# rasd3/3D-Dual-Fusion

Measured on AMD Instinct MI355X. Metric: nuScenes sweeps/sec (0.075 m voxel, ~60k pts), higher is better.
Workload: dtype f32 (fp32-grade throughout: every matrix-core GEMM -- C>=32 sparse convs, neck / head convs, FFN, query linears, image projection, value GEMM -- takes its fp32 operands as fp16 hi+lo pairs, 22 significand bits, 3 MFMA products, fp32 accumulate: <= 4e-6 of scale against float64, the grade of the exac

## Files before the change

3d-dual-fusion_amd/csrc/spconv_split.hip:

```cpp
#include <stdlib.h>
#include <algorithm>
#include <string.h>

#include "common.h"

namespace df3d {

typedef float f32x4 __attribute__((ext_vector_type(4)));
typedef unsigned int u32x4 __attribute__((ext_vector_type(4)));
typedef unsigned int u32x2 __attribute__((ext_vector_type(2)));
typedef __bf16 bf16x8 __attribute__((ext_vector_type(8)));

int timing_rec_begin(int cin, int cout, int kvol, int n_out, const int32_t *nbr, int split,
                     hipStream_t stream);
void timing_rec_end(int rec, hipStream_t stream);

DF3D_SPLIT_OVERFLOW_TU(spconv_split)

__device__ __forceinline__ void split3_pair_ref(float x0, float x1, unsigned &hi, unsigned &mid, unsigned &lo) {
  unsigned h, m;
  split_pair_bf16(x0, x1, h, m);
  const float r0 = (x0 - __uint_as_float(h << 16)) - __uint_as_float(m << 16);
  const float r1 = (x1 - __uint_as_float(h & 0xffff0000u)) - __uint_as_float(m & 0xffff0000u);
  unsigned l, unused;
// ... 58 lines not shown
  u32x4 ho, lo;
  split_pair(a[0], a[1], ho[0], lo[0]);
  split_pair(a[2], a[3], ho[1], lo[1]);
  split_pair(b[0], b[1], ho[2], lo[2]);
  split_pair(b[2], b[3], ho[3], lo[3]);
  out[2 * i] = ho;
  out[2 * i + 1] = lo;
}

__global__ __launch_bounds__(256) void rows_absmax_kernel(const float *__restrict__ x, size_t n4, size_t n, float *__restrict__ part) {
  float m = 0.f;
  const size_t stride = (size_t)gridDim.x * 256;
  size_t i = (size_t)blockIdx.x * 256 + threadIdx.x;
  auto upd = [&](f32x4 v) {
    m = fmaxf(fmaxf(m, fmaxf(__builtin_fabsf(v[0]), __builtin_fabsf(v[1]))), fmaxf(__builtin_fabsf(v[2]), __builtin_fabsf(v[3])));
    if (!(v[0] == v[0]) || !(v[1] == v[1]) || !(v[2] == v[2]) || !(v[3] == v[3])) m = __builtin_inff();
  };
  for (; i + 3 * stride < n4; i += 4 * stride) {
    const f32x4 v0 = ((const f32x4 *)x)[i], v1 = ((const f32x4 *)x)[i + stride], v2 = ((const f32x4 *)x)[i + 2 * stride],
                v3 = ((const f32x4 *)x)[i + 3 * stride];
    upd(v0), upd(v1), upd(v2), upd(v3);
  }
  for (; i < n4; i += stride) upd(((const f32x4 *)x)[i]);
  if (blockIdx.x == 0)
    for (size_t t = n4 * 4 + threadIdx.x; t < n; t += 256) m = fmaxf(m, __builtin_fabsf(x[t]));
#pragma unroll
  for (int o = 32; o > 0; o >>= 1) m = fmaxf(m, __shfl_xor(m, o, 64));
  __shared__ float wm[4];
  if ((threadIdx.x & 63) == 0) wm[threadIdx.x >> 6] = m;
  __syncthreads();
  if (threadIdx.x == 0) part[blockIdx.x] = fmaxf(fmaxf(wm[0], wm[1]), fmaxf(wm[2], wm[3]));
}

constexpr int POW2_PARTS = 1024;
__global__ __launch_bounds__(256) void pow2_scale_kernel(const float *__restrict__ part, int nparts, int channels,
                                                         float *__restrict__ scale, float *__restrict__ inv) {
  float m = 0.f;
  for (int i = threadIdx.x; i < nparts; i += 256) m = fmaxf(m, part[i]);
#pragma unroll
  for (int o = 32; o > 0; o >>= 1) m = fmaxf(m, __shfl_xor(m, o, 64));
  __shared__ float wm[4];
  if ((threadIdx.x & 63) == 0) wm[threadIdx.x >> 6] = m;
  __syncthreads();
  const float amax = fmaxf(fmaxf(wm[0], wm[1]), fmaxf(wm[2], wm[3]));
  float s = 1.f;
  if (amax > 0.f && amax < __builtin_inff()) {
    int k = 9 - ((int)((__float_as_uint(amax) >> 23) & 0xffu) - 127);
    k = k > 120 ? 120 : (k < -120 ? -120 : k);
    s = __uint_as_float((unsigned)(k + 127) << 23);
  }
  const int i = blockIdx.x * 256 + threadIdx.x;
  if (i == 0) scale[0] = s, scale[1] = amax;
  if (i < channels) inv[i] = 1.f / s;
}

__global__ __launch_bounds__(256) void split_rows_scaled_kernel(const float *__restrict__ x, size_t nblk, const float *__restrict__ scale,
                                                                u32x4 *__restrict__ out) {
  size_t i = (size_t)blockIdx.x * blockDim.x + threadIdx.x;
  if (i >= nblk) return;
  const float s = *scale;
  f32x4 a = ((const f32x4 *)x)[2 * i] * s, b = ((const f32x4 *)x)[2 * i + 1] * s;
  u32x4 ho, lo;
  split_pair(a[0], a[1], ho[0], lo[0]);
  split_pair(a[2], a[3], ho[1], lo[1]);
  split_pair(b[0], b[1], ho[2], lo[2]);
  split_pair(b[2], b[3], ho[3], lo[3]);
  out[2 * i] = ho;
  out[2 * i + 1] = lo;
}

__global__ __launch_bounds__(256) void split3_rows_kernel(const float *__restrict__ x, size_t nblk, u32x4 *__restrict__ out) {
  size_t i = (size_t)blockIdx.x * blockDim.x + threadIdx.x;
  if (i >= nblk) return;
  f32x4 a = ((const f32x4 *)x)[2 * i], b = ((const f32x4 *)x)[2 * i + 1];
  u32x4 ho, mo, lo;
  split3_pair(a[0], a[1], ho[0], mo[0], lo[0]);
  split3_pair(a[2], a[3], ho[1], mo[1], lo[1]);
  split3_pair(b[0], b[1], ho[2], mo[2], lo[2]);
  split3_pair(b[2], b[3], ho[3], mo[3], lo[3]);
  out[3 * i] = ho;
  out[3 * i + 1] = mo;
  out[3 * i + 2] = lo;
}

__global__ __launch_bounds__(256) void pack_weights3_kernel(const float *__restrict__ w, int K, int cin, int cout,
                                                            u32x4 *__restrict__ out) {
  const int KB = cin / 32;
  size_t total = (size_t)K * cin * cout / 8 * 3;
  size_t i = (size_t)blockIdx.x * blockDim.x + threadIdx.x;
  if (i >= total) return;
  int lane = (int)(i & 63);
  size_t r = i >> 6;
  int part = (int)(r % 3); r /= 3;
  int n = lane & 15, g = lane >> 4;
  const int CW = cout > 128 ? 128 : cout, CT = CW / 16;
  int ct = (int)(r % CT); r /= CT;
  int kb = (int)(r % KB); r /= KB;
  int k = (int)(r % K);
  int col = (int)(r / K) * CW + n * CT + ct;
  int ch0 = kb * 32 + g * 8;
  unsigned v[8];
#pragma unroll
  for (int e = 0; e < 8; e += 2) {
    unsigned h, m, l;
    split3_pair(w[((size_t)k * cin + ch0 + e) * cout + col], w[((size_t)k * cin + ch0 + e + 1) * cout + col], h, m, l);
    v[e >> 1] = part == 0 ? h : (part == 1 ? m : l);
  }
  out[i] = (u32x4){v[0], v[1], v[2], v[3]};
}

__global__ __launch_bounds__(256) void pack_weights_kernel(const float *__restrict__ w, int K, int cin, int cout,
                                                           u32x4 *__restrict__ out) {
  const int KB = cin / 32;
  size_t total = (size_t)K * cin * cout / 4;
  size_t i = (size_t)blockIdx.x * blockDim.x + threadIdx.x;
  if (i >= total) return;
  int lane = (int)(i & 63);
  size_t r = i >> 6;
  int part = (int)(r & 1); r >>= 1;
  int n = lane & 15, g = lane >> 4;
  const int CW = cout > 128 ? 128 : cout, CT = CW / 16;
  int ct = (int)(r % CT); r /= CT;
  int kb = (int)(r % KB); r /= KB;
  int k = (int)(r % K);
  int col = (int)(r / K) * CW + n * CT + ct;
  int ch0 = kb * 32 + g * 8;
  u32x4 o;
#pragma unroll
  for (int e = 0; e < 4; ++e) {
    unsigned hi, lo;
    split_pair_w(w[((size_t)k * cin + ch0 + 2 * e) * cout + col], w[((size_t)k * cin + ch0 + 2 * e + 1) * cout + col], hi, lo);
    o[e] = part ? lo : hi;
  }
  out[i] = o;
}

struct SplitConvArgs {
  const u32x4 *feat;
  const u32x4 *w;
  const int32_t *nbr;
  const float *bias, *scale, *shift, *residual;
  float *out;
  u32x4 *out_split;
  int n_in, n_out, K, relu;
  int dbg;
  int ldi;
  int in_goff;
  int ldo;
  int gy;
  const int32_t *cols;
  const int32_t *order;
  unsigned long long *trace;
  int cbw;
};

#ifdef DF3D_OS_TRACE
#define OS_STAMP(slot)                                                                                          \
  do {                                                                                                          \
    if (a.trace && (threadIdx.x & 63) == 0)                                                                     \
      a.trace[((size_t)(blockIdx.x + gridDim.x * blockIdx.y) * 16 + (threadIdx.x >> 6)) * 8 + (slot)] =        \
          __builtin_amdgcn_s_memtime();                                                                         \
  } while (0)
static unsigned long long *g_os_trace = nullptr;
extern "C" void df3d_debug_set_os_trace(void *p) { g_os_trace = (unsigned long long *)p; }
#else
#define OS_STAMP(slot) do { } while (0)
#endif

#ifdef DF3D_OS_QGATHER
#define OS_QROW (lane >> 2)
#define OS_QSUB (lane & 3)
#else
#define OS_QROW n
#define OS_QSUB g
#endif
#ifdef DF3D_OS_EXPERIMENTS
#define OS_DBG(bit) ((a.dbg & (bit)) != 0)
#else
#define OS_DBG(bit) false
#endif

#define DF3D_MFMA_BF16(A, B, C) \
  __builtin_amdgcn_mfma_f32_16x16x32_bf16(__builtin_bit_cast(bf16x8, A), __builtin_bit_cast(bf16x8, B), C, 0, 0, 0)
template <int NP>
__device__ __forceinline__ f32x4 mfma_parts(const u32x4 &A, const u32x4 &B, const f32x4 &C) {
  if constexpr (NP == 2) return DF3D_MFMA_F16(A, B, C);
  else return DF3D_MFMA_BF16(A, B, C);
}
template <int NP>
__device__ __forceinline__ constexpr float acc_unscale() { return NP == 2 ? DF3D_ACC_UNSCALE : 1.0f; }

__device__ __forceinline__ int xcd_tile(int bid, int nt) {
  const int q = nt >> 3, r = nt & 7, x = bid & 7;
  return x * q + (x < r ? x : r) + (bid >> 3);
}

__device__ __forceinline__ unsigned lds_addr(const void *p) {
  return (unsigned)(size_t)(const __attribute__((address_space(3))) char *)p;
}

struct StepCursor {
  unsigned m;
  int k, kb;
  bool live;
  __device__ __forceinline__ void init(unsigned mask) {
    m = mask;
    live = mask != 0u;
    k = live ? __builtin_ctz(mask) : 0;
    kb = 0;
  }
  template <int KB>
  __device__ __forceinline__ void next() {
    if (!live) return;
    if (++kb == KB) {
      const unsigned m2 = m & (m - 1u);
      if (m2) {
        m = m2;
        k = __builtin_ctz(m2);
        kb = 0;
      } else {
        live = false;
        kb = KB - 1;
      }
    }
  }
};

__device__ u32x4 g_zero_row[192];

template <int CIN, int COUT, int RT, int NW, int KPS, int NP = 2, int KS = 1, bool MG = false>
__global__ __launch_bounds__(NW * KS * 64) void spconv_os_split_kernel(SplitConvArgs a) {
  constexpr int CW = COUT > 128 ? 128 : COUT;
  constexpr int KB = CIN / 32 / KPS, CT = CW / 16, TM = 16 * RT * NW, WROWS = 16 * RT, RQ = CIN / 4;
  constexpr int WQ = KPS * CT * NP * 64;
  constexpr int NT = NW * 64;
  constexpr int WPT = (WQ + NT - 1) / NT;
  constexpr bool RING3 = KS == 1 && WPT <= 4;
  constexpr int NST = RING3 ? 3 : 2;
  __shared__ u32x4 Wl[KS][NST][WQ];
  __shared__ int nbrL[DF3D_MAX_KVOL][TM];
  __shared__ int rowL[TM];
  __shared__ unsigned wg_mask;

  const int wtid = threadIdx.x, lane = wtid & 63;
  const int grp = KS > 1 ? __builtin_amdgcn_readfirstlane(wtid / NT) : 0;
  const int tid = KS > 1 ? wtid - grp * NT : wtid, wave = tid >> 6;
  const int g = lane >> 4, n = lane & 15;
  int nt = gridDim.x, bid = blockIdx.x, tile = bid;
  tile = xcd_tile(bid, nt);
  const int row0 = tile * TM;
  const int col0 = blockIdx.y * CW;

  OS_STAMP(0);
  if (wtid == 0) wg_mask = 0u;
  __syncthreads();
  {
    constexpr int KSTEP = NT * KS / TM;
    static_assert(NT % TM == 0 && KSTEP >= 1, "tile shape");
    const int r = wtid % TM, k0 = wtid / TM;
    int row = row0 + r;
    row = row < a.n_out ? (a.order ? a.order[row] : row) : a.n_out;
    if (k0 == 0) rowL[r] = row;
    unsigned mine = 0u;
    int v[(DF3D_MAX_KVOL + KSTEP - 1) / KSTEP];
#pragma unroll
    for (int i = 0; i < (DF3D_MAX_KVOL + KSTEP - 1) / KSTEP; ++i) {
      int k = k0 + i * KSTEP;
      v[i] = (k < a.K && row < a.n_out) ? a.nbr[(size_t)k * a.n_out + row] : -1;
    }
#pragma unroll
    for (int i = 0; i < (DF3D_MAX_KVOL + KSTEP - 1) / KSTEP; ++i) {
      int k = k0 + i * KSTEP;
      if (k < a.K) nbrL[k][r] = v[i];
      if (TM >= 64) {
        if (__ballot(v[i] >= 0) != 0ull) mine |= 1u << (k & 31);
      } else if (v[i] >= 0) {
        atomicOr(&wg_mask, 1u << k);
      }
    }
    if (TM >= 64 && lane == 0 && mine) atomicOr(&wg_mask, mine);
  }
  __syncthreads();
  unsigned gmask = __builtin_amdgcn_readfirstlane(wg_mask);
  int nact = __popc(gmask);
  if constexpr (KS > 1) {
    const int per = (nact + KS - 1) / KS;
    unsigned rest = gmask, mine = 0u;
    for (int i = 0; rest; ++i, rest &= rest - 1u)
      if (i / per == grp) mine |= rest & (0u - rest);
    gmask = mine;
    nact = per;
  }
  const int steps = nact * KB;

  f32x4 acc[RT][CT];
#pragma unroll
  for (int rt = 0; rt < RT; ++rt)
#pragma unroll
    for (int ct = 0; ct < CT; ++ct) acc[rt][ct] = (f32x4){0.f, 0.f, 0.f, 0.f};

  constexpr int WD = WPT <= 4 ? 3 : 1;
  u32x4 w0[WPT], w1[WPT], w2[WPT];
  StepCursor cw, ca;
  cw.init(gmask);
  ca.init(gmask);
  auto load_w = [&](u32x4 (&wreg)[WPT]) {
    const u32x4 *src = a.w + ((size_t)blockIdx.y * a.K * KB + (size_t)(cw.k * KB + cw.kb)) * WQ;
#pragma unroll
    for (int i = 0; i < WPT; ++i) {
      int e = tid + NT * i;
      wreg[i] = src[(WQ % NT == 0 || e < WQ) ? e : 0];
    }
    cw.template next<KB>();
  };
  auto store_w = [&](int buf, u32x4 (&wreg)[WPT]) {
#pragma unroll
    for (int i = 0; i < WPT; ++i) {
      int e = tid + NT * i;
      if (WQ % NT == 0 || e < WQ) Wl[grp][buf][e] = wreg[i];
    }
  };
#ifndef DF3D_OS_ADEPTH
#define DF3D_OS_ADEPTH 3
#endif
  constexpr int AD = (RT * KPS * NP <= 4) ? DF3D_OS_ADEPTH : 3;
  static_assert(AD % 3 == 0, "the W register sets rotate with period 3");
  u32x4 ar[AD][RT][KPS][NP];
  int idxn[RT];
  auto peek_a = [&]() {
#pragma unroll
    for (int rt = 0; rt < RT; ++rt) idxn[rt] = nbrL[ca.k][wave * WROWS + rt * 16 + OS_QROW];
  };
  auto issue_a = [&](u32x4 (&dst)[RT][KPS][NP]) {
    const int kb = ca.kb * KPS;
#pragma unroll
    for (int rt = 0; rt < RT; ++rt) {
      const int idx = idxn[rt];
      if constexpr (MG) {
#pragma unroll
        for (int j = 0; j < KPS; ++j)
#pragma unroll
          for (int q = 0; q < NP; ++q) dst[rt][j][q] = (u32x4){0u, 0u, 0u, 0u};
        if (ca.live && idx >= 0) {
          const u32x4 *p = a.feat + (size_t)idx * a.ldi + blockIdx.y * a.in_goff + (kb * 4 + OS_QSUB) * NP;
#pragma unroll
          for (int j = 0; j < KPS; ++j)
#pragma unroll
            for (int q = 0; q < NP; ++q) dst[rt][j][q] = p[j * 4 * NP + q];
        }
        continue;
      }
      const u32x4 *p = (ca.live && idx >= 0 && !OS_DBG(1)) ? a.feat + (size_t)idx * a.ldi + blockIdx.y * a.in_goff
                                                             : g_zero_row;
      p += (kb * 4 + OS_QSUB) * NP;
#pragma unroll
      for (int j = 0; j < KPS; ++j) {
#pragma unroll
        for (int q = 0; q < NP; ++q) dst[rt][j][q] = p[j * 4 * NP + q];
      }
    }
    ca.template next<KB>();
  };
#ifdef DF3D_OS_QGATHER
  u32x4 rdy[RT][KPS][NP];
  auto to_operand = [&](u32x4 (&raw)[RT][KPS][NP]) {
#pragma unroll
    for (int rt = 0; rt < RT; ++rt)
#pragma unroll
      for (int j = 0; j < KPS; ++j)
#pragma unroll
        for (int q = 0; q < NP; ++q)
#pragma unroll
          for (int d = 0; d < 4; ++d)
            rdy[rt][j][q][d] = (unsigned)__builtin_amdgcn_ds_bpermute((4 * n + g) * 4, (int)raw[rt][j][q][d]);
  };
#endif
  constexpr int NBATCH_ = KPS * CT / 2;
  constexpr bool BNEXT_IN_PLACE = RING3 && NBATCH_ % 2 == 0;
  u32x4 bnext[BNEXT_IN_PLACE ? 1 : 2 * NP];
  u32x4 bq[2][2 * NP];
  auto step = [&](int s, u32x4 (&raw)[RT][KPS][NP], u32x4 (&rawn)[RT][KPS][NP], u32x4 (&wset)[WPT]) {
// ... 126 lines not shown
        acc[rt][c2] = mfma_parts<NP>(cur[rt][j][0], bh0, acc[rt][c2]);
        acc[rt][c2 + 1] = mfma_parts<NP>(cur[rt][j][0], bh1, acc[rt][c2 + 1]);
      }
      if (OS_DBG(8)) __builtin_amdgcn_s_setprio(0);
    }
    if constexpr (RING3) {
      const u32x4 *wn = Wl[grp][(s + 1) % 3] + lane;
#pragma unroll
      for (int q = 0; q < 2 * NP; ++q) (BNEXT_IN_PLACE ? bq[0][q] : bnext[q]) = wn[q * 64];
    }
    issue_a(raw);
#ifdef DF3D_OS_QGATHER
    to_operand(rawn);
#else
    (void)rawn;
#endif
  };

  OS_STAMP(1);
  if (steps > 0) {
    if constexpr (RING3) {
      load_w(w0);
      load_w(w1);
      store_w(0, w0);
      store_w(1, w1);
      load_w(w1);
      load_w(w2);
      load_w(w0);
    } else {
    load_w(w0);
    store_w(0, w0);
    if constexpr (WD == 3) {
      load_w(w1);
      load_w(w2);
      load_w(w0);
    } else {
      load_w(w0);
    }
    }
#pragma unroll
    for (int j = 0; j < AD; ++j) {
      peek_a();
      issue_a(ar[j]);
    }
    if constexpr (RING3) {
      __syncthreads();
#pragma unroll
      for (int q = 0; q < 2 * NP; ++q) (BNEXT_IN_PLACE ? bq[0][q] : bnext[q]) = Wl[grp][0][lane + q * 64];
    }
    OS_STAMP(2);
#ifdef DF3D_OS_QGATHER
    to_operand(ar[0]);
#endif
    for (int s = 0; s < steps; s += AD) {
#pragma unroll
      for (int j = 0; j < AD; j += 3) {
        step(s + j, ar[j], ar[(j + 1) % AD], w1);
        step(s + j + 1, ar[j + 1], ar[(j + 2) % AD], w2);
        step(s + j + 2, ar[j + 2], ar[(j + 3) % AD], w0);
      }
    }
  }
  OS_STAMP(3);
#ifdef DF3D_OS_TRACE
  if (a.trace && (threadIdx.x & 63) == 0) a.trace[((size_t)(blockIdx.x + gridDim.x * blockIdx.y) * 16 + (threadIdx.x >> 6)) * 8 + 5] = steps;
#endif

  if constexpr (KS > 1) {
    static_assert((KS - 1) * NW * RT * CT * 64 <= KS * 2 * WQ, "the partial sums must fit the weight stages");
    f32x4 *red = (f32x4 *)&Wl[0][0][0];
    __syncthreads();
    if (grp > 0) {
#pragma unroll
      for (int rt = 0; rt < RT; ++rt)
#pragma unroll
        for (int ct = 0; ct < CT; ++ct) red[((((grp - 1) * NW + wave) * RT + rt) * CT + ct) * 64 + lane] = acc[rt][ct];
    }
    __syncthreads();
    if (grp > 0) return;
#pragma unroll
    for (int q = 1; q < KS; ++q)
#pragma unroll
      for (int rt = 0; rt < RT; ++rt)
#pragma unroll
        for (int ct = 0; ct < CT; ++ct) acc[rt][ct] += red[((((q - 1) * NW + wave) * RT + rt) * CT + ct) * 64 + lane];
  }
  static_assert(CT == 2 || CT == 4 || CT == 8, "COUT must be 32, 64, 128 or 256");
  if constexpr (CT == 2) {
    const int col = col0 + n * 2;
    const float2 bi = a.bias ? *(const float2 *)(a.bias + col) : make_float2(0.f, 0.f);
    const float2 sc = a.scale ? *(const float2 *)(a.scale + col) : make_float2(1.f, 1.f);
    const float2 sh = a.shift ? *(const float2 *)(a.shift + col) : make_float2(0.f, 0.f);
    const int oc0 = a.cols ? a.cols[2 * blockIdx.y] : 0, ocnt = a.cols ? a.cols[2 * blockIdx.y + 1] : 0;
#pragma unroll
    for (int rt = 0; rt < RT; ++rt) {
#pragma unroll
      for (int r = 0; r < 4; ++r) {
        const int row = rowL[wave * WROWS + rt * 16 + 4 * g + r];
        if (row >= a.n_out) continue;
        float2 v = make_float2((acc[rt][0][r] * acc_unscale<NP>() + bi.x) * sc.x + sh.x,
                               (acc[rt][1][r] * acc_unscale<NP>() + bi.y) * sc.y + sh.y);
        if (a.cols) {
          if (a.relu) {
            v.x = fmaxf(v.x, 0.f);
            v.y = fmaxf(v.y, 0.f);
          }
          float *dst = a.out + (size_t)row * a.ldo + oc0 + n * 2;
          if (n * 2 < ocnt) dst[0] = v.x;
          if (n * 2 + 1 < ocnt) dst[1] = v.y;
          continue;
        }
        const size_t o = (size_t)row * a.ldo + col;
        if (a.residual) {
          if constexpr (NP == 1) {
            const unsigned rr = *(const unsigned *)((const char *)a.residual + o * 2);
            v.x += bf16lo_to_f32(rr);
            v.y += bf16hi_to_f32(rr);
          } else {
            const float2 rr = *(const float2 *)(a.residual + o);
            v.x += rr.x;
            v.y += rr.y;
          }
        }
        if (a.relu) {
          v.x = fmaxf(v.x, 0.f);
          v.y = fmaxf(v.y, 0.f);
        }
        if (a.out) *(float2 *)(a.out + o) = v;
        if (a.out_split) {
          if constexpr (NP == 3) {
            unsigned hp, mp, lp;
            split3_pair(v.x, v.y, hp, mp, lp);
            char *blk = (char *)a.out_split + (o >> 3) * 48 + (n & 3) * 4;
            *(unsigned *)blk = hp;
            *(unsigned *)(blk + 16) = mp;
            *(unsigned *)(blk + 32) = lp;
            continue;
          }
          if constexpr (NP == 1) {
            *(unsigned *)((char *)a.out_split + o * 2) = bf16_pair(v.x, v.y);
            continue;
          }
          unsigned hp, lp;
          split_pair(v.x, v.y, hp, lp);
          char *blk = (char *)a.out_split + (o >> 3) * 32 + (n & 3) * 4;
          *(unsigned *)blk = hp;
          *(unsigned *)(blk + 16) = lp;
        }
      }
    }
    OS_STAMP(4);
    return;
  } else {
  f32x4 bi[CT / 4], sc[CT / 4], sh[CT / 4];
#pragma unroll
  for (int q = 0; q < CT / 4; ++q) {
    const int col = col0 + n * CT + q * 4;
    bi[q] = a.bias ? *(const f32x4 *)(a.bias + col) : (f32x4){0.f, 0.f, 0.f, 0.f};
    sc[q] = a.scale ? *(const f32x4 *)(a.scale + col) : (f32x4){1.f, 1.f, 1.f, 1.f};
    sh[q] = a.shift ? *(const f32x4 *)(a.shift + col) : (f32x4){0.f, 0.f, 0.f, 0.f};
  }
#pragma unroll
  for (int rt = 0; rt < RT; ++rt) {
#pragma unroll
    for (int r = 0; r < 4; ++r) {
      const int row = rowL[wave * WROWS + rt * 16 + 4 * g + r];
      if (row >= a.n_out) continue;
      if (OS_DBG(32) && acc[rt][0][r] != 1234.567f) continue;
      const size_t o = (size_t)row * a.ldo + col0 + n * CT;
      unsigned h[CT / 2], l[CT / 2], m3[CT / 2];
#pragma unroll
      for (int q = 0; q < CT / 4; ++q) {
        f32x4 v = (f32x4){acc[rt][q * 4][r], acc[rt][q * 4 + 1][r], acc[rt][q * 4 + 2][r], acc[rt][q * 4 + 3][r]};
        v = (v * acc_unscale<NP>() + bi[q]) * sc[q] + sh[q];
        if (a.residual) {
          if constexpr (NP == 1) {
            const u32x2 rr = *(const u32x2 *)((const char *)a.residual + (o + q * 4) * 2);
            v += (f32x4){bf16lo_to_f32(rr[0]), bf16hi_to_f32(rr[0]), bf16lo_to_f32(rr[1]), bf16hi_to_f32(rr[1])};
          } else {
            v += *(const f32x4 *)(a.residual + o + q * 4);
          }
        }
        if (a.relu) {
          v[0] = fmaxf(v[0], 0.f);
          v[1] = fmaxf(v[1], 0.f);
          v[2] = fmaxf(v[2], 0.f);
          v[3] = fmaxf(v[3], 0.f);
        }
        if (a.out) *(f32x4 *)(a.out + o + q * 4) = v;
        if (a.out_split) {
          if constexpr (NP == 3) {
            split3_pair(v[0], v[1], h[q * 2], m3[q * 2], l[q * 2]);
            split3_pair(v[2], v[3], h[q * 2 + 1], m3[q * 2 + 1], l[q * 2 + 1]);
          } else if constexpr (NP == 1) {
            h[q * 2] = bf16_pair(v[0], v[1]);
            h[q * 2 + 1] = bf16_pair(v[2], v[3]);
          } else {
            split_pair(v[0], v[1], h[q * 2], l[q * 2]);
            split_pair(v[2], v[3], h[q * 2 + 1], l[q * 2 + 1]);
          }
        }
      }
      if constexpr (NP == 3) {
        if (a.out_split) {
          char *blk = (char *)a.out_split + (o >> 3) * 48;
          if constexpr (CT == 8) {
            *(u32x4 *)blk = (u32x4){h[0], h[1], h[2], h[3]};
            *(u32x4 *)(blk + 16) = (u32x4){m3[0], m3[1], m3[2], m3[3]};
            *(u32x4 *)(blk + 32) = (u32x4){l[0], l[1], l[2], l[3]};
          } else {
            blk += (n & 1) * 8;
            *(u32x2 *)blk = (u32x2){h[0], h[1]};
            *(u32x2 *)(blk + 16) = (u32x2){m3[0], m3[1]};
            *(u32x2 *)(blk + 32) = (u32x2){l[0], l[1]};
          }
        }
        continue;
      }
      if (a.out_split && NP == 1) {
        char *dst = (char *)a.out_split + o * 2;
        if constexpr (CT == 8) *(u32x4 *)dst = (u32x4){h[0], h[1], h[2], h[3]};
        else *(u32x2 *)dst = (u32x2){h[0], h[1]};
      } else if (a.out_split) {
        char *blk = (char *)a.out_split + (o >> 3) * 32;
        if constexpr (CT == 8) {
          *(u32x4 *)blk = (u32x4){h[0], h[1], h[2], h[3]};
          *(u32x4 *)(blk + 16) = (u32x4){l[0], l[1], l[2], l[3]};
        } else {
          blk += (n & 1) * 8;
          *(u32x2 *)blk = (u32x2){h[0], h[1]};
          *(u32x2 *)(blk + 16) = (u32x2){l[0], l[1]};
        }
      }
    }
  }
  OS_STAMP(4);
  }
}

template <int CIN, int CW>
__global__ __launch_bounds__(768) void spconv_os_lc_kernel(SplitConvArgs a) {
  constexpr int NP = 2, TM = 128, KB = CIN / 32, NS = 4;
  constexpr int RT = 2, CT = CW / 16;
  static_assert(CW == 128, "column block (a 64-column variant of this structure was measured: 24 KB per 384 MFMA clocks "
                           "makes the loaders the pole, 64 -> 64 K = 27 on 66k rows 85 us against 66 us of the kernel above)");
  constexpr int WQ = CT * NP * 64;
  constexpr int AQ = TM * 8;
  constexpr int NLOAD = 8, APL = 16 / NLOAD, WPL = (WQ / 64) / NLOAD;
  __shared__ u32x4 Al[NS][AQ];
  __shared__ u32x4 Wl[NS][WQ];
  __shared__ int nbrL[DF3D_MAX_KVOL][TM];
  __shared__ int rowL[TM];
  __shared__ unsigned wg_mask;

  const int tid = threadIdx.x, lane = tid & 63, wave = tid >> 6;
  const int g = lane >> 4, n = lane & 15;
  const int tile = xcd_tile(blockIdx.x, gridDim.x);
  const int row0 = tile * TM;
  const int cbw = a.cbw > 0 ? a.cbw : 1;
  const int cb0 = blockIdx.y * cbw;
  const int ncb = min(cbw, a.gy - cb0);
  OS_STAMP(6);

  if (tid == 0) wg_mask = 0u;
  __syncthreads();
  {
    constexpr int KSTEP = 768 / TM;
    constexpr int NPASS = (DF3D_MAX_KVOL + KSTEP - 1) / KSTEP;
    const int r = tid % TM, k0 = tid / TM;
    int row = row0 + r;
    row = row < a.n_out ? (a.order ? a.order[row] : row) : a.n_out;
    if (k0 == 0) rowL[r] = row;
    unsigned mine = 0u;
    int v[NPASS];
#pragma unroll
    for (int i = 0; i < NPASS; ++i) {
      int k = k0 + i * KSTEP;
      v[i] = (k < a.K && row < a.n_out) ? a.nbr[(size_t)k * a.n_out + row] : -1;
    }
#pragma unroll
    for (int i = 0; i < NPASS; ++i) {
      int k = k0 + i * KSTEP;
      if (k < a.K) nbrL[k][r] = v[i];
      if (__ballot(v[i] >= 0) != 0ull) mine |= 1u << (k & 31);
    }
    if (lane == 0 && mine) atomicOr(&wg_mask, mine);
  }
  __syncthreads();
  const unsigned gmask = __builtin_amdgcn_readfirstlane(wg_mask);
  const int steps = __popc(gmask) * KB;
  const int total = steps * ncb;
  auto swz = [](int nn) { return ((nn >> 2) & 1) | (((nn >> 1) & 1) << 2); };
  OS_STAMP(0);
#ifdef DF3D_OS_TRACE
  unsigned long long t_a = 0, t_b = 0, t_c = 0, t_x = 0;
#define LC_T0() t_x = __builtin_amdgcn_s_memtime()
#define LC_ACC(v) do { unsigned long long t_y = __builtin_amdgcn_s_memtime(); v += t_y - t_x; t_x = t_y; } while (0)
#define LC_DUMP()                                                                                                   \
  do {                                                                                                              \
    if (a.trace && lane == 0) {                                                                                     \
      unsigned long long *t_ = a.trace + ((size_t)(blockIdx.x + gridDim.x * blockIdx.y) * 16 + wave) * 8;           \
      t_[1] = t_a, t_[2] = t_b, t_[3] = t_c, t_[5] = steps;                                                         \
    }                                                                                                               \
  } while (0)
#else
#define LC_T0() do { } while (0)
#define LC_ACC(v) do { } while (0)
#define LC_DUMP() do { } while (0)
#endif

  if (wave >= 4) {
    __builtin_amdgcn_s_setprio(3);
    const int lw = wave - 4;
    StepCursor cu;
    cu.init(gmask);
    const u32x4 *abase[APL], *wbase = nullptr;
    int astep[APL];
    int cbl = cb0;
    auto issue = [&](int t) {
      const int st = t & (NS - 1);
      if (cu.kb == 0) {
        int idx[APL];
#pragma unroll
        for (int i = 0; i < APL; ++i) idx[i] = nbrL[cu.k][(lw * APL + i) * 8 + (lane >> 3)];
#pragma unroll
        for (int i = 0; i < APL; ++i) {
          const int r = (lw * APL + i) * 8 + (lane >> 3);
          const int unit = (lane & 7) ^ swz(r & 15);
          abase[i] = idx[i] >= 0 ? a.feat + (size_t)idx[i] * a.ldi + cbl * a.in_goff + unit : g_zero_row + (lane & 7);
          astep[i] = idx[i] >= 0 ? 8 : 0;
        }
        wbase = a.w + ((size_t)cbl * a.K * KB + (size_t)cu.k * KB) * WQ + (lw * WPL) * 64 + lane;
      }
      if (!OS_DBG(64)) {
#pragma unroll
        for (int i = 0; i < APL; ++i)
          __builtin_amdgcn_global_load_lds(abase[i] + cu.kb * astep[i],
                                           (__attribute__((address_space(3))) void *)&Al[st][(lw * APL + i) * 64], 16, 0, 0);
#pragma unroll
        for (int i = 0; i < WPL; ++i)
          __builtin_amdgcn_global_load_lds(wbase + (size_t)cu.kb * WQ + i * 64,
                                           (__attribute__((address_space(3))) void *)&Wl[st][(lw * WPL + i) * 64], 16, 0, 0);
      }
      cu.template next<KB>();
      if (!cu.live) {
        ++cbl;
        cu.init(gmask);
      }
    };
    constexpr int PPS = APL + WPL;
    LC_T0();
    for (int t = 0; t < NS && t < total; ++t) issue(t);
    LC_ACC(t_a);
    for (int s = -1; s < total; ++s) {
      if (s + 3 < total) asm volatile("s_waitcnt vmcnt(%0) lgkmcnt(0)" ::"n"(PPS) : "memory");
      else asm volatile("s_waitcnt vmcnt(0) lgkmcnt(0)" ::: "memory");
      LC_ACC(t_b);
      asm volatile("s_barrier" ::: "memory");
      LC_ACC(t_c);
      if (s >= 0 && s + NS < total) issue(s + NS);
      LC_ACC(t_a);
    }
    LC_DUMP();
    return;
  }

  __builtin_amdgcn_s_setprio(1);
  const int wr = wave;
  f32x4 acc[RT][CT];
#pragma unroll
  for (int rt = 0; rt < RT; ++rt)
#pragma unroll
    for (int ct = 0; ct < CT; ++ct) acc[rt][ct] = (f32x4){0.f, 0.f, 0.f, 0.f};
  const unsigned a_lds = lds_addr(&Al[0][0]) + (unsigned)((wr * 32 + n) * 8) * 16u;
  const unsigned a_addr0 = a_lds + (unsigned)((g * 2) ^ swz(n)) * 16u;
  const unsigned a_addr1 = a_lds + (unsigned)((g * 2 + 1) ^ swz(n)) * 16u;
  const unsigned w_addr = lds_addr(&Wl[0][0]) + (unsigned)lane * 16u;
#define LC_READ(dst, addr, off) asm volatile("ds_read_b128 %0, %1 offset:%2" : "=v"(dst) : "v"(addr), "n"(off))
#define LC_SB() __builtin_amdgcn_sched_barrier(0)
#define LC_M(rt, c, ap, br, buf, slot) acc[rt][c] = DF3D_MFMA_F16(af[buf][rt][ap], bq[slot][br], acc[rt][c])
#define LC_BATCH(i, buf, slot, RA, RB, RC, RD, RE, RF, RG, RH)                    \
  do {                                                                            \
    if (OS_DBG(4)) break;                                                         \
    LC_M(0, (i) * 2, 1, 0, buf, slot); LC_SB(); RA; LC_SB();                      \
    LC_M(0, (i) * 2 + 1, 1, 2, buf, slot); LC_SB(); RB; LC_SB();                  \
    LC_M(1, (i) * 2, 1, 0, buf, slot); LC_SB(); RC; LC_SB();                      \
    LC_M(1, (i) * 2 + 1, 1, 2, buf, slot); LC_SB(); RD; LC_SB();                  \
    LC_M(0, (i) * 2, 0, 1, buf, slot); LC_SB(); RE; LC_SB();                      \
    LC_M(0, (i) * 2 + 1, 0, 3, buf, slot); LC_SB(); RF; LC_SB();                  \
// ... 138 lines not shown
  if (steps == 0)
    for (int cb = cb0; cb < cb0 + ncb; ++cb) epilogue(cb);
  split_range_flag(e_amax);
#undef LC_READ
#undef LC_SB
#undef LC_M
#undef LC_BATCH
#undef LC_BATCH_X
#undef LC_WAITALL
#undef LC_NONE
#undef LC_READ_B4
#undef LC_READ_A4
#undef LC_STEP
  __builtin_amdgcn_s_setprio(0);
  LC_DUMP();
#undef LC_T0
#undef LC_ACC
#undef LC_DUMP
  OS_STAMP(4);

  OS_STAMP(7);
}

static int g_num_cu = 0;
static int num_cu() {
  if (!g_num_cu) {
    hipDeviceProp_t p;
    g_num_cu = (hipGetDeviceProperties(&p, 0) == hipSuccess && p.multiProcessorCount > 0) ? p.multiProcessorCount : 256;
  }
  return g_num_cu;
}

template <int CIN>
static int launch_os_lc(const SplitConvArgs &a_, hipStream_t stream) {
  SplitConvArgs a = a_;
  const int tiles = cdiv(a.n_out, 128), ncu = num_cu();
  int best_ny = a.gy;
  double best = 1e30;
  for (int ny = 1; ny <= a.gy; ++ny) {
    const double cost = (double)cdiv((long long)tiles * ny, ncu) * (cdiv(a.gy, ny) + 0.5);
    if (cost < best - 1e-9) best = cost, best_ny = ny;
  }
  a.cbw = cdiv(a.gy, best_ny);
  static const char *force = getenv("DF3D_LC_CBW");
  if (force && atoi(force) > 0) a.cbw = atoi(force) < a.gy ? atoi(force) : a.gy;
  hipLaunchKernelGGL((spconv_os_lc_kernel<CIN, 128>), dim3(tiles, cdiv(a.gy, a.cbw)), dim3(768), 0, stream, a);
  return DF3D_OK;
}

static bool use_lc(const SplitConvArgs &a) {
  const char *t = getenv("DF3D_OS_LC");
  if (a.cols) return false;
  if (t && t[0] == '0') return false;
  if (t && t[0] == '1') return true;
  return a.K > 1 && (long long)cdiv(a.n_out, 128) * a.gy >= 190;
}


template <int CIN, int COUT>
static int launch_os_split(const SplitConvArgs &a, hipStream_t stream) {
  int rt = 1, nw = a.n_out >= 16 * 1024 ? 8 : 2, kps = 1;
  if constexpr (COUT == 128 && CIN % 32 == 0) {
    if (use_lc(a)) return launch_os_lc<CIN>(a, stream);
  }
  static const char *cfg = getenv("DF3D_OS_CFG");
  if (cfg && cfg[0] && cfg[1] == ',') {
    rt = cfg[0] - '0';
    nw = atoi(cfg + 2);
    const char *c2 = strchr(cfg + 2, ',');
    if (c2) kps = atoi(c2 + 1);
  }
  constexpr int KMAX = CIN >= 64 ? 2 : 1;
  if (kps > KMAX) kps = KMAX;
#define DF3D_OS_LAUNCH(RT, NW, KPS)                                                                      \
  hipLaunchKernelGGL((spconv_os_split_kernel<CIN, COUT, RT, NW, KPS>), dim3(cdiv(a.n_out, 16 * RT * NW), a.gy), \
                     dim3(NW * 64), 0, stream, a)
  if (kps == 2) {
    if (rt == 2) DF3D_OS_LAUNCH(2, 4, KMAX);
    else if (nw == 2) DF3D_OS_LAUNCH(1, 2, KMAX);
    else if (nw == 8) DF3D_OS_LAUNCH(1, 8, KMAX);
    else DF3D_OS_LAUNCH(1, 4, KMAX);
  } else if (nw == 16) DF3D_OS_LAUNCH(1, 16, 1);
  else if (rt == 2 && nw == 8) DF3D_OS_LAUNCH(2, 8, 1);
  else if (nw == 8) {
    const char *mg = getenv("DF3D_OS_MASKED");
    const bool masked = mg ? mg[0] == '1' : (a.K == 27 && !a.cols && CIN == 32);
    if (masked)
      hipLaunchKernelGGL((spconv_os_split_kernel<CIN, COUT, 1, 8, 1, 2, 1, true>), dim3(cdiv(a.n_out, 128), a.gy), dim3(512), 0,
                         stream, a);
    else DF3D_OS_LAUNCH(1, 8, 1);
  }
  else if (rt == 2 && nw == 4) DF3D_OS_LAUNCH(2, 4, 1);
  else if (rt == 2 && nw == 2) DF3D_OS_LAUNCH(2, 2, 1);
  else if (rt == 1 && nw == 4) DF3D_OS_LAUNCH(1, 4, 1);
  else DF3D_OS_LAUNCH(1, 2, 1);
#undef DF3D_OS_LAUNCH
  return DF3D_OK;
}

template <int CIN, int COUT>
static int launch_os_split_wide(const SplitConvArgs &a, hipStream_t stream) {
  const int CS = a.gy;
  if constexpr (COUT % 128 == 0) {
    if (use_lc(a)) return launch_os_lc<CIN>(a, stream);
  }
  int rt = 1, nw = (long long)a.n_out * CS >= 128 * 384 ? 8 : (long long)a.n_out * CS >= 64 * 192 ? 4 : 2;
  static const char *cfg = getenv("DF3D_OS_WIDE");
  if (cfg && cfg[0] && cfg[1] == ',') {
    rt = cfg[0] - '0';
    nw = atoi(cfg + 2);
  }
  if constexpr (CIN <= 256 && COUT % 128 == 0) {
    const char *ks = getenv("DF3D_OS_KSPLIT");
    const long long waves = (long long)cdiv(a.n_out, 64) * CS * 4;
    if (!(cfg && cfg[0]) && nw == 4 && a.K >= 3 && !(ks && ks[0] == '0') && waves <= 6LL * num_cu()) {
      hipLaunchKernelGGL((spconv_os_split_kernel<CIN, COUT, 1, 4, 1, 2, 3>), dim3(cdiv(a.n_out, 64), CS), dim3(768), 0,
                         stream, a);
      return DF3D_OK;
    }
  }
#define DF3D_OS_LAUNCH(RT, NW)                                                                                  \
  hipLaunchKernelGGL((spconv_os_split_kernel<CIN, COUT, RT, NW, 1>), dim3(cdiv(a.n_out, 16 * RT * NW), CS), \
                     dim3(NW * 64), 0, stream, a)
  if (rt == 2 && nw == 4) DF3D_OS_LAUNCH(2, 4);
  else if (rt == 2) DF3D_OS_LAUNCH(2, 2);
  else if (nw == 8) DF3D_OS_LAUNCH(1, 8);
  else if (nw == 4) DF3D_OS_LAUNCH(1, 4);
  else DF3D_OS_LAUNCH(1, 2);
#undef DF3D_OS_LAUNCH
  return DF3D_OK;
}

template <int CIN, int COUT>
static int launch_os_bf16(const SplitConvArgs &a, hipStream_t stream) {
  if ((long long)a.n_out * a.gy >= 16 * 1024)
    hipLaunchKernelGGL((spconv_os_split_kernel<CIN, COUT, 1, 8, 1, 1>), dim3(cdiv(a.n_out, 128), a.gy), dim3(512), 0, stream, a);
  else
    hipLaunchKernelGGL((spconv_os_split_kernel<CIN, COUT, 1, 2, 1, 1>), dim3(cdiv(a.n_out, 32), a.gy), dim3(128), 0, stream, a);
  return DF3D_OK;
}

template <int CIN, int COUT>
static int launch_os_p3(const SplitConvArgs &a, hipStream_t stream) {
  const long long work = (long long)a.n_out * a.gy;
  if (work >= 32 * 1024)
    hipLaunchKernelGGL((spconv_os_split_kernel<CIN, COUT, 1, 8, 1, 3>), dim3(cdiv(a.n_out, 128), a.gy), dim3(512), 0, stream, a);
  else if (work >= 12 * 1024)
    hipLaunchKernelGGL((spconv_os_split_kernel<CIN, COUT, 1, 4, 1, 3>), dim3(cdiv(a.n_out, 64), a.gy), dim3(256), 0, stream, a);
  else
    hipLaunchKernelGGL((spconv_os_split_kernel<CIN, COUT, 1, 2, 1, 3>), dim3(cdiv(a.n_out, 32), a.gy), dim3(128), 0, stream, a);
  return DF3D_OK;
}

#define DF3D_CONV_SHAPES(X) \
  X(256, 256, wide, 1)      \
  X(256, 128, wide, 1)      \
  X(128, 256, wide, 1)      \
  X(512, 64, wide, 0)       \
  X(512, 128, wide, 0)      \
  X(128, 32, os, 0)         \
  X(128, 64, os, 1)         \
  X(128, 128, os, 1)        \
  X(64, 128, os, 1)         \
  X(64, 64, os, 1)          \
  X(32, 64, os, 1)          \
  X(64, 32, os, 1)          \
  X(32, 32, os, 1)

enum { FAM_os, FAM_wide };

template <int NP, int CIN, int COUT, int FAM, bool B16>
static int launch_shape(const SplitConvArgs &a, hipStream_t stream) {
  if constexpr (NP == 3) return launch_os_p3<CIN, COUT>(a, stream);
  else if constexpr (NP == 1 && B16) return launch_os_bf16<CIN, COUT>(a, stream);
  else if constexpr (NP == 1) return DF3D_EINVAL;
  else if constexpr (FAM == FAM_wide) return launch_os_split_wide<CIN, COUT>(a, stream);
  else return launch_os_split<CIN, COUT>(a, stream);
}

static bool shape_ok(int parts, int cin, int cout) {
#define X(CIN, COUT, FAM, B16) \
  if (cin == CIN && cout == COUT) return parts != 1 || B16;
  DF3D_CONV_SHAPES(X)
#undef X
  return false;
}

template <int NP>
static int launch_any(int cin, int cout, const SplitConvArgs &a, hipStream_t stream) {
#define X(CIN, COUT, FAM, B16) \
  if (cin == CIN && cout == COUT) return launch_shape<NP, CIN, COUT, FAM_##FAM, B16>(a, stream);
  DF3D_CONV_SHAPES(X)
#undef X
  return DF3D_EINVAL;
}

struct ConvFormat {
  int parts;
  const char *what;
  int timing;
  int both_bit;
  bool tuning;
  int (*rows)(const float *, long long, int, void *, void *);
  void (*pack_kernel)(const float *, int, int, int, u32x4 *);
  int (*launch)(int cin, int cout, const SplitConvArgs &, hipStream_t);
  int bytes_per_channel() const { return 2 * parts; }
  size_t packed_bytes(int kvol, int cin, int cout) const {
    if (!shape_ok(parts, cin, cout) || kvol <= 0 || kvol > DF3D_MAX_KVOL) return 0;
    return (size_t)kvol * cin * cout * bytes_per_channel();
  }
};

static const ConvFormat g_formats[3] = {
    {1, "bf16", 2, 0, false, df3d_rows_to_bf16, pack_weights_bf16_kernel, launch_any<1>},
    {2, "split-precision", 1, 8, true, df3d_split_rows, pack_weights_kernel, launch_any<2>},
    {3, "three-part", 3, 0, false, df3d_split_rows3, pack_weights3_kernel, launch_any<3>},
};
static const ConvFormat &conv_format(int parts) { return g_formats[parts - 1]; }

static int pack_filters(const ConvFormat &f, const char *entry, const float *filters, int groups, int kvol, int cin, int cout,
                        void *packed, hipStream_t stream) {
  DF3D_CHECK_ARG(filters && packed && groups >= 1, "%s: bad argument", entry);
  DF3D_CHECK_ARG(f.packed_bytes(kvol, cin, cout) != 0 && (groups == 1 || cout <= 128),
                 "%s: shape K=%d cin=%d cout=%d (%d groups) has no %s kernel", entry, kvol, cin, cout, groups, f.what);
  const size_t total = (size_t)groups * kvol * cin * cout / 8 * f.parts;
  hipLaunchKernelGGL(f.pack_kernel, dim3(cdiv((long long)total, 256)), dim3(256), 0, stream, filters, groups * kvol, cin, cout,
                     (u32x4 *)packed);
  DF3D_LAUNCH_CHECK();
  return DF3D_OK;
}

struct ConvCall {
  const void *in;
  int n_in, in_channels, cin, in_group_stride;
  const void *packed;
  int kvol, cout, groups;
  const int32_t *nbr;
  int n_out;
  const float *bias, *scale, *shift;
  const void *residual;
  int relu;
  float *out;
  int out_channels;
  const int32_t *out_cols;
  void *out_rows;
  const int32_t *order;
  bool tag_both;
};

static int conv_launch(const ConvFormat &f, const char *entry, const ConvCall &c, hipStream_t stream) {
  DF3D_CHECK_ARG(c.in && c.packed && c.nbr && (c.out || c.out_rows), "%s: null argument", entry);
  DF3D_CHECK_ARG(c.kvol > 0 && c.kvol <= DF3D_MAX_KVOL, "%s: kernel volume %d unsupported", entry, c.kvol);
  DF3D_CHECK_ARG(shape_ok(f.parts, c.cin, c.cout), "%s: cin=%d cout=%d has no %s kernel", entry, c.cin, c.cout, f.what);
  DF3D_CHECK_ARG(c.groups >= 1 && c.groups <= 65535, "%s: groups", entry);
  DF3D_CHECK_ARG(c.in_channels % 8 == 0 && c.in_group_stride % 8 == 0 && c.in_group_stride >= 0 &&
                     (long long)(c.groups - 1) * c.in_group_stride + c.cin <= c.in_channels,
                 "%s: input columns [g*%d, g*%d+%d) must lie inside the %d-channel rows", entry, c.in_group_stride,
                 c.in_group_stride, c.cin, c.in_channels);
  DF3D_CHECK_ARG(!c.residual || (c.groups == 1 && c.out_channels == c.cout), "%s: a residual needs one group and dense output rows",
                 entry);
  if (c.out_cols) {
    DF3D_CHECK_ARG(c.cout == 32 && !c.out_rows, "%s: compact output columns need cout = 32 and no operand rows out", entry);
  } else {
    DF3D_CHECK_ARG(c.out_channels % 8 == 0 && (long long)c.groups * c.cout <= c.out_channels,
                   "%s: %d x %d output columns do not fit %d-channel rows", entry, c.groups, c.cout, c.out_channels);
  }
  if (c.n_out == 0) return DF3D_OK;
  const char *dbg = f.tuning ? getenv("DF3D_OS_DBG") : nullptr;
  SplitConvArgs a = {(const u32x4 *)c.in, (const u32x4 *)c.packed, c.nbr, c.bias, c.scale, c.shift, (const float *)c.residual,
                     c.out, (u32x4 *)c.out_rows, c.n_in, c.n_out, c.kvol, c.relu, dbg ? atoi(dbg) : 0,
                     c.in_channels / 8 * f.parts, c.in_group_stride / 8 * f.parts, c.out_channels,
                     c.groups * (c.cout > 128 ? c.cout / 128 : 1), c.out_cols, c.order};
#ifdef DF3D_OS_TRACE
  if (f.tuning) a.trace = g_os_trace;
#endif
  int rec = timing_rec_begin(c.cin, c.cout * c.groups, c.kvol, c.n_out, c.nbr,
                             f.timing | (c.tag_both && c.out && c.out_rows ? f.both_bit : 0), stream);
  int rc = f.launch(c.cin, c.cout, a, stream);
  if (rc) return rc;
  timing_rec_end(rec, stream);
  DF3D_LAUNCH_CHECK();
  return DF3D_OK;
}

size_t conv_operand_packed_bytes(int parts, int kvol, int cin, int cout) { return conv_format(parts).packed_bytes(kvol, cin, cout); }

int conv_operand_rows(int parts, const float *x, long long n, int c, void *rows, hipStream_t stream) {
  return conv_format(parts).rows(x, n, c, rows, (void *)stream);
}

int conv_operand_run(int parts, const void *in, int n_in, int cin, const void *packed, int kvol, int cout, const int32_t *nbr,
                     int n_out, const float *bias, const float *scale, const float *shift, const void *residual, int relu,
                     float *out, void *out_rows, hipStream_t stream) {
  const ConvFormat &f = conv_format(parts);
  return conv_launch(f, "backbone_run", ConvCall{in, n_in, cin, cin, 0, packed, kvol, cout, 1, nbr, n_out, bias, scale, shift,
                                                 residual, relu, out, cout, nullptr, out_rows, nullptr, true},
                     stream);
}

}

using namespace df3d;

extern "C" size_t df3d_conv_packed_weight_bytes3(int kvol, int cin, int cout) { return conv_format(3).packed_bytes(kvol, cin, cout); }

extern "C" int df3d_conv_pack_weights3(const float *filters, int groups, int kvol, int cin, int cout, void *packed, void *stream_) {
  return pack_filters(conv_format(3), "conv_pack_weights3", filters, groups, kvol, cin, cout, packed, (hipStream_t)stream_);
}

extern "C" int df3d_split_rows3(const float *features, long long n, int c, void *split3, void *stream_) {
  hipStream_t stream = (hipStream_t)stream_;
  DF3D_CHECK_ARG(features && split3, "split_rows3: null argument");
  DF3D_CHECK_ARG(c > 0 && c % 8 == 0 && n >= 0, "split_rows3: channels must be a multiple of 8 (got %d)", c);
  size_t nblk = (size_t)n * c / 8;
  if (nblk == 0) return DF3D_OK;
  hipLaunchKernelGGL(split3_rows_kernel, dim3(cdiv((long long)nblk, 256)), dim3(256), 0, stream, features, nblk, (u32x4 *)split3);
  DF3D_LAUNCH_CHECK();
  return DF3D_OK;
}

extern "C" int df3d_conv_rows_split3(const void *in_split3, int n_in, int in_channels, int cin, int in_group_stride,
                                     const void *packed3, int kvol, int cout, int groups, const int32_t *nbr, int n_out,
                                     const float *bias, const float *scale, const float *shift, const float *residual,
                                     int relu, float *out, int out_channels, const int32_t *out_cols, void *out_split3,
                                     void *stream_) {
  return conv_launch(conv_format(3), "conv_rows_split3",
                     ConvCall{in_split3, n_in, in_channels, cin, in_group_stride, packed3, kvol, cout, groups, nbr, n_out, bias,
                              scale, shift, residual, relu, out, out_channels, out_cols, out_split3, nullptr, false},
                     (hipStream_t)stream_);
}

extern "C" size_t df3d_conv_packed_weight_bytes(int kvol, int cin, int cout) { return conv_format(2).packed_bytes(kvol, cin, cout); }

extern "C" int df3d_conv_pack_weights(const float *filters, int kvol, int cin, int cout, void *packed, void *stream_) {
  return pack_filters(conv_format(2), "conv_pack_weights", filters, 1, kvol, cin, cout, packed, (hipStream_t)stream_);
}

extern "C" int df3d_conv_pack_weights_groups(const float *filters, int groups, int kvol, int cin, int cout, void *packed,
                                             void *stream_) {
  DF3D_CHECK_ARG(cout <= 128, "conv_pack_weights_groups: shape K=%d cin=%d cout=%d has no grouped split-precision kernel", kvol, cin,
                 cout);
  return pack_filters(conv_format(2), "conv_pack_weights_groups", filters, groups, kvol, cin, cout, packed, (hipStream_t)stream_);
}

static int pow2_scale(const float *x, size_t ne, float *scale, float *inv, int inv_channels, hipStream_t stream) {
  int wgs = 1;
  if (ne) {
    wgs = (int)std::min<size_t>(POW2_PARTS, cdiv((long long)(ne / 4), 256 * 4) + 1);
    hipLaunchKernelGGL(rows_absmax_kernel, dim3(wgs), dim3(256), 0, stream, x, ne / 4, ne, scale + 2);
  } else {
    DF3D_HIP(hipMemsetAsync(scale + 2, 0, sizeof(float), stream));
  }
  hipLaunchKernelGGL(pow2_scale_kernel, dim3(std::max(1, cdiv(inv_channels, 256))), dim3(256), 0, stream, scale + 2, wgs,
                     inv_channels, scale, inv ? inv : scale);
  return DF3D_OK;
}

extern "C" int df3d_pow2_scale_floats(void) { return 2 + POW2_PARTS; }

extern "C" int df3d_split_rows_scaled(const float *features, long long n, int c, void *split, float *scale, float *inv_scale,
                                      int inv_channels, void *stream_) {
  hipStream_t stream = (hipStream_t)stream_;
  DF3D_CHECK_ARG(features && split && scale && inv_scale, "split_rows_scaled: null argument");
  DF3D_CHECK_ARG(c > 0 && c % 8 == 0 && n >= 0 && inv_channels >= 1, "split_rows_scaled: channels must be a multiple of 8 (got %d)", c);
  DF3D_CHECK_ARG((size_t)features % 16 == 0, "split_rows_scaled: rows must be 16-byte aligned");
  const size_t ne = (size_t)n * c, nblk = ne / 8;
  int rc = pow2_scale(features, ne, scale, inv_scale, inv_channels, stream);
  if (rc) return rc;
  if (nblk)
    hipLaunchKernelGGL(split_rows_scaled_kernel, dim3(cdiv((long long)nblk, 256)), dim3(256), 0, stream, features, nblk, scale,
                       (u32x4 *)split);
  DF3D_LAUNCH_CHECK();
  return DF3D_OK;
}

extern "C" int df3d_rows_pow2_scale(const float *x, long long n_elems, float *scale, void *stream_) {
  hipStream_t stream = (hipStream_t)stream_;
  DF3D_CHECK_ARG(x && scale && n_elems >= 0, "rows_pow2_scale: bad argument");
  DF3D_CHECK_ARG((size_t)x % 16 == 0, "rows_pow2_scale: rows must be 16-byte aligned");
  int rc = pow2_scale(x, (size_t)n_elems, scale, nullptr, 0, stream);
  if (rc) return rc;
  DF3D_LAUNCH_CHECK();
  return DF3D_OK;
}

extern "C" int df3d_split_rows(const float *features, long long n, int c, void *split, void *stream_) {
  hipStream_t stream = (hipStream_t)stream_;
  DF3D_CHECK_ARG(features && split, "split_rows: null argument");
  DF3D_CHECK_ARG(c > 0 && c % 8 == 0 && n >= 0, "split_rows: channels must be a multiple of 8 (got %d)", c);
  size_t nblk = (size_t)n * c / 8;
  if (nblk == 0) return DF3D_OK;
  hipLaunchKernelGGL(split_rows_kernel, dim3(cdiv((long long)nblk, 256)), dim3(256), 0, stream, features, nblk,
                     (u32x4 *)split);
  DF3D_LAUNCH_CHECK();
  return DF3D_OK;
}

extern "C" int df3d_sparse_conv_split(const void *features_split, int n_in, int cin, const void *packed_filters,
                                      int kvol, int cout, const int32_t *nbr, int n_out, const float *bias,
                                      const float *scale, const float *shift, const float *residual, int relu,
                                      float *out, void *out_split, const int32_t *tile_rows, int ntiles,
                                      void *stream_) {
  return conv_launch(conv_format(2), "sparse_conv_split",
                     ConvCall{features_split, n_in, cin, cin, 0, packed_filters, kvol, cout, 1, nbr, n_out, bias, scale, shift,
                              residual, relu, out, cout, nullptr, out_split, ntiles == -1 ? tile_rows : nullptr, true},
                     (hipStream_t)stream_);
}

extern "C" int df3d_conv_rows_split(const void *in_split, int n_in, int in_channels, int cin, int in_group_stride,
                                    const void *packed_filters, int kvol, int cout, int groups, const int32_t *nbr,
                                    int n_out, const float *bias, const float *scale, const float *shift, int relu,
                                    float *out, int out_channels, const int32_t *out_cols, void *out_split,
                                    void *stream_) {
  return conv_launch(conv_format(2), "conv_rows_split",
                     ConvCall{in_split, n_in, in_channels, cin, in_group_stride, packed_filters, kvol, cout, groups, nbr, n_out,
                              bias, scale, shift, nullptr, relu, out, out_channels, out_cols, out_split, nullptr, false},
                     (hipStream_t)stream_);
}

extern "C" int df3d_rows_to_bf16(const float *features, long long n, int c, void *rows_bf16, void *stream_) {
  hipStream_t stream = (hipStream_t)stream_;
  DF3D_CHECK_ARG(c > 0 && c % 8 == 0 && n >= 0, "rows_to_bf16: channels must be a multiple of 8 (got %d)", c);
  size_t nblk = (size_t)n * c / 8;
  if (nblk == 0) return DF3D_OK;
  DF3D_CHECK_ARG(features && rows_bf16, "rows_to_bf16: null argument");
  hipLaunchKernelGGL(bf16_rows_kernel, dim3(cdiv((long long)nblk, 256)), dim3(256), 0, stream, features, nblk,
                     (u32x4 *)rows_bf16);
  DF3D_LAUNCH_CHECK();
  return DF3D_OK;
}

extern "C" int df3d_rows_from_bf16(const void *rows_bf16, long long n, int c, float *features, void *stream_) {
  hipStream_t stream = (hipStream_t)stream_;
  DF3D_CHECK_ARG(c > 0 && c % 8 == 0 && n >= 0, "rows_from_bf16: channels must be a multiple of 8 (got %d)", c);
  size_t nblk = (size_t)n * c / 8;
  if (nblk == 0) return DF3D_OK;
  DF3D_CHECK_ARG(features && rows_bf16, "rows_from_bf16: null argument");
  hipLaunchKernelGGL(bf16_rows_to_f32_kernel, dim3(cdiv((long long)nblk, 256)), dim3(256), 0, stream,
                     (const u32x4 *)rows_bf16, nblk, features);
  DF3D_LAUNCH_CHECK();
  return DF3D_OK;
}

extern "C" size_t df3d_conv_packed_weight_bytes_bf16(int kvol, int cin, int cout) { return conv_format(1).packed_bytes(kvol, cin, cout); }

extern "C" int df3d_conv_pack_weights_bf16(const float *filters, int kvol, int cin, int cout, void *packed,
                                           void *stream_) {
  return pack_filters(conv_format(1), "conv_pack_weights_bf16", filters, 1, kvol, cin, cout, packed, (hipStream_t)stream_);
}

extern "C" int df3d_sparse_conv_bf16(const void *features_bf16, int n_in, int cin, const void *packed_filters, int kvol,
                                     int cout, const int32_t *nbr, int n_out, const float *bias, const float *scale,
                                     const float *shift, const void *residual_bf16, int relu, float *out,
                                     void *out_bf16, void *stream_) {
  return conv_launch(conv_format(1), "sparse_conv_bf16",
                     ConvCall{features_bf16, n_in, cin, cin, 0, packed_filters, kvol, cout, 1, nbr, n_out, bias, scale, shift,
                              residual_bf16, relu, out, cout, nullptr, out_bf16, nullptr, true},
                     (hipStream_t)stream_);
}
```

3d-dual-fusion_amd/dualfusion/_lib.py:

```python
import ctypes
import os

_HERE = os.path.dirname(os.path.abspath(__file__))
LIB_PATH = os.path.join(os.path.dirname(_HERE), "csrc", "libdf3d_hip.so")

c_int = ctypes.c_int
c_uint = ctypes.c_uint
c_longlong = ctypes.c_longlong
c_size_t = ctypes.c_size_t
c_float = ctypes.c_float
c_void_p = ctypes.c_void_p
c_ulonglong = ctypes.c_ulonglong
c_char_p = ctypes.c_char_p

SIGNATURES = {
    "df3d_version": (c_int, []),
    "df3d_last_error": (c_char_p, []),
    "df3d_device_count": (c_int, []),
    "df3d_device_arch": (c_int, [c_char_p, c_int]),
    "df3d_split_overflow": (c_int, [c_int, c_char_p, c_int]),
    "df3d_split_overflow_collect": (c_int, [c_void_p, c_int, c_void_p]),
    "df3d_split_overflow_units": (c_int, [c_char_p, c_int]),
    "df3d_hard_voxelize_workspace_bytes": (c_size_t, [c_int, c_int, c_int]),
    "df3d_hard_voxelize": (c_int, [c_void_p, c_int, c_int, c_void_p, c_void_p, c_int, c_int, c_int,
                                   c_void_p, c_void_p, c_void_p, c_void_p, c_void_p, c_void_p, c_size_t, c_void_p]),
    "df3d_hard_voxelize_batched": (c_int, [c_void_p, c_int, c_int, c_void_p, c_void_p, c_int, c_int, c_int, c_int,
                                           c_void_p, c_void_p, c_void_p, c_void_p, c_void_p, c_void_p, c_size_t,
                                           c_void_p]),
    "df3d_grid_bytes": (c_size_t, [c_int, c_void_p]),
    "df3d_grid_build": (c_int, [c_void_p, c_int, c_int, c_void_p, c_void_p, c_size_t, c_void_p, c_void_p]),
    "df3d_subm_neighbors": (c_int, [c_void_p, c_void_p, c_void_p, c_int, c_int, c_void_p, c_void_p, c_void_p,
                                    c_void_p, c_void_p]),
    "df3d_conv_out_indices": (c_int, [c_void_p, c_int, c_int, c_void_p, c_void_p, c_void_p, c_void_p, c_void_p,
                                      c_void_p, c_void_p, c_size_t, c_void_p, c_int, c_void_p, c_void_p]),
    "df3d_conv_neighbors": (c_int, [c_void_p, c_void_p, c_void_p, c_int, c_int, c_void_p, c_void_p, c_void_p,
                                    c_void_p, c_void_p, c_void_p, c_void_p]),
    "df3d_conv_transpose_out_indices": (c_int, [c_void_p, c_int, c_int, c_void_p, c_void_p, c_void_p, c_void_p, c_void_p,
                                                c_void_p, c_void_p, c_size_t, c_void_p, c_int, c_void_p, c_void_p]),
    "df3d_conv_transpose_neighbors": (c_int, [c_void_p, c_void_p, c_void_p, c_int, c_int, c_void_p, c_void_p, c_void_p,
                                              c_void_p, c_void_p, c_void_p, c_void_p]),
    "df3d_nbr_to_pairs_workspace_bytes": (c_size_t, [c_int, c_int]),
    "df3d_nbr_to_pairs": (c_int, [c_void_p, c_int, c_int, c_int, c_void_p, c_void_p, c_void_p, c_size_t, c_void_p]),
    "df3d_pairs_to_nbr": (c_int, [c_void_p, c_void_p, c_int, c_int, c_int, c_void_p, c_void_p]),
    "df3d_sparse_conv_fused": (c_int, [c_void_p, c_int, c_int, c_void_p, c_int, c_int, c_void_p, c_int,
                                       c_void_p, c_void_p, c_void_p, c_void_p, c_int, c_void_p, c_void_p]),
    "df3d_nbr_row_lists_bytes": (c_size_t, [c_int, c_int]),
    "df3d_nbr_row_lists": (c_int, [c_void_p, c_int, c_int, c_int, c_void_p, c_size_t, c_void_p]),
    "df3d_sparse_conv_fused_lists": (c_int, [c_void_p, c_int, c_int, c_void_p, c_int, c_int, c_void_p, c_void_p, c_int, c_void_p,
                                             c_void_p, c_void_p, c_void_p, c_int, c_void_p, c_void_p, c_void_p]),
    "df3d_sparse_conv_grouped": (c_int, [c_void_p, c_int, c_int, c_int, c_int, c_void_p, c_int, c_int, c_int, c_void_p, c_int,
                                         c_void_p, c_void_p, c_void_p, c_int, c_void_p, c_int, c_int, c_void_p]),
    "df3d_conv_tile_count": (c_int, [c_int, c_int, c_int, c_int]),
    "df3d_conv_tiles_workspace_bytes": (c_size_t, [c_int]),
    "df3d_conv_tiles": (c_int, [c_void_p, c_int, c_int, c_int, c_void_p, c_void_p, c_size_t, c_void_p]),
    "df3d_sparse_conv_fused_tiled": (c_int, [c_void_p, c_int, c_int, c_void_p, c_int, c_int, c_void_p, c_int,
                                             c_void_p, c_void_p, c_void_p, c_void_p, c_int, c_void_p, c_void_p, c_int,
                                             c_void_p]),
    "df3d_timing_begin": (c_int, []),
    "df3d_timing_end": (c_int, []),
    "df3d_timing_get": (c_int, [c_int, c_void_p, c_void_p]),
    "df3d_sparse_to_dense": (c_int, [c_void_p, c_void_p, c_int, c_int, c_int, c_void_p, c_void_p, c_void_p]),
    "df3d_ms_deform_attn_forward": (c_int, [c_void_p, c_void_p, c_void_p, c_void_p, c_void_p,
                                            c_int, c_int, c_int, c_int, c_int, c_int, c_int, c_void_p, c_void_p]),
    "df3d_ms_deform_attn_backward": (c_int, [c_void_p, c_void_p, c_void_p, c_void_p, c_void_p, c_void_p, c_int, c_int,
                                             c_int, c_int, c_int, c_int, c_int, c_void_p, c_void_p, c_void_p, c_void_p]),
    "df3d_ms_deform_attn_backward_binned_workspace_bytes": (c_size_t, [c_int, c_int, c_int, c_int, c_int, c_int]),
    "df3d_ms_deform_attn_backward_binned_slab_bytes": (c_size_t, [c_int, c_int, c_int, c_int, c_int, c_int, c_int]),
    "df3d_ms_deform_attn_backward_binned": (c_int, [c_void_p] * 6 + [c_int] * 7 + [c_void_p] * 4 + [c_size_t, c_void_p, c_void_p]),
    "df3d_ms_deform_attn_backward_plan": (c_int, [c_int] * 7 + [c_void_p, c_void_p, c_int]),
    "df3d_ms_deform_attn_backward_binned_ml_workspace_bytes": (c_size_t, [c_int] * 5 + [c_void_p, c_int]),
    "df3d_ms_deform_attn_backward_binned_ml_slab_bytes": (c_size_t, [c_int] * 6 + [c_void_p]),
    "df3d_ms_deform_attn_backward_binned_ml": (c_int, [c_void_p] * 8 + [c_int] * 7 + [c_void_p] * 4 + [c_size_t, c_void_p, c_void_p]),
    "df3d_ms_deform_attn_forward_f64": (c_int, [c_void_p] * 5 + [c_int] * 7 + [c_void_p, c_void_p]),
    "df3d_ms_deform_attn_backward_f64_workspace_bytes": (c_size_t, [c_int] * 6),
    "df3d_ms_deform_attn_backward_f64": (c_int, [c_void_p] * 6 + [c_int] * 7 + [c_void_p] * 4 + [c_size_t, c_void_p]),
    "df3d_furthest_point_sample": (c_int, [c_void_p, c_int, c_int, c_int, c_void_p, c_void_p, c_void_p]),
    "df3d_pe_gather_add": (c_int, [c_void_p, c_void_p, c_void_p, c_void_p, c_void_p, c_void_p, c_void_p, c_longlong, c_int, c_int,
                                   c_void_p, c_void_p]),
    "df3d_group_attention": (c_int, [c_void_p, c_int, c_int, c_int, c_int, c_void_p, c_void_p]),
    "df3d_group_attention_split": (c_int, [c_void_p, c_int, c_int, c_int, c_int, c_void_p, c_void_p, c_void_p]),
    "df3d_group_attention_backward": (c_int, [c_void_p, c_void_p, c_int, c_int, c_int, c_int, c_void_p, c_void_p]),
    "df3d_ball_query": (c_int, [c_void_p, c_void_p, c_int, c_int, c_int, c_float, c_float, c_int, c_void_p, c_void_p]),
    "df3d_group_points": (c_int, [c_void_p, c_void_p, c_int, c_int, c_int, c_int, c_int, c_void_p, c_void_p]),
    "df3d_gather_points": (c_int, [c_void_p, c_void_p, c_int, c_int, c_int, c_int, c_void_p, c_void_p]),
    "df3d_project_voxels": (c_int, [c_void_p, c_int, c_int, c_int, c_void_p, c_void_p, c_void_p, c_void_p, c_void_p,
                                    c_void_p, c_float, c_void_p, c_void_p, c_void_p, c_void_p, c_void_p, c_void_p,
                                    c_void_p]),
    "df3d_scatter_to_image": (c_int, [c_void_p, c_void_p, c_void_p, c_void_p, c_void_p, c_int, c_int, c_int, c_int,
                                      c_int, c_int, c_void_p, c_void_p, c_void_p]),
    "df3d_assemble_queries": (c_int, [c_void_p, c_void_p, c_void_p, c_void_p, c_void_p, c_void_p, c_void_p,
                                      c_int, c_int, c_int, c_int, c_int, c_int, c_int, c_int,
                                      c_void_p, c_void_p, c_void_p, c_void_p, c_void_p]),
    "df3d_scatter_winner": (c_int, [c_void_p, c_void_p, c_void_p, c_int, c_int, c_int, c_int, c_int, c_void_p, c_void_p]),
    "df3d_gate_scatter_rows": (c_int, [c_void_p, c_int, c_void_p, c_void_p, c_void_p, c_void_p, c_void_p, c_int, c_int, c_int,
                                       c_int, c_int, c_void_p, c_void_p, c_int, c_void_p]),
    "df3d_gate_scatter": (c_int, [c_void_p, c_void_p, c_void_p, c_void_p, c_int, c_int, c_int, c_int, c_int,
                                  c_void_p, c_void_p, c_int, c_void_p]),
    "df3d_gate_finish": (c_int, [c_void_p, c_void_p, c_void_p, c_int, c_int, c_int, c_void_p, c_void_p]),
    "df3d_query_pixel_rows_workspace_bytes": (c_size_t, [c_int, c_int, c_int, c_int]),
    "df3d_query_pixel_rows": (c_int, [c_void_p, c_void_p, c_void_p, c_int, c_int, c_int, c_int, c_int, c_void_p, c_void_p,
                                      c_void_p, c_size_t, c_void_p]),
    "df3d_assemble_queries2_compact": (c_int, [c_void_p, c_void_p, c_void_p, c_void_p, c_void_p, c_void_p, c_void_p, c_void_p,
                                               c_void_p, c_int, c_int, c_int, c_int, c_int, c_int, c_int, c_int, c_void_p,
                                               c_void_p, c_void_p, c_void_p, c_void_p, c_void_p, c_void_p]),
    "df3d_imgproj_split_compact": (c_int, [c_void_p, c_int, c_int, c_int, c_void_p, c_void_p, c_void_p, c_void_p, c_void_p,
                                           c_void_p]),
    "df3d_gate_rows": (c_int, [c_void_p, c_int, c_void_p, c_void_p, c_void_p, c_int, c_int, c_int, c_void_p, c_int, c_void_p]),
    "df3d_gate_finish_bias": (c_int, [c_void_p, c_void_p, c_void_p, c_void_p, c_int, c_int, c_int, c_void_p, c_void_p]),
    "df3d_fusion_writeback_split": (c_int, [c_void_p, c_void_p, c_void_p, c_void_p, c_void_p, c_int, c_int, c_int, c_int,
                                            c_void_p, c_void_p, c_void_p]),
    "df3d_sparse_to_dense_rows_split": (c_int, [c_void_p, c_void_p, c_int, c_int, c_int, c_void_p, c_void_p, c_void_p]),
    "df3d_query_slots": (c_int, [c_void_p, c_void_p, c_int, c_int, c_int, c_void_p, c_void_p, c_void_p]),
    "df3d_assemble_queries2": (c_int, [c_void_p, c_void_p, c_void_p, c_void_p, c_void_p, c_void_p, c_void_p,
                                       c_void_p, c_void_p, c_int, c_int, c_int, c_int, c_int, c_int, c_int, c_int,
                                       c_void_p, c_void_p, c_void_p, c_void_p, c_void_p, c_void_p, c_void_p]),
    "df3d_assemble_queries2_slots": (c_int, [c_void_p, c_void_p, c_void_p, c_void_p, c_void_p, c_void_p, c_void_p,
                                             c_void_p, c_void_p, c_int, c_int, c_int, c_int, c_int, c_int, c_int, c_int,
                                             c_void_p, c_void_p, c_void_p, c_void_p, c_void_p, c_void_p, c_void_p, c_void_p,
                                             c_void_p, c_void_p]),
    "df3d_conv_packed_weight_bytes": (c_size_t, [c_int, c_int, c_int]),
    "df3d_conv_pack_weights": (c_int, [c_void_p, c_int, c_int, c_int, c_void_p, c_void_p]),
    "df3d_bn_rows_supported": (c_int, [c_int]),
    "df3d_bn_rows_scratch_doubles": (c_int, [c_int]),
    "df3d_bn_rows_forward": (c_int, [c_void_p, c_longlong, c_int, c_void_p, c_void_p, c_float, c_float, c_int, c_void_p,
                                     c_void_p, c_void_p, c_void_p, c_void_p, c_void_p]),
    "df3d_bn_rows_backward": (c_int, [c_void_p, c_void_p, c_longlong, c_int, c_void_p, c_int, c_void_p, c_void_p, c_void_p,
                                      c_void_p, c_void_p]),
    "df3d_conv_pack_weights_groups": (c_int, [c_void_p, c_int, c_int, c_int, c_int, c_void_p, c_void_p]),
    "df3d_split_rows_scaled": (c_int, [c_void_p, c_longlong, c_int, c_void_p, c_void_p, c_void_p, c_int, c_void_p]),
    "df3d_split_rows": (c_int, [c_void_p, c_longlong, c_int, c_void_p, c_void_p]),
    "df3d_sparse_conv_split": (c_int, [c_void_p, c_int, c_int, c_void_p, c_int, c_int, c_void_p, c_int, c_void_p,
                                       c_void_p, c_void_p, c_void_p, c_int, c_void_p, c_void_p, c_void_p, c_int,
                                       c_void_p]),
    "df3d_ffn_packed_bytes": (c_size_t, [c_int, c_int]),
    "df3d_ffn_pack": (c_int, [c_void_p, c_void_p, c_int, c_int, c_void_p, c_void_p]),
    "df3d_ffn_fused": (c_int, [c_void_p, c_longlong, c_int, c_int, c_void_p, c_void_p, c_void_p, c_void_p, c_void_p,
                               c_void_p, c_float, c_void_p, c_void_p]),
    "df3d_ffn_set_precision": (c_int, [c_int]),
    "df3d_ffn_fused_jobs": (c_int, [c_void_p, c_int, c_int, c_int, c_void_p]),
    "df3d_timing_count_pairs": (c_int, [c_int]),
    "df3d_timing_filter": (c_int, [c_int, c_int, c_int]),
    "df3d_timing_sample": (c_int, [c_int]),
    "df3d_timing_get2": (c_int, [c_int, c_void_p, c_void_p, c_void_p, c_void_p]),
    "df3d_sparse_to_dense_rows": (c_int, [c_void_p, c_void_p, c_int, c_int, c_int, c_void_p, c_void_p, c_void_p]),
    "df3d_conv2d_neighbors": (c_int, [c_int, c_int, c_int, c_int, c_int, c_int, c_int, c_int, c_void_p, c_void_p]),
    "df3d_rows_to_bf16": (c_int, [c_void_p, ctypes.c_longlong, c_int, c_void_p, c_void_p]),
    "df3d_rows_from_bf16": (c_int, [c_void_p, ctypes.c_longlong, c_int, c_void_p, c_void_p]),
    "df3d_conv_packed_weight_bytes_bf16": (c_size_t, [c_int, c_int, c_int]),
    "df3d_conv_pack_weights_bf16": (c_int, [c_void_p, c_int, c_int, c_int, c_void_p, c_void_p]),
    "df3d_sparse_conv_bf16": (c_int, [c_void_p, c_int, c_int, c_void_p, c_int, c_int, c_void_p, c_int, c_void_p, c_void_p,
                                      c_void_p, c_void_p, c_int, c_void_p, c_void_p, c_void_p]),
    "df3d_invert_neighbors": (c_int, [c_void_p, c_int, c_int, c_int, c_void_p, c_void_p]),
    "df3d_chanfirst_dot": (c_int, [c_void_p, c_void_p, c_int, c_int, c_longlong, c_void_p, c_void_p]),
    "df3d_sparse_conv_grad_filters_scaled": (c_int, [c_void_p, c_int, c_int, c_void_p, c_int, c_int, c_void_p, c_int, c_void_p,
                                                    c_void_p, c_void_p]),
    "df3d_sparse_conv_grad_filters_bf16": (c_int, [c_void_p, c_int, c_int, c_void_p, c_int, c_int, c_void_p, c_int, c_void_p, c_void_p]),
    "df3d_rows_grad_weights_scaled": (c_int, [c_void_p, c_void_p, c_longlong, c_int, c_int, c_void_p, c_void_p, c_void_p, c_void_p]),
    "df3d_grad_filters_kernel": (c_int, [c_int, c_int, c_int, c_int, c_int]),
    "df3d_pow2_scale_floats": (c_int, []),
    "df3d_rows_pow2_scale": (c_int, [c_void_p, c_longlong, c_void_p, c_void_p]),
    "df3d_rows_grad_weights": (c_int, [c_void_p, c_void_p, c_longlong, c_int, c_int, c_void_p, c_void_p]),
    "df3d_sparse_conv_grad_filters": (c_int, [c_void_p, c_int, c_int, c_void_p, c_int, c_int, c_void_p, c_int, c_void_p,
                                              c_void_p]),
    "df3d_conv_rows_split": (c_int, [c_void_p, c_int, c_int, c_int, c_int, c_void_p, c_int, c_int, c_int, c_void_p, c_int,
                                     c_void_p, c_void_p, c_void_p, c_int, c_void_p, c_int, c_void_p, c_void_p, c_void_p]),
    "df3d_conv_packed_weight_bytes3": (c_size_t, [c_int, c_int, c_int]),
    "df3d_conv_pack_weights3": (c_int, [c_void_p, c_int, c_int, c_int, c_int, c_void_p, c_void_p]),
    "df3d_split_rows3": (c_int, [c_void_p, ctypes.c_longlong, c_int, c_void_p, c_void_p]),
    "df3d_conv_rows_split3": (c_int, [c_void_p, c_int, c_int, c_int, c_int, c_void_p, c_int, c_int, c_int, c_void_p, c_int,
                                      c_void_p, c_void_p, c_void_p, c_void_p, c_int, c_void_p, c_int, c_void_p, c_void_p,
                                      c_void_p]),
    "df3d_boxes_bev_pairwise": (c_int, [c_void_p, c_int, c_void_p, c_int, c_int, c_void_p, c_void_p]),
    "df3d_nms_bev_workspace_bytes": (c_size_t, [c_int, c_int]),
    "df3d_nms_bev": (c_int, [c_void_p, c_void_p, c_int, c_int, c_float, c_int, c_int, c_void_p, c_void_p, c_void_p,
                             c_size_t, c_void_p]),
    "df3d_centerhead_predict_workspace_bytes": (c_size_t, [c_int, c_void_p]),
    "df3d_centerhead_predict": (c_int, [c_void_p, c_int, c_void_p, c_void_p, c_void_p, c_void_p, c_void_p, c_void_p,
                                        c_size_t, c_void_p]),
    "df3d_head_final_conv": (c_int, [c_void_p, c_int, c_int, c_int, c_int, c_int, c_void_p, c_void_p, c_void_p, c_void_p,
                                     c_int, c_void_p]),
    "df3d_head_final_packed_bytes": (c_size_t, [c_int]),
    "df3d_head_final_pack": (c_int, [c_void_p, c_int, c_void_p, c_void_p]),
    "df3d_head_final_conv_packed": (c_int, [c_void_p, c_int, c_int, c_int, c_int, c_int, c_void_p, c_void_p, c_void_p,
                                            c_void_p, c_int, c_void_p]),
    "df3d_head_final_conv_backward": (c_int, [c_void_p, c_int, c_void_p, c_int, c_int, c_int, c_int, c_int, c_void_p, c_void_p,
                                              c_void_p, c_void_p, c_void_p]),
    "df3d_centerhead_loss_workspace_bytes": (c_size_t, [c_int, c_int, c_int, c_int]),
    "df3d_centerhead_loss": (c_int, [c_void_p, c_void_p, c_int, c_int, c_int, c_int, c_int, c_int, c_void_p, c_int, c_float,
                                     c_void_p, c_void_p, c_size_t, c_void_p]),
    "df3d_centerhead_loss_grad": (c_int, [c_void_p, c_void_p, c_void_p, c_int, c_int, c_int, c_int, c_int, c_int, c_void_p, c_int, c_float,
                                     c_void_p, c_void_p, c_size_t, c_void_p]),
    "df3d_centerhead_loss_slots": (c_int, [c_void_p, c_void_p, c_int, c_int, c_int, c_int, c_int, c_int, c_void_p, c_int, c_float,
                                           c_void_p, c_void_p, c_size_t, c_void_p]),
    "df3d_head_regress_packed_bytes": (c_size_t, [c_int]),
    "df3d_head_regress_pack": (c_int, [c_void_p, c_int, c_void_p, c_void_p]),
    "df3d_head_regress_at": (c_int, [c_void_p, c_int, c_int, c_int, c_void_p, c_int, c_int, c_int, c_void_p, c_void_p, c_void_p,
                                     c_void_p, c_void_p, c_void_p, c_void_p, c_void_p, c_void_p]),
    "df3d_heatmap_proposals_workspace_bytes":(c_size_t, [c_int, c_int, c_int, c_int]),
    "df3d_heatmap_proposals": (c_int, [c_void_p, c_int, c_int, c_int, c_int, c_int, c_int, c_uint, c_int, c_void_p, c_int,
                                       c_int, c_void_p, c_void_p, c_void_p, c_void_p, c_void_p, c_void_p, c_void_p,
                                       c_void_p, c_size_t, c_void_p]),
    "df3d_transfusion_decode": (c_int, [c_void_p, c_void_p, c_void_p, c_int, c_int, c_int, c_void_p, c_void_p, c_void_p,
                                        c_void_p, c_void_p, c_void_p]),
    "df3d_furthest_point_sample_with_dist": (c_int, [c_void_p, c_int, c_int, c_int, c_void_p, c_void_p, c_void_p]),
    "df3d_group_points_grad": (c_int, [c_void_p, c_void_p, c_int, c_int, c_int, c_int, c_int, c_void_p, c_void_p]),
    "df3d_gather_points_grad": (c_int, [c_void_p, c_void_p, c_int, c_int, c_int, c_int, c_void_p, c_void_p]),
    "df3d_rows_linear_packed_bytes": (c_size_t, [c_int, c_int]),
    "df3d_rows_linear": (c_int, [c_void_p, c_void_p, c_void_p, c_longlong, c_int, c_void_p, c_int, c_int, c_void_p, c_void_p, c_int,
                                 c_int, c_void_p, c_int, c_int, c_void_p, c_void_p, c_void_p, c_float, c_void_p]),
    "df3d_voxel_image_sample": (c_int, [c_void_p, c_int, c_int, c_float, c_void_p, c_void_p, c_void_p, c_void_p, c_void_p, c_int, c_int,
                                        c_int, c_int, c_int, c_float, c_float, c_void_p, c_void_p, c_void_p, c_void_p, c_void_p,
                                        c_void_p]),
    "df3d_backbone_inputs_ready": (c_int, [c_void_p]),
    "df3d_lt_layer_packed_bytes": (c_longlong, []),
    "df3d_lt_layer_vector_floats": (c_int, []),
    "df3d_lt_layer": (c_int, [c_void_p, c_int, c_int, c_int, c_int, c_int, c_int, c_void_p, c_void_p, c_float, c_float, c_void_p, c_void_p]),
    "df3d_lt_layer_pe_packed_bytes": (c_longlong, []),
    "df3d_lt_layer_pe_vector_floats": (c_int, []),
    "df3d_lt_layer_gather": (c_int, [c_void_p, c_void_p, c_void_p, c_int, c_void_p, c_void_p, c_float, c_float, c_void_p, c_void_p]),
    "df3d_lt_layer_scatter": (c_int, [c_void_p, c_int, c_void_p, c_void_p, c_float, c_float, c_void_p, c_void_p, c_void_p]),
    "df3d_boxes_overlap_bev_xyxyr": (c_int, [c_void_p, c_int, c_void_p, c_int, c_void_p, c_void_p]),
    "df3d_tf_match_cost": (c_int, [c_void_p, c_int, c_int, c_int, c_int, c_int, c_void_p, c_void_p, c_void_p, c_int, c_int,
                                   c_void_p, c_void_p, c_void_p, c_void_p, c_void_p]),
    "df3d_draw_heatmap_gaussian": (c_int, [c_void_p, c_void_p, c_void_p, c_int, c_int, c_int, c_int, c_int, c_int, c_void_p,
                                           c_void_p, c_void_p]),
    "df3d_gaussian_focal_loss_workspace_bytes": (c_size_t, [c_longlong]),
    "df3d_gaussian_focal_loss": (c_int, [c_void_p, c_longlong, c_longlong, c_longlong, c_void_p, c_int, c_int, c_int, c_float,
                                         c_float, c_float, c_void_p, c_void_p, c_void_p, c_size_t, c_void_p]),
    "df3d_tf_query_loss": (c_int, [c_void_p, c_void_p, c_void_p, c_int, c_int, c_int, c_int, c_int, c_int, c_int, c_void_p,
                                   c_void_p, c_void_p, c_int, c_int, c_void_p, c_void_p, c_void_p, c_void_p]),
    "df3d_sparse_maxpool": (c_int, [c_void_p, c_int, c_int, c_void_p, c_int, c_int, c_void_p, c_void_p]),
    "df3d_sparse_maxpool_backward": (c_int, [c_void_p, c_void_p, c_void_p, c_int, c_int, c_void_p, c_int, c_void_p, c_void_p]),
    "df3d_dynamic_voxelize": (c_int, [c_void_p, c_longlong, c_int, c_void_p, c_void_p, c_void_p, c_void_p]),
    "df3d_dynamic_scatter_plan_workspace_bytes": (c_size_t, [c_longlong, c_void_p]),
    "df3d_dynamic_scatter_plan": (c_int, [c_void_p, c_longlong, c_int] + [c_void_p] * 7 + [c_size_t, c_void_p]),
    "df3d_dynamic_scatter_reduce": (c_int, [c_void_p, c_int, c_int, c_void_p, c_void_p, c_int, c_int, c_void_p, c_void_p]),
    "df3d_voxel_to_point": (c_int, [c_void_p, c_int, c_int, c_void_p, c_void_p, c_longlong, c_void_p, c_void_p]),
    "df3d_dynamic_scatter_max_backward": (c_int, [c_void_p, c_void_p, c_void_p, c_int, c_longlong, c_int, c_int, c_void_p,
                                                  c_void_p, c_void_p, c_void_p]),
    "df3d_topk_keys_workspace_bytes": (c_size_t, [c_int, c_longlong, c_int]),
    "df3d_topk_keys": (c_int, [c_void_p, c_int, c_longlong, c_int, c_void_p, c_void_p, c_void_p, c_size_t, c_void_p]),
    "df3d_cross_attention_workspace_bytes": (c_size_t, [c_int, c_int, c_int, c_int]),
    "df3d_cross_attention_train": (c_int, [c_void_p, c_int, c_void_p, c_int, c_void_p, c_int, c_int, c_int, c_int, c_int, c_int,
                                           c_float, c_float, c_ulonglong, c_void_p, c_int, c_void_p, c_void_p, c_size_t, c_void_p]),
    "df3d_cross_attention_backward": (c_int, [c_void_p, c_int, c_void_p, c_int, c_void_p, c_int, c_void_p, c_int, c_void_p,
                                              c_void_p, c_int, c_int, c_int, c_int, c_int, c_float, c_float, c_ulonglong,
                                              c_void_p, c_int, c_void_p, c_int, c_void_p, c_int, c_void_p]),
    "df3d_cross_attention": (c_int, [c_void_p, c_int, c_void_p, c_int, c_void_p, c_int, c_int, c_int, c_int, c_int, c_int,
                                     c_float, c_void_p, c_int, c_void_p, c_size_t, c_void_p]),
    "df3d_imgproj_packed_bytes": (c_size_t, [c_int, c_int]),
    "df3d_imgproj_pack": (c_int, [c_void_p, c_int, c_int, c_void_p, c_void_p]),
    "df3d_imgproj_split": (c_int, [c_void_p, c_int, c_int, c_int, c_void_p, c_void_p, c_void_p, c_void_p]),
    "df3d_value_fold_gemm": (c_int, [c_void_p, c_void_p, c_int, c_int, c_void_p, c_void_p, c_void_p, c_float, c_int,
                                     c_void_p, c_void_p, c_void_p, c_void_p, c_void_p, c_void_p, c_void_p]),
    "df3d_value_fold_gemm_bf16": (c_int, [c_void_p, c_void_p, c_int, c_int, c_void_p, c_void_p, c_void_p, c_float, c_int,
                                          c_void_p, c_void_p, c_void_p, c_void_p, c_void_p, c_void_p, c_void_p]),
    "df3d_backbone_run": (c_int, [c_void_p, c_int, c_void_p, c_void_p, c_int, c_int, c_int, c_void_p, c_void_p,
                                  c_size_t, c_void_p, c_void_p, c_void_p]),
    "df3d_backbone_geometry": (c_int, [c_void_p, c_int, c_void_p, c_int, c_int, c_int, c_void_p, c_void_p, c_size_t, c_void_p,
                                       c_void_p, c_void_p, c_void_p]),
    "df3d_backbone_convs": (c_int, [c_void_p, c_void_p, c_void_p, c_size_t, c_void_p, c_void_p, c_void_p]),
    "df3d_backbone_convs_range": (c_int, [c_void_p, c_void_p, c_int, c_int, c_void_p, c_size_t, c_void_p, c_void_p, c_void_p]),
    "df3d_backbone_geometry_wait": (c_int, [c_void_p, c_void_p]),
    "df3d_frame_head_image_wait": (c_int, [c_void_p, c_void_p]),
    "df3d_head_worker_create": (c_void_p, [c_int]),
    "df3d_head_worker_destroy": (c_int, [c_void_p]),
    "df3d_frame_head_submit": (c_int, [c_void_p, c_void_p, c_void_p, c_size_t, c_void_p]),
    "df3d_frame_head_wait": (c_int, [c_void_p, c_void_p, c_void_p, c_void_p, c_void_p]),
    "df3d_backbone_release": (c_int, [c_void_p]),
    "df3d_actr_prep": (c_int, [c_void_p, c_void_p, c_void_p, c_longlong, c_int, c_void_p, c_void_p, c_void_p]),
    "df3d_relu_dropout_bf16": (c_int, [c_void_p, c_longlong, c_float, c_ulonglong, c_void_p]),
    "df3d_relu_dropout_backward_bf16": (c_int, [c_void_p, c_void_p, c_longlong, c_float, c_void_p, c_void_p]),
    "df3d_relu_dropout": (c_int, [c_void_p, c_longlong, c_float, c_ulonglong, c_void_p]),
    "df3d_relu_dropout_backward": (c_int, [c_void_p, c_void_p, c_longlong, c_float, c_void_p, c_void_p]),
    "df3d_dropout_add_layernorm": (c_int, [c_void_p, c_void_p, c_void_p, c_void_p, c_float, c_float, c_ulonglong, c_longlong, c_int,
                                           c_void_p, c_void_p, c_void_p, c_void_p]),
    "df3d_dropout_add_layernorm_backward": (c_int, [c_void_p, c_void_p, c_void_p, c_void_p, c_float, c_ulonglong, c_longlong, c_int,
                                                    c_void_p, c_void_p, c_void_p, c_void_p, c_void_p]),
    "df3d_add_layernorm": (c_int, [c_void_p, c_void_p, c_void_p, c_void_p, c_float, c_longlong, c_int, c_void_p,
                                   c_void_p]),
    "df3d_add_layernorm_split": (c_int, [c_void_p, c_void_p, c_void_p, c_void_p, c_float, c_longlong, c_int, c_void_p,
                                   c_void_p, c_void_p]),
    "df3d_bigate_sum": (c_int, [c_void_p, c_void_p, c_void_p, c_void_p, c_void_p, c_void_p, c_longlong, c_int,
                                c_void_p, c_void_p, c_void_p]),
    "df3d_ms_deform_attn_fused": (c_int, [c_void_p, c_longlong, c_void_p, c_void_p, c_void_p, c_void_p, c_void_p,
                                          c_void_p, c_void_p, c_longlong,
                                          c_int, c_int, c_int, c_int, c_int, c_int, c_int, c_void_p, c_void_p]),
    "df3d_ms_deform_attn_fused_bf16": (c_int, [c_void_p, c_longlong, c_void_p, c_void_p, c_void_p, c_void_p, c_void_p,
                                               c_void_p, c_void_p, c_longlong,
                                               c_int, c_int, c_int, c_int, c_int, c_int, c_int, c_void_p, c_void_p]),
    "df3d_rows_groupnorm": (c_int, [c_void_p, c_int, c_int, c_int, c_int, c_void_p, c_void_p, c_float, c_void_p,
                                    c_void_p, c_void_p]),
    "df3d_scaled_moments": (c_int, [c_void_p, c_longlong, c_longlong, c_void_p, c_int, c_int, c_int, c_void_p,
                                    c_void_p]),
    "df3d_groupnorm_fold": (c_int, [c_void_p, c_void_p, c_void_p, c_void_p, c_float, c_int, c_int, c_int, c_int,
                                    c_void_p, c_void_p, c_int, c_void_p, c_void_p, c_void_p]),
    "df3d_fusion_writeback": (c_int, [c_void_p, c_void_p, c_void_p, c_void_p, c_void_p, c_int, c_int, c_int, c_int,
                                      c_void_p, c_void_p]),
}

_lib = None


DF3D_OK, DF3D_EINVAL, DF3D_ENOMEM, DF3D_EHIP = 0, -1, -2, -3


class Df3dError(RuntimeError):
    pass


class StreamArg(c_void_p):
    """What ops._stream() passes as the stream of a launch: lets a recording launch tape (dualfusion/tape.py) tell launches
    from queries and find the argument to rewrite."""


_recorder = None


# ... 34 lines not shown
```

3d-dual-fusion_amd/dualfusion/apitimer.py:

```python
import ctypes

from . import _lib

_NO_STREAM = ("df3d_version", "df3d_last_error", "df3d_device_count", "df3d_device_arch", "df3d_timing_", "df3d_ffn_set_precision",
              "df3d_conv_tile_count", "df3d_bn_rows_supported", "df3d_bn_rows_scratch_doubles", "df3d_debug_")
CONV_ENTRIES = ("df3d_sparse_conv_fused", "df3d_sparse_conv_grouped", "df3d_sparse_conv_fused_tiled", "df3d_sparse_conv_split", "df3d_sparse_conv_bf16",
                "df3d_conv_rows_split", "df3d_backbone_run")


def _ops_stream():
    from . import ops
    return ops._stream()


def _ival(a):
    if isinstance(a, bool):
        return int(a)
    if isinstance(a, int):
        return a
    if isinstance(a, (ctypes.c_int, ctypes.c_longlong, ctypes.c_size_t, ctypes.c_uint)):
        return int(a.value)
    if isinstance(a, float):
        return a
    if isinstance(a, ctypes.c_float):
        return float(a.value)
    return None


class _Proxy(object):
    def __init__(self, real, timer):
        self.__dict__["_real"], self.__dict__["_timer"], self.__dict__["_cache"] = real, timer, {}

    def __getattr__(self, name):
        fn = getattr(self._real, name)
        if not name.startswith("df3d_") or name.endswith("_bytes") or any(name.startswith(p) for p in _NO_STREAM):
            return fn
        w = self._cache.get(name)
        if w is None:
            timer = self._timer

            def w(*args, _fn=fn, _name=name):
                return timer._call(_name, _fn, args)
            self._cache[name] = w
        return w


class ApiTimer(object):
    def __init__(self):
        self.hip = ctypes.CDLL("libamdhip64.so")
        self.hip.hipEventCreate.argtypes = [ctypes.POINTER(ctypes.c_void_p)]
        self.hip.hipEventRecord.argtypes = [ctypes.c_void_p, ctypes.c_void_p]
        self.hip.hipEventElapsedTime.argtypes = [ctypes.POINTER(ctypes.c_float), ctypes.c_void_p, ctypes.c_void_p]
        self.hip.hipEventDestroy.argtypes = [ctypes.c_void_p]
        self.hip.hipDeviceSynchronize.argtypes = []
        self._raw, self.records, self._real = [], [], None

    def _event(self):
        e = ctypes.c_void_p()
        if self.hip.hipEventCreate(ctypes.byref(e)) != 0:
            raise _lib.Df3dError("hipEventCreate failed")
        return e

    def _call(self, name, fn, args):
        stream = args[-1] if args else None
        if isinstance(stream, int):
            stream = ctypes.c_void_p(stream)
        if not isinstance(stream, ctypes.c_void_p) or (stream.value or 0) != (_ops_stream().value or 0):
            return fn(*args)
        extra = None
        if name == "df3d_ffn_fused_jobs":
            try:
                arr = getattr(args[0], "_obj", args[0])
                extra = sum(int(arr[i].rows) for i in range(int(_ival(args[1]))))
            except Exception:
                extra = None
        elif name == "df3d_centerhead_loss_slots":
            try:
                arr = getattr(args[0], "_obj", args[0])
                extra = sum(int(arr[i].num_classes) for i in range(int(_ival(args[2]))))
            except Exception:
                extra = None
        e0, e1 = self._event(), self._event()
        self.hip.hipEventRecord(e0, stream)
        rc = fn(*args)
        self.hip.hipEventRecord(e1, stream)
        self._raw.append((name, e0, e1, tuple(_ival(a) for a in args), extra))
        return rc

    def start(self):
        self._real = _lib.load()
        _lib._lib = _Proxy(self._real, self)
        return self

    def stop(self):
        _lib._lib = self._real
        self.hip.hipDeviceSynchronize()
        ms = ctypes.c_float()
        for name, e0, e1, ints, extra in self._raw:
            self.hip.hipEventElapsedTime(ctypes.byref(ms), e0, e1)
            self.records.append(dict(name=name, ms=float(ms.value), args=ints, extra=extra))
            self.hip.hipEventDestroy(e0)
            self.hip.hipEventDestroy(e1)
        self._raw = []
        return self.records


def _msda(a, value_bytes=4):
    N, S, M, D, Lq, L, P = a[10:17]
    by = min(N * S * M * D, N * Lq * M * L * P * 4 * D) * value_bytes + N * Lq * M * L * P * 12 + N * Lq * M * D * 4
    return by, 10 * N * Lq * M * L * P * D, "hbm", "bilinear sampling + weighted sum of %d x %d queries, %d heads x %d points" % (N, Lq, M, L * P)


def _msda_f64(a, at, backward=False):
    N, S, M, D, Lq, L, P = a[at:at + 7]
    value_bytes = 8
    pts = N * Lq * M * L * P
    by = min(N * S * M * D, pts * 4 * D) * value_bytes + pts * 3 * value_bytes + N * Lq * M * D * value_bytes
    what = "bilinear sampling + weighted sum of %d x %d queries, %d heads x %d points, float64" % (N, Lq, M, L * P)
    if not backward:
        return by, 10 * pts * D, "hbm", what
    by += N * Lq * M * D * value_bytes + N * S * M * D * value_bytes + pts * 3 * value_bytes + pts * 4 * 4 * 3 + N * S * M * 12
    return by, 30 * pts * D, "hbm", "backward of " + what + " (ordered sums, no float atomics)"


def _ffn(a, rows):
    d_model, d_ffn = a[2], a[3]
    if rows is None:
        return None, None, "mfma", "fused feed-forward"
    return rows * d_model * 8 + 2 * d_model * d_ffn * 4, 4 * rows * d_model * d_ffn, "mfma", "LayerNorm(x + W2 relu(W1 x)) of %d query rows" % rows


def _imgproj(a):
    nimg, cin, S = a[1], a[2], a[3]
    return nimg * S * (cin * 4 + 512 + 4), 2 * nimg * S * cin * 144, "hbm", "u = Wcat[144 x %d] img of %d maps x %d pixels -> split rows + gate" % (cin, nimg, S)


def _value_gemm(a, out_bytes=4):
    nimg, S = a[2], a[3]
    return nimg * S * (512 * 2 + 256 * out_bytes), 2 * nimg * S * 128 * 256 + 4 * nimg * S * 128, "hbm", "GroupNorm moments + folded value GEMM [%d x %d px, 128] -> 256" % (nimg, S)


def _assemble(a):
    n, C, Ci, B, ncam, H, W, max_ne = a[9:17]
    return B * ncam * max_ne * (C + Ci + 5) * 4, 0, "hbm", "gather of %d x %d query slots: %d voxel + %d image channels" % (B * ncam, max_ne, C, Ci)


def _rows(elems_in, elems_out, what):
    return (elems_in + elems_out) * 4, 0, "hbm", what


def _regress_at(a):
    B, H, W, T, M, NB = a[1], a[2], a[3], a[5], a[6], a[7]
    banks = T * NB
    by = banks * (147456 + 9 * 64 * 4 * 4) + T * B * M * (9 + 40)
    return by, 0, "hbm", "regression branches at the live ones of %d object slots, %d tasks x %d branches (latency-bound)" % (B * M, T, NB)


def _loss_slots(a, classes):
    n, B, H, W, M, D = a[2:8]
    if classes is None:
# ... 78 lines not shown
```

3d-dual-fusion_amd/dualfusion/heads.py:

```python
import copy
import os

import torch
from torch import nn

from . import ops as _ops
from .registry import HEADS


def _clamped_sigmoid(x):
    return torch.clamp(x.sigmoid_(), min=1e-4, max=1 - 1e-4)


def _transpose_and_gather_feat(feat, ind):
    feat = feat.permute(0, 2, 3, 1).contiguous()
    feat = feat.view(feat.size(0), -1, feat.size(3))
    return feat.gather(1, ind.unsqueeze(2).expand(ind.size(0), ind.size(1), feat.size(2)))


def reg_loss(output, mask, ind, target):
    pred = _transpose_and_gather_feat(output, ind)
    mask = mask.float().unsqueeze(2)
    loss = torch.nn.functional.l1_loss(pred * mask, target * mask, reduction='none')
    loss = loss / (mask.sum() + 1e-4)
# ... 166 lines not shown
        for k in ("_row_plan", "_row_fit", "_plan_tensors"):
            self.__dict__.pop(k, None)
        return super(CenterHead, self).train(mode)

    def _state_tensors(self):
        ts = self.__dict__.get("_plan_tensors")
        if ts is None:
            ts = self.__dict__["_plan_tensors"] = list(self.parameters()) + list(self.buffers())
        return ts

    def _row_kernels_fit(self, x):
        hit = self.__dict__.get("_row_fit")
        if hit is None:
            hit = self.__dict__["_row_fit"] = self._row_kernels_fit_uncached()
        return hit

    def _row_kernels_fit_uncached(self):
        sc = self.shared_conv[0]
        ok = sc.in_channels == 512 and sc.out_channels == 64 and sc.kernel_size == (3, 3)
        for task in self.tasks:
            for head in task.heads:
                fc = getattr(task, head)
                ok = ok and len(fc) == 4 and isinstance(fc[1], nn.BatchNorm2d) and fc[0].kernel_size == (3, 3) \
                    and fc[0].out_channels == 64 and fc[3].out_channels <= 32
        return ok

    def _train_rows_fit(self):
        bns = [getattr(task, head)[1] for task in self.tasks for head in task.heads]
        fcs = [getattr(task, head) for task in self.tasks for head in task.heads]
        return (all(fc[3].out_channels <= 4 and fc[3].bias is not None and fc[0].bias is not None for fc in fcs)
                and all((b.momentum, b.eps, b.training, b.affine, b.track_running_stats) ==
                        (bns[0].momentum, bns[0].eps, bns[0].training, bns[0].affine, bns[0].track_running_stats) for b in bns))

    @staticmethod
    def _filters(conv, pad_to=None):
        w = conv.weight.detach().float().permute(2, 3, 1, 0).reshape(9, conv.in_channels, conv.out_channels)
        if pad_to is not None and pad_to > conv.out_channels:
            w = torch.cat([w, w.new_zeros(9, conv.in_channels, pad_to - conv.out_channels)], 2)
        return w.contiguous()

    @staticmethod
    def _fold(bn):
        scale = bn.weight.float() * torch.rsqrt(bn.running_var.float() + bn.eps)
        return scale, bn.bias.float() - bn.running_mean.float() * scale

    def _plan(self):
        key = tuple((p.data_ptr(), p._version) for p in self._state_tensors()) + (_ops.split_parts(),)
        plan = self.__dict__.get("_row_plan")
        if plan is not None and plan["key"] == key:
            return plan
        sc, sbn = self.shared_conv[0], self.shared_conv[1]
        s_scale, s_shift = self._fold(sbn)
        dev = sc.weight.device
        mid_filters, mid_bias, mid_scale, mid_shift, fin_packed, fin_bias, cols, layout = [], [], [], [], [], [], [], []
        fin_w4, fin_b4 = [], []
        c0 = 0
        for t, task in enumerate(self.tasks):
            for head in task.heads:
                fc = getattr(task, head)
                mid_filters.append(self._filters(fc[0]))
                mid_bias.append(fc[0].bias.detach().float())
                a, b = self._fold(fc[1])
                mid_scale.append(a)
                mid_shift.append(b)
                k = fc[3].out_channels
                fin_packed.append(_ops.conv_pack_weights(self._filters(fc[3], 32)))
                fin_bias.append(torch.cat([fc[3].bias.detach().float(), torch.zeros(32 - k, device=dev)]))
                if k <= 4:
                    fin_w4.append(self._filters(fc[3], 4))
                    fin_b4.append(torch.cat([fc[3].bias.detach().float(), torch.zeros(4 - k, device=dev)]))
                cols.append((c0, k))
                layout.append((t, head, c0, k))
                c0 += k
        mid_pair = 2 if len(mid_filters) % 2 == 0 else 1
        mid_packed = [_ops.conv_pack_weights(torch.cat(mid_filters[i:i + mid_pair], dim=2).contiguous())
                      for i in range(0, len(mid_filters), mid_pair)]
        plan = dict(key=key, shared=_ops.conv_pack_weights(self._filters(sc)), s_bias=sc.bias.detach().float().contiguous(),
                    s_scale=s_scale.contiguous(), s_shift=s_shift.contiguous(),
                    mid=torch.cat(mid_packed), mid_pair=mid_pair, mid_bias=torch.cat(mid_bias).contiguous(),
                    mid_scale=torch.cat(mid_scale).contiguous(), mid_shift=torch.cat(mid_shift).contiguous(),
                    fin=torch.cat(fin_packed), fin_bias=torch.cat(fin_bias).contiguous(),
                    cols=torch.tensor(cols, dtype=torch.int32, device=dev).contiguous(), layout=layout,
                    groups=len(cols), width=(c0 + 7) // 8 * 8, nbr={},
                    fin_w4=torch.stack(fin_w4).contiguous() if len(fin_w4) == len(cols) else None,
                    fin_b4=torch.stack(fin_b4).contiguous() if len(fin_b4) == len(cols) else None)
        self.__dict__["_row_plan"] = plan
        return plan

    @torch.no_grad()
    def forward_rows_fp32(self, x):
        from .necks import _rows_of
        key = tuple((p.data_ptr(), p._version) for p in self._state_tensors())
        plan = self.__dict__.get("_row_plan_fp32")
        if plan is None or plan["key"] != key:
            sc, sbn = self.shared_conv[0], self.shared_conv[1]
            dev = sc.weight.device
            s_scale, s_shift = self._fold(sbn)
            branches = [(t, head, getattr(task, head)) for t, task in enumerate(self.tasks) for head in task.heads]
            nb = len(branches)
            per = int(os.environ.get("DF3D_HEAD_FP32_PAIR", "2"))
            if nb % per:
                per = 1
            folds = [self._fold(fc[1]) for _, _, fc in branches]
            mid_w = torch.stack([torch.cat([self._filters(fc[0]) for _, _, fc in branches[i:i + per]], 2)
                                 for i in range(0, nb, per)]).contiguous()
            mid_bias = torch.cat([fc[0].bias.detach().float() if fc[0].bias is not None else torch.zeros(64, device=dev)
                                  for _, _, fc in branches]).contiguous()
            kp = 16 if max(fc[3].out_channels for _, _, fc in branches) <= 16 else 32
            fin_w = torch.stack([self._filters(fc[3], kp) for _, _, fc in branches]).contiguous()
            fin_b = torch.cat([torch.cat([fc[3].bias.detach().float() if fc[3].bias is not None
                                          else torch.zeros(fc[3].out_channels, device=dev),
                                          torch.zeros(kp - fc[3].out_channels, device=dev)]) for _, _, fc in branches]).contiguous()
            plan = dict(key=key, shared=self._filters(sc), s_bias=sc.bias.detach().float().contiguous() if sc.bias is not None else None,
                        s_scale=s_scale.contiguous(), s_shift=s_shift.contiguous(), branches=branches, kp=kp,
                        mid_w=mid_w, mid_bias=mid_bias, mid_scale=torch.cat([f[0] for f in folds]).contiguous(),
                        mid_shift=torch.cat([f[1] for f in folds]).contiguous(), fin_w=fin_w, fin_b=fin_b, nbr={})
            self.__dict__["_row_plan_fp32"] = plan
        B, _, H, W = x.shape
        rows, _ = _rows_of(x)
        if (B, H, W) not in plan["nbr"]:
            plan["nbr"][(B, H, W)] = _ops.conv2d_neighbors(B, H, W, 3, 3, 1, 1, False, x.device)[0]
        nbr = plan["nbr"][(B, H, W)]
        n = B * H * W
        s1 = _ops.sparse_conv_fused(rows.contiguous(), plan["shared"], nbr, n, bias=plan["s_bias"], scale=plan["s_scale"],
                                    shift=plan["s_shift"], relu=True)
        mid = _ops.sparse_conv_grouped(s1, plan["mid_w"], nbr, n, bias=plan["mid_bias"], scale=plan["mid_scale"],
                                       shift=plan["mid_shift"], relu=True, group_in=0)
        out = _ops.sparse_conv_grouped(mid, plan["fin_w"], nbr, n, bias=plan["fin_b"], group_in=64)
        rets = [dict() for _ in self.tasks]
        kp = plan["kp"]
        for i, (t, head, fc) in enumerate(plan["branches"]):
            k = fc[3].out_channels
            r = out[:, i * kp:i * kp + k]
            v = r.view(B, H, W, k).permute(0, 3, 1, 2)
            v._df3d_rows = (r, None, v._version)
            rets[t][head] = v
        return rets

    @torch.no_grad()
    def forward_rows(self, x):
        from .necks import _rows_of
        plan = self._plan()
        B, _, H, W = x.shape
        rows, split = _rows_of(x)
        if (split is None or split.dtype != torch.uint8
                or split.shape[1] != _ops.split_width(rows.shape[1])):
            split = _ops.split_rows(rows.contiguous())
        if (B, H, W) not in plan["nbr"]:
            plan["nbr"][(B, H, W)] = _ops.conv2d_neighbors(B, H, W, 3, 3, 1, 1, False, x.device)[0]
        nbr = plan["nbr"][(B, H, W)]
        n = B * H * W
        G = plan["groups"]
        _, s1 = _ops.conv_rows_split(split, 512, 0, plan["shared"], 64, 1, nbr, n, plan["s_bias"], plan["s_scale"],
                                     plan["s_shift"], relu=True, want_out=False, want_split=True)
        _, s2 = _ops.conv_rows_split(s1, 64, 0, plan["mid"], 64 * plan["mid_pair"], G // plan["mid_pair"], nbr, n,
                                     plan["mid_bias"], plan["mid_scale"], plan["mid_shift"], relu=True, want_out=False,
                                     want_split=True)
        if (plan["fin_w4"] is not None and os.environ.get("DF3D_HEAD_FINAL", "valu") == "valu"
                and _ops.CONV_PRECISION != "split3"):
            if "fin_pk" not in plan:
                plan["fin_pk"] = (_ops.head_final_pack(plan["fin_w4"])
                                  if os.environ.get("DF3D_HEADFINAL", "mfma")[:1] != "v" else None)
            out = _ops.head_final_conv(s2, B, H, W, plan["fin_w4"], plan["fin_b4"], plan["cols"], plan["width"],
                                       packed=plan["fin_pk"])
        else:
            out, _ = _ops.conv_rows_split(s2, 64, 64, plan["fin"], 32, G, nbr, n, plan["fin_bias"], None, None, relu=False,
                                          out_channels=plan["width"], out_cols=plan["cols"])
        rets = [dict() for _ in self.tasks]
        for t, head, c0, k in plan["layout"]:
            r = out[:, c0:c0 + k]
            v = r.view(B, H, W, k).permute(0, 3, 1, 2)
            v._df3d_rows = (r, None, v._version)
            rets[t][head] = v
        return rets

    _SITE_CODES = (("reg", 2), ("height", 1), ("dim", 3), ("vel", 2), ("rot", 2))

    def _sites_plan(self, plan):
        if "sites" in plan:
            return plan["sites"]
        plan["sites"] = None
        names = [n for n, _ in self._SITE_CODES]
        vel = all("vel" in task.heads for task in self.tasks)
        want = {n: k for n, k in self._SITE_CODES if vel or n != "vel"}
        for task in self.tasks:
            if set(task.heads) != set(want) | {"hm"} or any(getattr(task, n)[3].out_channels != k for n, k in want.items()) \
                    or any(getattr(task, n)[0].bias is None or getattr(task, n)[3].bias is None for n in task.heads):
                return None
        dev = self.shared_conv[0].weight.device
        pad4 = lambda fc: torch.cat([fc[3].bias.detach().float(), torch.zeros(4 - fc[3].out_channels, device=dev)])
        hms = [task.hm for task in self.tasks]
        pair = 2 if len(hms) % 2 == 0 else 1
        f1 = [self._filters(fc[0]) for fc in hms]
        folds = [self._fold(fc[1]) for fc in hms]
        cols, c0 = [], 0
        for fc in hms:
            cols.append((c0, fc[3].out_channels))
            c0 += fc[3].out_channels
        w4 = torch.stack([self._filters(fc[3], 4) for fc in hms]).contiguous()
        sites = dict(hm_mid=torch.cat([_ops.conv_pack_weights(torch.cat(f1[i:i + pair], dim=2).contiguous())
                                       for i in range(0, len(f1), pair)]), hm_pair=pair,
                     hm_bias=torch.cat([fc[0].bias.detach().float() for fc in hms]).contiguous(),
                     hm_scale=torch.cat([a for a, _ in folds]).contiguous(), hm_shift=torch.cat([b for _, b in folds]).contiguous(),
                     hm_w4=w4, hm_b4=torch.stack([pad4(fc) for fc in hms]).contiguous(),
                     hm_pk=_ops.head_final_pack(w4) if os.environ.get("DF3D_HEADFINAL", "mfma")[:1] != "v" else None,
                     hm_cols=cols, hm_cols_dev=torch.tensor(cols, dtype=torch.int32, device=dev).contiguous(),
                     hm_width=(c0 + 7) // 8 * 8, vel=vel, ncodes=10 if vel else 8)
        banks, rcols = [], []
        for task in self.tasks:
            c = 0
            for n in names:
                if n in want:
                    banks.append(getattr(task, n))
                    rcols.append((c, want[n]))
                    c += want[n]
        rfolds = [self._fold(fc[1]) for fc in banks]
        sites.update(w1=_ops.head_regress_pack(torch.stack([self._filters(fc[0]) for fc in banks]).contiguous()),
                     bias1=torch.stack([fc[0].bias.detach().float() for fc in banks]).contiguous(),
                     scale1=torch.stack([a for a, _ in rfolds]).contiguous(), shift1=torch.stack([b for _, b in rfolds]).contiguous(),
                     w2=torch.stack([self._filters(fc[3], 4) for fc in banks]).contiguous(),
                     b2=torch.stack([pad4(fc) for fc in banks]).contiguous(),
                     cols=torch.tensor(rcols, dtype=torch.int32, device=dev).contiguous())
        plan["sites"] = sites
        return sites

    def loss_sites_wanted(self, example):
        if os.environ.get("DF3D_HEAD_LOSS_SITES", "1") == "0" or self.dataset not in ('waymo', 'nuscenes'):
            return False
        if not isinstance(example, dict):
            return False
        T = len(self.tasks)
        for k in ("hm", "ind", "mask", "cat", "anno_box"):
            v = example.get(k)
            if not isinstance(v, (list, tuple)) or len(v) < T or not all(torch.is_tensor(a) and a.is_cuda for a in v[:T]):
                return False
        return True

    def loss_sites_fit(self, x):
        if (self.training or torch.is_grad_enabled() or not x.is_cuda or x.dtype != torch.float32 or not self._row_kernels_fit(x)
                or _ops.CONV_PRECISION in ("fp32", "split3") or os.environ.get("DF3D_HEAD_FINAL", "valu") != "valu"):
            return False
        plan = self._plan()
        if plan["fin_w4"] is None:
            return False
        sites = self._sites_plan(plan)
        return sites is not None and len(self.code_weights) == sites["ncodes"]

    @torch.no_grad()
    def forward_loss_dense(self, x):
        from .necks import _rows_of
        self.__dict__.pop("_packed_train", None)
        plan = self._plan()
        sites = self._sites_plan(plan)
        B, _, H, W = x.shape
        rows, split = _rows_of(x)
        if (split is None or split.dtype != torch.uint8 or split.shape[1] != _ops.split_width(rows.shape[1])):
            split = _ops.split_rows(rows.contiguous())
        if (B, H, W) not in plan["nbr"]:
            plan["nbr"][(B, H, W)] = _ops.conv2d_neighbors(B, H, W, 3, 3, 1, 1, False, x.device)[0]
        nbr = plan["nbr"][(B, H, W)]
        n = B * H * W
        T = len(self.tasks)
        _, s1 = _ops.conv_rows_split(split, 512, 0, plan["shared"], 64, 1, nbr, n, plan["s_bias"], plan["s_scale"],
                                     plan["s_shift"], relu=True, want_out=False, want_split=True)
        _, s2 = _ops.conv_rows_split(s1, 64, 0, sites["hm_mid"], 64 * sites["hm_pair"], T // sites["hm_pair"], nbr, n,
                                     sites["hm_bias"], sites["hm_scale"], sites["hm_shift"], relu=True, want_out=False,
                                     want_split=True)
        out = _ops.head_final_conv(s2, B, H, W, sites["hm_w4"], sites["hm_b4"], sites["hm_cols_dev"], sites["hm_width"],
                                   packed=sites["hm_pk"])
        return out, s1, (B, H, W)

    @torch.no_grad()
    def loss_sites(self, example, dense):
        out_hm, s1, (B, H, W) = dense
        sites = self._sites_plan(self._plan())
        T = len(self.tasks)
        pred = _ops.head_regress_at(s1, B, H, W, [example['ind'][t] for t in range(T)], [example['mask'][t] for t in range(T)],
                                    sites["w1"], sites["bias1"], sites["scale1"], sites["shift1"], sites["w2"], sites["b2"],
                                    sites["cols"])
        ncodes = sites["ncodes"]
        tasks = []
        for t, (c0, k) in enumerate(sites["hm_cols"]):
            p = pred[t]
            d = dict(hm=out_hm[:, c0:c0 + k], reg=p[:, 0:2], height=p[:, 2:3], dim=p[:, 3:6], rot=p[:, ncodes - 2:ncodes])
            if sites["vel"]:
                d['vel'] = p[:, 6:8]
            tasks.append(d)
        targets = [dict(hm=example['hm'][t], ind=example['ind'][t], mask=example['mask'][t], cat=example['cat'][t],
                        anno_box=example['anno_box'][t]) for t in range(T)]
        out = _ops.centerhead_loss(tasks, targets, B, H, W, self.code_weights, self.weight, reg_by_slot=True)
        return {'loss': out[:, 0], 'hm_loss': out[:, 1], 'loc_loss': out[:, 2], 'num_positive': out[:, 3],
                'loc_loss_elem': out[:, 4:4 + ncodes]}

    def _final_pack(self, branches, dev):
        key = (tuple(fc[3].out_channels for _, _, fc in branches), str(dev))
        hit = self.__dict__.get("_final_pack_cache")
        if hit is not None and hit["key"] == key:
            return hit
        widx, bidx, cols, layout = [], [], [], []
        wbase = bbase = c0 = 0
        for _, _, fc in branches:
            k = fc[3].out_channels
            assert k <= 4 and fc[3].in_channels == 64 and fc[3].kernel_size == (3, 3)
            j, c, tap = torch.meshgrid(torch.arange(4), torch.arange(64), torch.arange(9), indexing="ij")
            idx = wbase + (j * 64 + c) * 9 + tap
            idx = torch.where(j < k, idx, torch.full_like(idx, -1))
            widx.append(idx.permute(2, 1, 0))
            bidx.append(torch.tensor([bbase + jj if jj < k else -1 for jj in range(4)]))
            cols.append((c0, k))
            layout.append((c0, k))
            wbase += k * 64 * 9
            bbase += k
            c0 += k
        widx = torch.stack(widx)
        bidx = torch.stack(bidx)
        widx[widx < 0] = wbase
        bidx[bidx < 0] = bbase
        def inverse(idx, n):
            inv = torch.zeros(n + 1, dtype=torch.long)
            flat = idx.reshape(-1)
            inv[flat] = torch.arange(flat.numel())
            return inv
        hit = dict(key=key, widx=widx.to(dev), bidx=bidx.to(dev), layout=layout, width=(c0 + 7) // 8 * 8,
                   winv=inverse(widx, wbase).to(dev), binv=inverse(bidx, bbase).to(dev),
                   cols=torch.tensor(cols, dtype=torch.int32, device=dev).contiguous())
        self.__dict__["_final_pack_cache"] = hit
        return hit

    def forward_rows_train(self, x):
        from .necks import _bn_rows, _rows_of, _train_stack
        F = torch.nn.functional
        tables = self.__dict__.setdefault("_train_tables", {})
        B, _, H, W = x.shape
        rows, _ = _rows_of(x)
        sc, sbn = self.shared_conv[0], self.shared_conv[1]
        s, _, _ = _train_stack([(sc, sbn, True, 1)], rows, B, H, W, tables)
        nbr = tables[(B, H, W, 3, 3, 1, 1, False)][0]
        mkey = (B, H, W, "mirror")
        if mkey not in tables:
            tables[mkey] = nbr.flip(0).contiguous()
        branches = [(t, head, getattr(task, head)) for t, task in enumerate(self.tasks) for head in task.heads]
        G = len(branches)
        w = torch.cat([fc[0].weight.reshape(-1) for _, _, fc in branches]).view(G, 64, 64, 3, 3)
        w = w.permute(0, 3, 4, 2, 1).reshape(G, 9, 64, 64)
        b = torch.cat([fc[0].bias for _, _, fc in branches])
        m = _BranchConvFunction.apply(s, w, b, nbr, tables[mkey])
        bns = [fc[1] for _, _, fc in branches]
        mean = torch.cat([bn.running_mean for bn in bns])
        var = torch.cat([bn.running_var for bn in bns])
        if bns[0].training and _ops.bn_rows_supported(G * 64):
            m = _ops.BatchNormRowsFunction.apply(m, torch.cat([bn.weight for bn in bns]), torch.cat([bn.bias for bn in bns]),
                                                 mean, var, bns[0].momentum, bns[0].eps, True)
        else:
            m = torch.relu(F.batch_norm(m, mean, var, torch.cat([bn.weight for bn in bns]),
                                        torch.cat([bn.bias for bn in bns]), bns[0].training, bns[0].momentum, bns[0].eps))
        if bns[0].training:
            with torch.no_grad():
                torch._foreach_copy_([bn.running_mean for bn in bns], list(mean.split(64)))
                torch._foreach_copy_([bn.running_var for bn in bns], list(var.split(64)))
                torch._foreach_add_([bn.num_batches_tracked for bn in bns], 1)
        pack = self._final_pack(branches, m.device)
        flat_w = torch.cat([fc[3].weight.reshape(-1) for _, _, fc in branches] + [m.new_zeros(1)])
        flat_b = torch.cat([fc[3].bias for _, _, fc in branches] + [m.new_zeros(1)])
        w4 = _PermuteGather.apply(flat_w, pack["widx"].reshape(-1), pack["winv"]).view(G, 9, 64, 4)
        b4 = _PermuteGather.apply(flat_b, pack["bidx"].reshape(-1), pack["binv"]).view(G, 4)
        out = _HeadFinalFunction.apply(m, w4, b4, pack["cols"], pack["width"], B, H, W)
        rets = [dict() for _ in self.tasks]
        maps = out.view(B, H, W, -1)
        cols = [dict() for _ in self.tasks]
        for (t, head, fc), (c0, k) in zip(branches, pack["layout"]):
            cols[t][head] = (c0, k)
        self.__dict__["_packed_train"] = (out, cols, (B, H, W))
        for (t, head, fc), (c0, k) in zip(branches, pack["layout"]):
            v = maps[..., c0:c0 + k].permute(0, 3, 1, 2)
            rets[t][head] = v.clone() if head == 'hm' else v
        return rets

    def loss_rows(self, example):
        stash = self.__dict__.pop("_packed_train", None)
        if stash is None or self.dataset not in ('waymo', 'nuscenes'):
            return None
        out, cols, (B, H, W) = stash
        need = ("hm", "ind", "mask", "cat", "anno_box")
        if any(k not in example for k in need) or not all(torch.is_tensor(v) and v.is_cuda for k in need for v in example[k]):
            return None
        targets = [dict(hm=example["hm"][t].float(), ind=example["ind"][t].long(), mask=example["mask"][t],
                        cat=example["cat"][t].long(), anno_box=example["anno_box"][t].float()) for t in range(len(self.tasks))]
        vals = _ops.CenterHeadLossFunction.apply(out, cols, targets, B, H, W, list(self.code_weights), float(self.weight))
        n = len(self.code_weights)
        det = vals.detach()
        return {"loss": [vals[t, 0] for t in range(len(cols))], "hm_loss": [det[t, 1] for t in range(len(cols))],
                "loc_loss": [det[t, 2] for t in range(len(cols))], "loc_loss_elem": [det[t, 4:4 + n] for t in range(len(cols))],
                "num_positive": [det[t, 3] for t in range(len(cols))]}

    def loss(self, example, preds_dicts, batch_dict=None, host_copies=True, **kwargs):
        from collections import defaultdict
        self.__dict__.pop("_packed_train", None)
        rets = []
        for task_id, preds_dict in enumerate(preds_dicts):
            preds_dict['hm'] = _clamped_sigmoid(preds_dict['hm'])
            hm_loss = fast_focal_loss(preds_dict['hm'], example['hm'][task_id], example['ind'][task_id],
                                      example['mask'][task_id], example['cat'][task_id])
            target_box = example['anno_box'][task_id]
            if self.dataset not in ('waymo', 'nuscenes'):
                raise NotImplementedError()
            if 'vel' in preds_dict:
                preds_dict['anno_box'] = torch.cat((preds_dict['reg'], preds_dict['height'], preds_dict['dim'],
                                                    preds_dict['vel'], preds_dict['rot']), dim=1)
            else:
                preds_dict['anno_box'] = torch.cat((preds_dict['reg'], preds_dict['height'], preds_dict['dim'],
                                                    preds_dict['rot']), dim=1)
                target_box = target_box[..., [0, 1, 2, 3, 4, 5, -2, -1]]
            box_loss = reg_loss(preds_dict['anno_box'], example['mask'][task_id], example['ind'][task_id], target_box)
            loc_loss = (box_loss * box_loss.new_tensor(self.code_weights)).sum()
            loss = hm_loss + self.weight * loc_loss
            ret = {}
            if batch_dict is not None and "auxseg_loss" in batch_dict:
                auxseg_loss = sum(a[task_id] for a in batch_dict['auxseg_loss'])
                ret['auxseg_loss'] = auxseg_loss
                loss = loss + auxseg_loss
# ... 90 lines not shown
```

3d-dual-fusion_amd/dualfusion/necks.py:

```python
import os
import numpy as np
import torch
from torch import nn

from . import ops as _ops
from .registry import MM_BACKBONES, MM_NECKS, NECKS


def _bn(norm_cfg, planes):
    cfg = dict(norm_cfg or dict(type="BN", eps=1e-3, momentum=0.01))
    t = cfg.pop("type", "BN")
    if t not in ("BN", "BN2d"):
        raise KeyError("unsupported norm type for the BEV neck: %s" % t)
    cfg.pop("requires_grad", None)
    return nn.BatchNorm2d(planes, **cfg)


def _bn_rows(bn, x, relu=False):
    return _ops.batch_norm_rows(bn, x, relu)


def _train_stack(groups, rows, B, H, W, tables):
    from .spconv.conv import SparseConvFunction
    for conv, bn, relu, pad in groups:
# ... 35 lines not shown

class _Layer(object):

    def __init__(self, conv, bn, relu):
        self.conv, self.bn, self.relu = conv, bn, relu
        self.transposed = isinstance(conv, nn.ConvTranspose2d)
        self._key = None

    def prepare(self, pad):
        c = self.conv
        key = (c.weight.data_ptr(), c.weight._version, self.bn.running_var._version, self.bn.weight._version,
               _ops.CONV_PRECISION)
        if key == self._key:
            return
        w = c.weight.detach().float()
        if self.transposed:
            self.filters = w.permute(2, 3, 0, 1).reshape(-1, w.shape[0], w.shape[1]).contiguous()
        else:
            self.filters = w.permute(2, 3, 1, 0).reshape(-1, w.shape[1], w.shape[0]).contiguous()
        self.weights = _ops.ConvFilters(self.filters)
        inv = torch.rsqrt(self.bn.running_var.float() + self.bn.eps)
        self.scale = (self.bn.weight.float() * inv).contiguous()
        self.shift = (self.bn.bias.float() - self.bn.running_mean.float() * self.scale).contiguous()
        self.bias = c.bias.detach().float().contiguous() if c.bias is not None else None
        self.kh, self.kw = int(c.kernel_size[0]), int(c.kernel_size[1])
        self.stride = int(c.stride[0])
        self.pad = pad
        self._key = key


@NECKS.register_module
class RPN(nn.Module):
    def __init__(self, layer_nums, ds_layer_strides, ds_num_filters, us_layer_strides, us_num_filters,
                 num_input_features, norm_cfg=None, name="rpn", logger=None, **kwargs):
        super(RPN, self).__init__()
        self._layer_strides = list(ds_layer_strides)
        self._num_filters = list(ds_num_filters)
        self._layer_nums = list(layer_nums)
        self._upsample_strides = list(us_layer_strides)
        self._num_upsample_filters = list(us_num_filters)
        self._num_input_features = num_input_features
        self._norm_cfg = norm_cfg if norm_cfg is not None else dict(type="BN", eps=1e-3, momentum=0.01)
        assert len(self._layer_strides) == len(self._layer_nums) == len(self._num_filters)
        assert len(self._num_upsample_filters) == len(self._upsample_strides)
        self._upsample_start_idx = len(self._layer_nums) - len(self._upsample_strides)
        ratios = [self._upsample_strides[i] / np.prod(self._layer_strides[:i + self._upsample_start_idx + 1])
                  for i in range(len(self._upsample_strides))]
        assert all(r == ratios[0] for r in ratios)
        in_filters = [self._num_input_features] + self._num_filters[:-1]
        blocks, deblocks = [], []
        for i, layer_num in enumerate(self._layer_nums):
            planes = self._num_filters[i]
            mods = [nn.ZeroPad2d(1), nn.Conv2d(in_filters[i], planes, 3, stride=self._layer_strides[i], bias=False),
                    _bn(self._norm_cfg, planes), nn.ReLU()]
            for _ in range(layer_num):
                mods += [nn.Conv2d(planes, planes, 3, padding=1, bias=False), _bn(self._norm_cfg, planes), nn.ReLU()]
            blocks.append(nn.Sequential(*mods))
            j = i - self._upsample_start_idx
            if j >= 0:
                stride = self._upsample_strides[j]
                up = self._num_upsample_filters[j]
                if stride > 1:
                    conv = nn.ConvTranspose2d(planes, up, int(stride), stride=int(stride), bias=False)
                else:
                    st = int(np.round(1 / stride))
                    conv = nn.Conv2d(planes, up, st, stride=st, bias=False)
                deblocks.append(nn.Sequential(conv, _bn(self._norm_cfg, up), nn.ReLU()))
        self.blocks = nn.ModuleList(blocks)
        self.deblocks = nn.ModuleList(deblocks)

    @property
    def downsample_factor(self):
        factor = np.prod(self._layer_strides)
        if len(self._upsample_strides) > 0:
            factor /= self._upsample_strides[-1]
        return factor

    def init_weights(self):
        for m in self.modules():
            if isinstance(m, nn.Conv2d):
                nn.init.xavier_uniform_(m.weight)

    def forward_reference(self, x):
        ups = []
        for i in range(len(self.blocks)):
            x = self.blocks[i](x)
            if i - self._upsample_start_idx >= 0:
                ups.append(self.deblocks[i - self._upsample_start_idx](x))
        return torch.cat(ups, dim=1) if ups else x

    @staticmethod
    def _groups(seq):
        mods = list(seq)
        out, pad, i = [], 0, 0
        while i < len(mods):
            m = mods[i]
            if isinstance(m, nn.ZeroPad2d):
                pad = int(m.padding[0])
                i += 1
                continue
            assert isinstance(m, (nn.Conv2d, nn.ConvTranspose2d)) and isinstance(mods[i + 1], nn.BatchNorm2d)
            relu = i + 2 < len(mods) and isinstance(mods[i + 2], nn.ReLU)
            out.append((m, mods[i + 1], relu, pad + int(m.padding[0])))
            pad = 0
            i += 3 if relu else 2
        return out

    def _plan(self):
        plan = self.__dict__.get("_row_plan")
        if plan is None:
            plan = {"blocks": [[(_Layer(c, b, r), p) for c, b, r, p in self._groups(blk)] for blk in self.blocks],
                    "deblocks": [[(_Layer(c, b, r), p) for c, b, r, p in self._groups(d)] for d in self.deblocks],
                    "nbr": {}}
            self.__dict__["_row_plan"] = plan
        return plan

    def train(self, mode=True):
        self.__dict__.pop("_row_plan", None)
        return super(RPN, self).train(mode)

    @staticmethod
    def _table(layer, pad, B, H, W, tables, device):
        layer.prepare(pad)
        key = (B, H, W, layer.kh, layer.kw, layer.stride, layer.pad, layer.transposed)
        if key not in tables:
            tables[key] = _ops.conv2d_neighbors(B, H, W, layer.kh, layer.kw, layer.stride, layer.pad, layer.transposed,
                                                device)
        return tables[key]

    def accepts_split_rows(self):
        if _ops.CONV_PRECISION != "split" or self.training or os.environ.get("DF3D_FUSION_TAIL", "1") != "1":
            return False
        plan = self._plan()
        if not plan["blocks"] or not plan["blocks"][0]:
            return False
        layer, pad = plan["blocks"][0][0]
        layer.prepare(pad)
        return layer.weights.kind == "split"

    @staticmethod
    def _cat_width(plan):
        if plan.get("cat", (None, 0))[0] != _ops.CONV_PRECISION:
            lasts = [stack[-1] for stack in plan["deblocks"] if stack]
            for layer, pad in lasts:
                layer.prepare(pad)
            ok = (len(lasts) > 1 and len(lasts) == len(plan["deblocks"]) and os.environ.get("DF3D_NECK_CAT", "1") != "0"
                  and all(l.weights.kind in ("split", "split3") and l.filters.shape[2] % 8 == 0 for l, _ in lasts))
            plan["cat"] = (_ops.CONV_PRECISION, sum(l.filters.shape[2] for l, _ in lasts) if ok else 0)
        return plan["cat"][1]

    @staticmethod
    def _run(layer, pad, rows, split, B, H, W, tables):
        nbr, Ho, Wo = RPN._table(layer, pad, B, H, W, tables, rows.device)
        out, orows = _ops.conv(layer.weights, nbr, nbr.shape[1], rows=rows, operand=split, bias=layer.bias, scale=layer.scale,
                               shift=layer.shift, relu=layer.relu)
        return out, orows, Ho, Wo

    @torch.no_grad()
    def forward_rows(self, rows, B, H, W):
        plan = self._plan()
        tables = plan["nbr"]
        if isinstance(rows, SplitRows):
            x, xs = _NoRows(rows.split.device), rows.split
        else:
            x, xs = rows.contiguous(), None
        ups = []
        cat, cat_rows, cat_split, col0 = self._cat_width(plan), None, None, 0
        for i, blk in enumerate(plan["blocks"]):
            for layer, pad in blk:
                x, xs, H, W = self._run(layer, pad, x, xs, B, H, W, tables)
            j = i - self._upsample_start_idx
            if j >= 0:
                u, us, uh, uw = x, xs, H, W
                stack = plan["deblocks"][j]
                for layer, pad in stack[:-1] if cat else stack:
                    u, us, uh, uw = self._run(layer, pad, u, us, B, uh, uw, tables)
                if cat:
                    layer, pad = stack[-1]
                    nbr, uh, uw = self._table(layer, pad, B, uh, uw, tables, x.device)
                    if cat_rows is None:
                        cat_rows = torch.empty((nbr.shape[1], cat), dtype=torch.float32, device=x.device)
                        cat_split = torch.empty((nbr.shape[1], _ops.split_width(cat)), dtype=torch.uint8, device=x.device)
                    K, cin, cout = layer.filters.shape
                    _ops.conv_rows_split(us if us is not None else _ops.split_rows(u), cin, 0, layer.weights.packed, cout, 1, nbr,
                                         nbr.shape[1], layer.bias, layer.scale, layer.shift, layer.relu,
                                         into=(cat_rows, cat_split, col0))
                    col0 += cout
                    u = None
                ups.append((u, uh, uw))
        if not ups:
            return x.view(B, H, W, -1).permute(0, 3, 1, 2)
        uh, uw = ups[0][1], ups[0][2]
        assert all(h == uh and w == uw for _, h, w in ups)
        if cat:
            return _as_nchw(cat_rows, cat_split, B, uh, uw)
        out = torch.cat([u for u, _, _ in ups], 1) if len(ups) > 1 else ups[0][0]
        return out.view(B, uh, uw, -1).permute(0, 3, 1, 2)

    def forward_rows_train(self, rows, B, H, W):
        tables = self.__dict__.setdefault("_train_tables", {})
        ups = []
        for i, blk in enumerate(self.blocks):
            rows, H, W = _train_stack(self._groups(blk), rows, B, H, W, tables)
            j = i - self._upsample_start_idx
            if j >= 0:
                ups.append(_train_stack(self._groups(self.deblocks[j]), rows, B, H, W, tables))
        if not ups:
            return rows.view(B, H, W, -1).permute(0, 3, 1, 2).contiguous()
        uh, uw = ups[0][1], ups[0][2]
        assert all(h == uh and w == uw for _, h, w in ups)
        out = torch.cat([u for u, _, _ in ups], 1) if len(ups) > 1 else ups[0][0]
        return out.view(B, uh, uw, -1).permute(0, 3, 1, 2).contiguous()

    def forward(self, x):
        if not x.is_cuda or x.dtype != torch.float32:
            return self.forward_reference(x)
        B, C, H, W = x.shape
        rows = x.permute(0, 2, 3, 1).reshape(B * H * W, C)
        if self.training or torch.is_grad_enabled():
            return self.forward_rows_train(rows, B, H, W)
        return self.forward_rows(rows, B, H, W)


def _norm2d(norm_cfg, planes):
    cfg = dict(norm_cfg or dict(type="BN", eps=1e-3, momentum=0.01))
    t = cfg.pop("type", "BN")
    if t not in ("BN", "BN2d"):
        raise KeyError("unsupported norm type for the BEV neck: %s" % t)
    cfg.pop("requires_grad", None)
    return nn.BatchNorm2d(planes, **cfg)


def _conv2d(conv_cfg, cin, cout, k, **kw):
    cfg = dict(conv_cfg or dict(type="Conv2d", bias=False))
    t = cfg.pop("type", "Conv2d")
    if t not in ("Conv2d", "Conv"):
        raise KeyError("unsupported conv type for the BEV neck: %s" % t)
    kw.update(cfg)
    return nn.Conv2d(cin, cout, k, **kw)


def _rows_of(x):
    cached = getattr(x, "_df3d_rows", None)
    if cached is not None and cached[2] == x._version:
        return cached[0], cached[1]
    B, C, H, W = x.shape
    return x.permute(0, 2, 3, 1).reshape(B * H * W, C), None


def _as_nchw(rows, split, B, H, W):
    out = rows.view(B, H, W, -1).permute(0, 3, 1, 2)
    out._df3d_rows = (rows, split, out._version)
    return out


class _RowStacks(nn.Module):

    def _stacks(self, name, seqs):
        plan = self.__dict__.get("_row_plan")
        if plan is None:
            plan = self.__dict__["_row_plan"] = {"nbr": {}}
        if name not in plan:
            plan[name] = [[(_Layer(c, b, r), p) for c, b, r, p in RPN._groups(s)] for s in seqs]
        return plan[name], plan["nbr"]

    def train(self, mode=True):
        self.__dict__.pop("_row_plan", None)
        return super(_RowStacks, self).train(mode)

    @staticmethod
    def _fast(x):
        return x.is_cuda and x.dtype == torch.float32 and not torch.is_grad_enabled()


@MM_BACKBONES.register_module()
class SECOND(_RowStacks):
    def __init__(self, in_channels=128, out_channels=[128, 128, 256], layer_nums=[3, 5, 5], layer_strides=[2, 2, 2],
                 norm_cfg=dict(type="BN", eps=1e-3, momentum=0.01), conv_cfg=dict(type="Conv2d", bias=False)):
        super(SECOND, self).__init__()
        assert len(layer_strides) == len(layer_nums) == len(out_channels)
        in_filters = [in_channels] + list(out_channels[:-1])
        blocks = []
        for i, layer_num in enumerate(layer_nums):
            mods = [_conv2d(conv_cfg, in_filters[i], out_channels[i], 3, stride=layer_strides[i], padding=1),
                    _norm2d(norm_cfg, out_channels[i]), nn.ReLU(inplace=True)]
            for _ in range(layer_num):
                mods += [_conv2d(conv_cfg, out_channels[i], out_channels[i], 3, padding=1),
                         _norm2d(norm_cfg, out_channels[i]), nn.ReLU(inplace=True)]
            blocks.append(nn.Sequential(*mods))
        self.blocks = nn.ModuleList(blocks)

    def init_weights(self, pretrained=None):
        if isinstance(pretrained, str):
            self.load_state_dict(torch.load(pretrained, map_location="cpu").get("state_dict", {}), strict=False)

    def forward_reference(self, x):
        outs = []
        for blk in self.blocks:
            x = blk(x)
            outs.append(x)
        return tuple(outs)

    def forward(self, x):
        if (self.training or torch.is_grad_enabled()) and _train_rows_ok(x):
            tables = self.__dict__.setdefault("_train_tables", {})
            B, _, H, W = x.shape
            rows, _ = _rows_of(x)
            outs = []
# ... 83 lines not shown
```

3d-dual-fusion_amd/dualfusion/ops.py:

```python
import collections
import ctypes
import os

import torch

from . import _lib


_raw_stream = getattr(torch._C, "_cuda_getCurrentRawStream", None)


def _stream():
    if _raw_stream is not None:
        return _lib.StreamArg(_raw_stream(torch.cuda.current_device()))
    return _lib.StreamArg(torch.cuda.current_stream().cuda_stream)


def _ptr(t):
    if t is None:
        return ctypes.c_void_p(0)
    rec = _lib._recorder
    if rec is not None:
        rec._tape.keep.append(t)
    return ctypes.c_void_p(t.data_ptr())
# ... 385 lines not shown


class grad_precision(_Arithmetic):

    def _inside(self, mode, all_fp32):
        return ("split3" if mode == "split" else mode), all_fp32


_Format = collections.namedtuple("_Format", "parts dtype packed_bytes pack pack_groups rows conv conv_rows")
FORMATS = {
    "bf16": _Format(1, torch.bfloat16, "df3d_conv_packed_weight_bytes_bf16", "df3d_conv_pack_weights_bf16", None,
                    "df3d_rows_to_bf16", "df3d_sparse_conv_bf16", None),
    "split": _Format(2, torch.uint8, "df3d_conv_packed_weight_bytes", "df3d_conv_pack_weights", "df3d_conv_pack_weights_groups",
                     "df3d_split_rows", "df3d_sparse_conv_split", "df3d_conv_rows_split"),
    "split3": _Format(3, torch.uint8, "df3d_conv_packed_weight_bytes3", "df3d_conv_pack_weights3", "df3d_conv_pack_weights3",
                      "df3d_split_rows3", "df3d_conv_rows_split3", "df3d_conv_rows_split3"),
}
_PACK_TAKES_GROUPS = ("df3d_conv_pack_weights_groups", "df3d_conv_pack_weights3")


def split_kind():
    return "split3" if CONV_PRECISION == "split3" else "split"


def operand_width(kind, channels):
    fmt = FORMATS[kind]
    return 2 * fmt.parts * int(channels) // fmt.dtype.itemsize


def split_parts():
    return FORMATS[split_kind()].parts


def split_width(channels):
    return operand_width(split_kind(), channels)


def conv_kind(kvol, cin, cout):
    fmt = FORMATS.get(CONV_PRECISION)
    if fmt is not None and getattr(_lib.load(), fmt.packed_bytes)(int(kvol), int(cin), int(cout)) > 0:
        return CONV_PRECISION
    return "fp32"


def conv_split_supported(kvol, cin, cout):
    return CONV_PRECISION in ("split", "split3") and conv_kind(kvol, cin, cout) != "fp32"


def conv_bf16_supported(kvol, cin, cout):
    return _lib.load().df3d_conv_packed_weight_bytes_bf16(int(kvol), int(cin), int(cout)) > 0


def grad_scaled():
    return os.environ.get("DF3D_GRAD_SCALED", "1") != "0"


ConvGradPlan = collections.namedtuple("ConvGradPlan", "mode scaled blocks wgrad_bf16 fixed_scale")


def conv_grad_plan(kvol, cin, cout, amp, grouped=False):
    kvol, cin, cout, amp = int(kvol), int(cin), int(cout), bool(amp)
    mode = CONV_PRECISION

    def serves(m, c_in, c_out):
        return m in FORMATS and getattr(_lib.load(), FORMATS[m].packed_bytes)(kvol, c_in, c_out) > 0

    if grouped:
        if mode == "split" and grad_scaled():
            return ConvGradPlan("split", True, False, False, False)
        if mode in ("split", "split3"):
            return ConvGradPlan("split3", False, False, False, False)
        return ConvGradPlan("split", False, False, False, True)
    in_blocks = cin > 128 and cin % 128 == 0
    if mode == "split" and not amp and cout % 8 == 0 and grad_scaled():
        whole = serves("split", cout, cin)
        if whole or (in_blocks and serves("split", cout, 128)):
            return ConvGradPlan("split", True, not whole, False, False)
    if amp and serves("bf16", cout, cin):
        return ConvGradPlan("bf16", False, False, True, False)
    if mode == "bf16":
        return ConvGradPlan("fp32", False, False, amp, False)
    mode = "split3" if mode == "split" else mode
    return ConvGradPlan(mode, False, in_blocks and not serves(mode, cout, cin) and serves(mode, cout, 128), amp, False)


def _pack_filters(kind, filters, grouped=False):
    lib = _lib.load()
    fmt = FORMATS[kind]
    _chk(filters, torch.float32, "filters")
    G = filters.shape[0] if grouped else 1
    K, cin, cout = filters.shape[-3:]
    entry = fmt.pack_groups if grouped else fmt.pack
    nbytes = getattr(lib, fmt.packed_bytes)(K, cin, cout)
    if entry is None or nbytes == 0 or (grouped and cout > 128):
        raise _lib.Df3dError("no %s%s kernel for K=%d cin=%d cout=%d" % ("grouped " if grouped else "", kind, K, cin, cout))
    packed = torch.empty((G * nbytes,), dtype=torch.uint8, device=filters.device)
    args = (_ptr(filters),) + ((G,) if entry in _PACK_TAKES_GROUPS else ()) + (K, cin, cout, _ptr(packed), _stream())
    _lib.check(getattr(lib, entry)(*args), entry)
    return packed


def conv_pack_weights(filters):
    return _pack_filters(split_kind(), filters)


def conv_pack_weights_groups(filters):
    return _pack_filters(split_kind(), filters, grouped=True)


def conv_pack_weights_bf16(filters):
    return _pack_filters("bf16", filters)


def operand_rows(kind, features):
    lib = _lib.load()
    fmt = FORMATS[kind]
    _chk(features, torch.float32, "features")
    n, c = features.shape
    out = torch.empty((n, operand_width(kind, c)), dtype=fmt.dtype, device=features.device)
    _lib.check(getattr(lib, fmt.rows)(_ptr(features), n, c, _ptr(out), _stream()), fmt.rows)
    return out


def split_rows(features):
    return operand_rows(split_kind(), features)


def rows_to_bf16(features):
    return operand_rows("bf16", features)


def rows_from_bf16(rows):
    lib = _lib.load()
    _chk(rows, torch.bfloat16, "rows")
    n, c = rows.shape
    out = torch.empty((n, c), dtype=torch.float32, device=rows.device)
    _lib.check(lib.df3d_rows_from_bf16(_ptr(rows), n, c, _ptr(out), _stream()), "df3d_rows_from_bf16")
    return out


def split_rows_scaled(features, inv_channels):
    lib = _lib.load()
    _chk(features, torch.float32, "features")
    n, c = features.shape
    out = torch.empty((n, 4 * c), dtype=torch.uint8, device=features.device)
    scale = torch.empty((int(lib.df3d_pow2_scale_floats()),), dtype=torch.float32, device=features.device)
    inv = torch.empty((int(inv_channels),), dtype=torch.float32, device=features.device)
    rc = lib.df3d_split_rows_scaled(_ptr(features), n, c, _ptr(out), _ptr(scale), _ptr(inv), int(inv_channels), _stream())
    _lib.check(rc, "df3d_split_rows_scaled")
    return out, inv, scale


def _conv_operands(kind, rows, packed, nbr, n_out, cin, cout, bias, scale, shift, residual, relu, want_f32, want_rows,
                   order=None):
    lib = _lib.load()
    fmt = FORMATS[kind]
    _chk(rows, fmt.dtype, "operand rows")
    _chk(packed, torch.uint8, "packed")
    _chk(nbr, torch.int32, "nbr")
    K = nbr.shape[0]
    if rows.shape[1] != operand_width(kind, cin) or packed.numel() != K * cin * cout * 2 * fmt.parts:
        raise _lib.Df3dError("%s operands do not match K=%d cin=%d cout=%d" % (kind, K, cin, cout))
    for t, nm in ((bias, "bias"), (scale, "scale"), (shift, "shift")):
        if t is not None:
            _chk(t, torch.float32, nm)
    if residual is not None:
        _chk(residual, torch.bfloat16 if kind == "bf16" else torch.float32, "residual")
    dev = nbr.device
    out = torch.empty((n_out, cout), dtype=torch.float32, device=dev) if want_f32 else None
    orows = torch.empty((n_out, operand_width(kind, cout)), dtype=fmt.dtype, device=dev) if want_rows else None
    head = (_ptr(rows), rows.shape[0], cin)
    epilogue = (_ptr(bias), _ptr(scale), _ptr(shift), _ptr(residual), int(bool(relu)))
    if kind == "bf16":
        rc = lib.df3d_sparse_conv_bf16(*head, _ptr(packed), K, cout, _ptr(nbr), int(n_out), *epilogue, _ptr(out), _ptr(orows),
                                       _stream())
    elif kind == "split":
        rc = lib.df3d_sparse_conv_split(*head, _ptr(packed), K, cout, _ptr(nbr), int(n_out), *epilogue, _ptr(out), _ptr(orows),
                                        _ptr(order), -1 if order is not None else 0, _stream())
    else:
        rc = lib.df3d_conv_rows_split3(*head, cin, 0, _ptr(packed), K, cout, 1, _ptr(nbr), int(n_out), *epilogue, _ptr(out), cout,
                                       None, _ptr(orows), _stream())
    _lib.check(rc, fmt.conv)
    return out, orows


def sparse_conv_split(features_split, packed, nbr, n_out, cin, cout, bias=None, scale=None, shift=None,
                      residual=None, relu=False, emit_split=True, order=None):
    return _conv_operands(split_kind(), features_split, packed, nbr, n_out, cin, cout, bias, scale, shift, residual, relu,
                          True, emit_split, order)


def sparse_conv_bf16(rows, packed, nbr, n_out, cin, cout, bias=None, scale=None, shift=None, residual=None, relu=False,
                     want_f32=False, want_bf16=True):
    return _conv_operands("bf16", rows, packed, nbr, n_out, cin, cout, bias, scale, shift, residual, relu, want_f32, want_bf16)


class ConvFilters(object):
    __slots__ = ("filters", "kind", "packed")

    def __init__(self, filters, kind=None):
        K, cin, cout = filters.shape
        self.filters = filters
        self.kind = conv_kind(K, cin, cout) if kind is None else kind
        self.packed = _pack_filters(self.kind, filters) if self.kind != "fp32" else None


def conv_filters(owner, weight, kvol, cin, cout):
    kind = conv_kind(kvol, cin, cout)
    key = (weight.data_ptr(), weight._version, str(weight.device), kind)
    cache = owner.__dict__.setdefault("_conv_filters", {})
    hit = cache.get(kind)
    if hit is None or hit[0] != key:
        hit = cache[kind] = (key, ConvFilters(weight.detach().contiguous().float().view(kvol, cin, cout), kind))
    return hit[1]


def is_operand(kind, rows, channels):
    fmt = FORMATS.get(kind)
    return (fmt is not None and isinstance(rows, torch.Tensor) and rows.dtype == fmt.dtype and rows.dim() == 2
            and rows.shape[1] == operand_width(kind, channels))


def conv(filters, nbr, n_out, rows=None, operand=None, bias=None, scale=None, shift=None, residual=None, relu=False,
         want_f32=True, want_operand=True, tiles=None, order=None):
    kind = filters.kind
    K, cin, cout = filters.filters.shape
    if kind == "fp32":
        return sparse_conv_fused(rows, filters.filters, nbr, n_out, bias=bias, scale=scale, shift=shift, residual=residual,
                                 relu=relu, tiles=tiles), None
    if kind != CONV_PRECISION:
        raise _lib.Df3dError("conv: filters packed for %r cannot run in the %r mode; pack them again (conv_filters does)"
                             % (kind, CONV_PRECISION))
    if not is_operand(kind, operand, cin):
        operand = operand_rows(kind, rows)
    if kind == "bf16":
        if residual is not None and residual.dtype != torch.bfloat16:
            residual = rows_to_bf16(residual.contiguous().float())
        return _conv_operands(kind, operand, filters.packed, nbr, n_out, cin, cout, bias, scale, shift, residual, relu,
                              want_f32, want_operand)
    return _conv_operands(kind, operand, filters.packed, nbr, n_out, cin, cout, bias, scale, shift, residual, relu, True,
                          want_operand, order)


def invert_neighbors(nbr, n_in):
    lib = _lib.load()
    _chk(nbr, torch.int32, "nbr")
    K, n_out = nbr.shape
    inv = torch.empty((K, int(n_in)), dtype=torch.int32, device=nbr.device)
    rc = lib.df3d_invert_neighbors(_ptr(nbr), K, n_out, int(n_in), _ptr(inv), _stream())
    _lib.check(rc, "df3d_invert_neighbors")
    return inv


def rows_pow2_scale(x):
    lib = _lib.load()
    _chk(x, torch.float32, "x")
    scale = torch.empty((int(lib.df3d_pow2_scale_floats()),), dtype=torch.float32, device=x.device)
    _lib.check(lib.df3d_rows_pow2_scale(_ptr(x), int(x.numel()), _ptr(scale), _stream()), "df3d_rows_pow2_scale")
    return scale


def sparse_conv_grad_filters(features, grad_out, nbr, grad_scale=None, bf16=False):
    lib = _lib.load()
    _chk(features, torch.float32, "features")
    _chk(grad_out, torch.float32, "grad_out")
    _chk(nbr, torch.int32, "nbr")
    K, n_out = nbr.shape
    if grad_out.shape[0] != n_out:
        raise ValueError("grad_out rows do not match the neighbour table")
    cin, cout = features.shape[1], grad_out.shape[1]
    gw = torch.empty((K, cin, cout), dtype=torch.float32, device=features.device)
    entry, scale = "df3d_sparse_conv_grad_filters", ()
    if bf16 and os.environ.get("DF3D_WGRAD_BF16", "1") != "0":
        entry += "_bf16"
    elif grad_scale is not None and grad_scaled():
        _chk(grad_scale, torch.float32, "grad_scale")
        entry, scale = entry + "_scaled", (_ptr(grad_scale),)
    rc = getattr(lib, entry)(_ptr(features), features.shape[0], cin, _ptr(grad_out), n_out, cout, _ptr(nbr), K, *scale, _ptr(gw),
                             _stream())
    _lib.check(rc, entry)
    return gw


def rows_grad_weights(x, grad_out, x_scale=None, g_scale=None, two_part=False):
    lib = _lib.load()
    _chk(x, torch.float32, "x")
    _chk(grad_out, torch.float32, "grad_out")
    n, cin = x.shape
    if grad_out.shape[0] != n:
        raise _lib.Df3dError("rows_grad_weights: %d rows against %d" % (n, grad_out.shape[0]))
    cout = grad_out.shape[1]
    gw = torch.empty((cin, cout), dtype=torch.float32, device=x.device)
    entry, scales = "df3d_rows_grad_weights", ()
    if (two_part or x_scale is not None or g_scale is not None) and grad_scaled():
        entry, scales = entry + "_scaled", (_ptr(x_scale), _ptr(g_scale))
    _lib.check(getattr(lib, entry)(_ptr(x), _ptr(grad_out), int(n), int(cin), int(cout), *scales, _ptr(gw), _stream()), entry)
    return gw


def _column_blocks(wt):
    K, cout, cin = wt.shape
    return wt.view(K, cout, cin // 128, 128).permute(2, 0, 1, 3).contiguous()


def sparse_conv_backward(features, filters, grad_out, nbr, subm, inv=None, bf16=False):
    K = nbr.shape[0]
    n_in = features.shape[0]
    grad_out = grad_out.contiguous()
    if inv is None:
        if subm:
            inv = getattr(nbr, "_df3d_mirror", None)
            if inv is None or inv[1] != nbr._version:
                inv = nbr._df3d_mirror = (nbr.flip(0).contiguous(), nbr._version)
            inv = inv[0]
        else:
            inv = invert_neighbors(nbr, n_in)
    wt = filters.transpose(1, 2).contiguous()
    cout, cin = wt.shape[1], wt.shape[2]
    plan = conv_grad_plan(K, cin, cout, bf16)
    rows = inv_s = g_scale = None
    with precision(plan.mode):
        if plan.scaled:
            rows, inv_s, g_scale = split_rows_scaled(grad_out, cin)
        if plan.blocks:
            g_in, _ = conv_rows_split(rows if plan.scaled else split_rows(grad_out), cout, 0,
                                      conv_pack_weights_groups(_column_blocks(wt)), 128, cin // 128, inv, n_in, scale=inv_s)
        else:
            g_in, _ = conv(ConvFilters(wt), inv, n_in, rows=grad_out, operand=rows, scale=inv_s, want_operand=False)
    return g_in, sparse_conv_grad_filters(features.contiguous(), grad_out, nbr, grad_scale=g_scale, bf16=plan.wgrad_bf16)


def conv_rows_split(in_split, cin, in_group_stride, packed, cout, groups, nbr, n_out, bias=None, scale=None, shift=None,
                    relu=False, out_channels=None, out_cols=None, want_out=True, want_split=False, into=None):
    lib = _lib.load()
    _chk(in_split, torch.uint8, "in_split")
    _chk(packed, torch.uint8, "packed")
    _chk(nbr, torch.int32, "nbr")
    fmt = FORMATS[split_kind()]
    pb = 2 * fmt.parts
    n_in, in_channels = in_split.shape[0], in_split.shape[1] // pb
    K = nbr.shape[0]
    if packed.numel() != groups * K * cin * cout * pb or in_split.shape[1] != pb * in_channels:
        raise _lib.Df3dError("packed filters do not match groups=%d K=%d cin=%d cout=%d (%d parts)" % (groups, K, cin, cout, pb // 2))
    for t, nm in ((bias, "bias"), (scale, "scale"), (shift, "shift")):
        if t is not None:
            _chk(t, torch.float32, nm)
    dev = in_split.device

    def launch(po, oc, pcols, ps):
        residual = (None,) if fmt.parts == 3 else ()
        rc = getattr(lib, fmt.conv_rows)(_ptr(in_split), n_in, in_channels, int(cin), int(in_group_stride), _ptr(packed), K,
                                         int(cout), int(groups), _ptr(nbr), int(n_out), _ptr(bias), _ptr(scale), _ptr(shift),
                                         *residual, int(bool(relu)), po, oc, pcols, ps, _stream())
        _lib.check(rc, fmt.conv_rows)

    if into is not None:
        out, osp, col0 = into
        col0 = int(col0)
        if out_cols is not None or (out is None and osp is None) or col0 % 8:
            raise _lib.Df3dError("conv_rows_split: `into` takes rows and a column offset that is a multiple of 8")
        oc = out.shape[1] if out is not None else osp.shape[1] // pb
        for t, dt, w, nm in ((out, torch.float32, oc, "into rows"), (osp, torch.uint8, pb * oc, "into split rows")):
            if t is not None:
                _chk(t, dt, nm)
                if tuple(t.shape) != (n_out, w):
                    raise _lib.Df3dError("conv_rows_split: %s must be [%d, %d]" % (nm, n_out, w))
        if col0 + groups * cout > oc:
            raise _lib.Df3dError("conv_rows_split: columns [%d, %d) outside %d-channel rows" % (col0, col0 + groups * cout, oc))
        po = ctypes.c_void_p(out.data_ptr() + 4 * col0) if out is not None else None
        ps = ctypes.c_void_p(osp.data_ptr() + pb * col0) if osp is not None else None
        launch(po, oc, None, ps)
        return out, osp
    oc = int(out_channels if out_channels is not None else groups * cout)
    out = torch.empty((n_out, oc), dtype=torch.float32, device=dev) if want_out else None
    osp = torch.empty((n_out, pb * oc), dtype=torch.uint8, device=dev) if want_split else None
    launch(_ptr(out), oc, _ptr(out_cols), _ptr(osp))
    return out, osp


def head_final_pack(weights):
    lib = _lib.load()
    _chk(weights, torch.float32, "weights")
    G = weights.shape[0]
    if tuple(weights.shape[1:]) != (9, 64, 4):
        raise _lib.Df3dError("head_final_pack: weights [G,9,64,4] expected")
    packed = torch.empty(int(lib.df3d_head_final_packed_bytes(G)), dtype=torch.uint8, device=weights.device)
    _lib.check(lib.df3d_head_final_pack(_ptr(weights), G, _ptr(packed), _stream()), "df3d_head_final_pack")
    return packed


def head_final_conv(in_split, batch, H, W, weights, bias, out_cols, out_channels, packed=None):
    lib = _lib.load()
    _chk(in_split, torch.uint8, "in_split")
    _chk(weights, torch.float32, "weights")
    _chk(bias, torch.float32, "bias")
    _chk(out_cols, torch.int32, "out_cols")
    G = weights.shape[0]
    if tuple(weights.shape[1:]) != (9, 64, 4) or tuple(bias.shape) != (G, 4) or tuple(out_cols.shape) != (G, 2):
        raise _lib.Df3dError("head_final_conv: weights [G,9,64,4], bias [G,4], out_cols [G,2] expected")
    n = int(batch) * int(H) * int(W)
    if in_split.shape[0] != n:
        raise _lib.Df3dError("head_final_conv: %d rows for a %dx%dx%d map" % (in_split.shape[0], batch, H, W))
    out = torch.empty((n, int(out_channels)), dtype=torch.float32, device=in_split.device)
    if packed is not None:
        _chk(packed, torch.uint8, "packed")
        if packed.numel() != lib.df3d_head_final_packed_bytes(G):
            raise _lib.Df3dError("head_final_conv: packed filters do not match %d branches" % G)
        rc = lib.df3d_head_final_conv_packed(_ptr(in_split), in_split.shape[1] // 4, int(batch), int(H), int(W), G,
                                             _ptr(packed), _ptr(bias), _ptr(out_cols), _ptr(out), int(out_channels),
                                             _stream())
        _lib.check(rc, "df3d_head_final_conv_packed")
        return out
    rc = lib.df3d_head_final_conv(_ptr(in_split), in_split.shape[1] // 4, int(batch), int(H), int(W), G, _ptr(weights),
                                  _ptr(bias), _ptr(out_cols), _ptr(out), int(out_channels), _stream())
    _lib.check(rc, "df3d_head_final_conv")
    return out


def head_regress_pack(filters):
    lib = _lib.load()
    _chk(filters, torch.float32, "filters")
    if filters.dim() != 4 or tuple(filters.shape[1:]) != (9, 64, 64):
        raise _lib.Df3dError("head_regress_pack: filters [banks,9,64,64] expected")
    banks = filters.shape[0]
    packed = torch.empty(int(lib.df3d_head_regress_packed_bytes(banks)), dtype=torch.uint8, device=filters.device)
    _lib.check(lib.df3d_head_regress_pack(_ptr(filters), banks, _ptr(packed), _stream()), "df3d_head_regress_pack")
    return packed


def _ind_mask(ind, mask, batch):
    if mask.dtype == torch.bool:
        mask = mask.view(torch.uint8)
    if ind.dtype != torch.int64 or mask.dtype != torch.uint8 or ind.dim() != 2 or ind.shape[0] != batch or mask.shape != ind.shape:
        raise ValueError("targets ind (int64) / mask (uint8 or bool) must be [%d, max_objs]" % batch)
    if not (ind.is_cuda and mask.is_cuda):
        raise _lib.Df3dError("head_regress_at: targets must live on the GPU (no CPU fallback)")
    return ind.contiguous(), mask.contiguous()


def head_regress_at(s1_split, batch, H, W, inds, masks, packed, bias1, scale1, shift1, w2, b2, cols):
    lib = _lib.load()
    T = len(inds)
    banks = w2.shape[0]
    _chk(s1_split, torch.uint8, "s1_split")
    _chk(packed, torch.uint8, "packed")
    _chk(cols, torch.int32, "cols")
    for t_, nm in ((bias1, "bias1"), (scale1, "scale1"), (shift1, "shift1"), (w2, "w2"), (b2, "b2")):
        _chk(t_, torch.float32, nm)
    n = int(batch) * int(H) * int(W)
    if tuple(s1_split.shape) != (n, 256):
        raise _lib.Df3dError("head_regress_at: split rows [%d, 256] expected for a %dx%dx%d map of 64 channels" % (n, batch, H, W))
    if T < 1 or banks % T or packed.numel() != lib.df3d_head_regress_packed_bytes(banks) or tuple(w2.shape[1:]) != (9, 64, 4) \
            or tuple(b2.shape) != (banks, 4) or tuple(cols.shape) != (banks, 2) \
            or any(tuple(v.shape) != (banks, 64) for v in (bias1, scale1, shift1)):
        raise _lib.Df3dError("head_regress_at: operands do not describe %d banks over %d tasks" % (banks, T))
    tg = (_HeadTargets * T)()
    keep = []
    M = int(inds[0].shape[1])
    for i in range(T):
        ind, mask = _ind_mask(inds[i], masks[i], batch)
        if ind.shape[1] != M:
            raise ValueError("head_regress_at: tasks disagree about max_objs")
        keep.append((ind, mask))
        tg[i].ind, tg[i].mask = ind.data_ptr(), mask.data_ptr()
    pred = torch.empty((T, int(batch) * M, LOSS_MAX_CODES), dtype=torch.float32, device=s1_split.device)
    rc = lib.df3d_head_regress_at(_ptr(s1_split), int(batch), int(H), int(W), ctypes.byref(tg), T, M, banks // T, _ptr(packed),
                                  _ptr(bias1), _ptr(scale1), _ptr(shift1), _ptr(w2), _ptr(b2), _ptr(cols), _ptr(pred), _stream())
    _lib.check(rc, "df3d_head_regress_at")
    return pred


def sparse_to_dense(features, indices, batch, shape):
    lib = _lib.load()
    _chk(features, torch.float32, "features")
    _chk(indices, torch.int32, "indices")
    n, C = features.shape
    out = torch.empty([int(batch), C] + [int(s) for s in shape], dtype=torch.float32, device=features.device)
    shp_p, keep = _lib.int3(shape)
    rc = lib.df3d_sparse_to_dense(_ptr(features), _ptr(indices), n, C, int(batch), shp_p, _ptr(out), _stream())
    _lib.check(rc, "df3d_sparse_to_dense")
    return out


def sparse_to_dense_rows(features, indices, batch, shape):
    lib = _lib.load()
    _chk(features, torch.float32, "features")
    _chk(indices, torch.int32, "indices")
    n, C = features.shape
    D, H, W = [int(v) for v in shape]
    out = torch.empty((int(batch) * H * W, C * D), dtype=torch.float32, device=features.device)
    shp_p, keep = _lib.int3(shape)
    rc = lib.df3d_sparse_to_dense_rows(_ptr(features), _ptr(indices), n, C, int(batch), shp_p, _ptr(out), _stream())
    _lib.check(rc, "df3d_sparse_to_dense_rows")
    return out


def sparse_to_dense_rows_split(features, indices, batch, shape):
    lib = _lib.load()
    _chk(features, torch.float32, "features")
    _chk(indices, torch.int32, "indices")
    n, C = features.shape
    D, H, W = [int(v) for v in shape]
# ... 1884 lines not shown
```

include/df3d_hip.h:

```cpp
#ifndef DF3D_HIP_H_
#define DF3D_HIP_H_

#include <stddef.h>
#include <stdint.h>

#ifdef __cplusplus
extern "C" {
#endif

#define DF3D_OK 0
#define DF3D_EINVAL (-1)
#define DF3D_ENOMEM (-2)
#define DF3D_EHIP (-3)

#define DF3D_MAX_KVOL 32

int df3d_version(void);
const char *df3d_last_error(void);
int df3d_device_count(void);
int df3d_device_arch(char *buf, int buflen);
int df3d_split_overflow(int reset, char *where, int where_len);
int df3d_split_overflow_collect(uint32_t *out, int reset, void *stream);
int df3d_split_overflow_units(char *buf, int buflen);

size_t df3d_hard_voxelize_workspace_bytes(int num_points, int max_points, int max_voxels);
int df3d_hard_voxelize(const float *points, int num_points, int num_features,
                       const float *voxel_size_host, const float *coors_range_host,
                       int max_points, int max_voxels, int break_at_cap,
                       float *voxels, int32_t *coors, int32_t *num_points_per_voxel,
                       float *mean, int32_t *voxel_num,
                       void *workspace, size_t workspace_bytes, void *stream);
int df3d_hard_voxelize_batched(const float *points, int num_points, int num_features,
                               const float *voxel_size_host, const float *coors_range_host,
                               int max_points, int max_voxels, int break_at_cap, int batch_index,
                               float *voxels, int32_t *coors4, int32_t *num_points_per_voxel,
                               float *mean, int32_t *voxel_num,
                               void *workspace, size_t workspace_bytes, void *stream);

size_t df3d_grid_bytes(int batch, const int *shape_host);
int df3d_grid_build(const int32_t *indices, int n, int batch, const int *shape_host,
                    void *grid, size_t grid_bytes, int32_t *perm, void *stream);
int df3d_subm_neighbors(const void *grid, const int32_t *perm, const int32_t *indices, int n,
                        int batch, const int *shape_host, const int *ksize_host,
                        const int *dilation_host, int32_t *nbr, void *stream);
int df3d_conv_out_indices(const int32_t *indices, int n, int batch, const int *in_shape_host,
                          const int *out_shape_host, const int *ksize_host, const int *stride_host,
                          const int *padding_host, const int *dilation_host,
                          void *out_grid, size_t out_grid_bytes,
                          int32_t *out_indices, int out_cap, int32_t *num_out, void *stream);
int df3d_conv_neighbors(const void *in_grid, const int32_t *in_perm, const int32_t *out_indices,
                        int n_out, int batch, const int *in_shape_host, const int *ksize_host,
                        const int *stride_host, const int *padding_host, const int *dilation_host,
                        int32_t *nbr, void *stream);
int df3d_conv_transpose_out_indices(const int32_t *indices, int n, int batch, const int *in_shape, const int *out_shape,
                                    const int *ksize, const int *stride, const int *padding, const int *dilation,
                                    void *out_grid, size_t out_grid_bytes, int32_t *out_indices, int out_cap,
                                    int32_t *num_out, void *stream);
int df3d_conv_transpose_neighbors(const void *in_grid, const int32_t *in_perm, const int32_t *out_indices, int n_out,
                                  int batch, const int *in_shape, const int *ksize, const int *stride,
                                  const int *padding, const int *dilation, int32_t *nbr, void *stream);
size_t df3d_nbr_to_pairs_workspace_bytes(int kvol, int n_out);
int df3d_nbr_to_pairs(const int32_t *nbr, int kvol, int n_out, int n_in,
                      int32_t *indice_pairs, int32_t *indice_num,
                      void *workspace, size_t workspace_bytes, void *stream);
int df3d_pairs_to_nbr(const int32_t *indice_pairs, const int32_t *indice_num_host, int kvol,
                      int n_in, int n_out, int32_t *nbr, void *stream);

int df3d_sparse_conv_fused(const float *features, int n_in, int cin,
                           const float *filters, int kvol, int cout,
                           const int32_t *nbr, int n_out,
                           const float *bias, const float *scale, const float *shift,
                           const float *residual, int relu, float *out, void *stream);

int df3d_conv_tile_count(int n_out, int cin, int cout, int kvol);
size_t df3d_conv_tiles_workspace_bytes(int n_out);
int df3d_conv_tiles(const int32_t *nbr, int kvol, int n_out, int ntiles, int32_t *tile_rows,
                    void *workspace, size_t workspace_bytes, void *stream);
int df3d_sparse_conv_fused_tiled(const float *features, int n_in, int cin,
                                 const float *filters, int kvol, int cout,
                                 const int32_t *nbr, int n_out,
                                 const float *bias, const float *scale, const float *shift,
                                 const float *residual, int relu, float *out,
                                 const int32_t *tile_rows, int ntiles, void *stream);

size_t df3d_nbr_row_lists_bytes(int kvol, int n_out);
int df3d_nbr_row_lists(const int32_t *nbr, int kvol, int n_out, int n_in, void *lists, size_t lists_bytes, void *stream);
int df3d_sparse_conv_fused_lists(const float *features, int n_in, int cin, const float *filters, int kvol, int cout,
                                 const int32_t *nbr, const void *lists, int n_out, const float *bias, const float *scale,
                                 const float *shift, const float *residual, int relu, float *out, void *out_split,
                                 void *stream);

int df3d_timing_begin(void);
int df3d_timing_end(void);
int df3d_timing_get(int i, int *shape4_host, float *ms_host);
int df3d_timing_count_pairs(int on);
int df3d_timing_filter(int cin, int cout, int kvol);
int df3d_timing_sample(int every);
int df3d_timing_get2(int i, int *shape4, float *ms, long long *pairs, int *split);

int df3d_sparse_conv_grouped(const float *features, int n_in, int cin, int ld_in, int group_in, const float *filters, int kvol,
                             int cout, int groups, const int32_t *nbr, int n_out, const float *bias, const float *scale,
                             const float *shift, int relu, float *out, int ld_out, int group_out, void *stream);
int df3d_sparse_to_dense(const float *features, const int32_t *indices, int n, int channels,
                         int batch, const int *shape_host, float *out, void *stream);

int df3d_sparse_to_dense_rows(const float *features, const int32_t *indices, int n, int channels, int batch,
                              const int *shape_host, float *out_rows, void *stream);
int df3d_sparse_to_dense_rows_split(const float *features, const int32_t *indices, int n, int channels, int batch,
                                    const int *shape_host, void *out_split, void *stream);
int df3d_conv2d_neighbors(int batch, int H, int W, int kh, int kw, int stride, int pad, int transposed,
                          int32_t *nbr, void *stream);

int df3d_rows_to_bf16(const float *features, long long n, int c, void *rows_bf16, void *stream);
int df3d_rows_from_bf16(const void *rows_bf16, long long n, int c, float *features, void *stream);
size_t df3d_conv_packed_weight_bytes_bf16(int kvol, int cin, int cout);
int df3d_conv_pack_weights_bf16(const float *filters, int kvol, int cin, int cout, void *packed, void *stream);
int df3d_sparse_conv_bf16(const void *features_bf16, int n_in, int cin, const void *packed_filters, int kvol, int cout,
                          const int32_t *nbr, int n_out, const float *bias, const float *scale, const float *shift,
                          const void *residual_bf16, int relu, float *out, void *out_bf16, void *stream);

int df3d_invert_neighbors(const int32_t *nbr, int kvol, int n_out, int n_in, int32_t *inv, void *stream);
int df3d_sparse_conv_grad_filters(const float *features, int n_in, int cin, const float *grad_out, int n_out, int cout,
                                  const int32_t *nbr, int kvol, float *grad_filters, void *stream);
int df3d_rows_grad_weights(const float *x, const float *grad_out, long long n, int cin, int cout, float *grad_weights,
                           void *stream);
int df3d_sparse_conv_grad_filters_scaled(const float *features, int n_in, int cin, const float *grad_out, int n_out, int cout,
                                         const int32_t *nbr, int kvol, const float *grad_scale, float *grad_filters, void *stream);
int df3d_rows_grad_weights_scaled(const float *x, const float *grad_out, long long n, int cin, int cout, const float *x_scale,
                                  const float *g_scale, float *grad_weights, void *stream);
int df3d_sparse_conv_grad_filters_bf16(const float *features, int n_in, int cin, const float *grad_out, int n_out, int cout,
                                       const int32_t *nbr, int kvol, float *grad_filters, void *stream);
int df3d_grad_filters_kernel(int form, int kvol, int cin, int cout, int n_out);
int df3d_rows_pow2_scale(const float *x, long long n_elems, float *scale, void *stream);
int df3d_pow2_scale_floats(void);
int df3d_chanfirst_dot(const float *x, const float *g, int nmaps, int channels, long long S, float *out, void *stream);

int df3d_bn_rows_supported(int c);
int df3d_bn_rows_scratch_doubles(int c);
int df3d_bn_rows_forward(const float *x, long long n, int c, const float *weight, const float *bias, float eps,
                         float momentum, int relu, float *running_mean, float *running_var, double *sums, float *saved,
                         float *y, void *stream);
int df3d_bn_rows_backward(const float *x, const float *dy, long long n, int c, const float *saved, int relu, double *sums,
                          float *dx, float *dweight, float *dbias, void *stream);

int df3d_conv_rows_split(const void *in_split, int n_in, int in_channels, int cin, int in_group_stride,
                         const void *packed_filters, int kvol, int cout, int groups, const int32_t *nbr, int n_out,
                         const float *bias, const float *scale, const float *shift, int relu, float *out,
                         int out_channels, const int32_t *out_cols, void *out_split, void *stream);

size_t df3d_conv_packed_weight_bytes3(int kvol, int cin, int cout);
int df3d_conv_pack_weights3(const float *filters, int groups, int kvol, int cin, int cout, void *packed, void *stream);
int df3d_split_rows3(const float *features, long long n, int c, void *split3, void *stream);
int df3d_conv_rows_split3(const void *in_split3, int n_in, int in_channels, int cin, int in_group_stride, const void *packed3,
                          int kvol, int cout, int groups, const int32_t *nbr, int n_out, const float *bias, const float *scale,
                          const float *shift, const float *residual, int relu, float *out, int out_channels,
                          const int32_t *out_cols, void *out_split3, void *stream);

#define DF3D_NMS_NORMAL 0
#define DF3D_NMS_ROTATED 1
#define DF3D_NMS_CIRCLE 2
int df3d_boxes_bev_pairwise(const float *boxes_a, int na, const float *boxes_b, int nb, int mode, float *out,
                            void *stream);
size_t df3d_nms_bev_workspace_bytes(int lists, int cap);
int df3d_nms_bev(const float *boxes, const int32_t *counts, int lists, int cap, float thresh, int mode, int max_keep,
                 int32_t *keep, int32_t *num_keep, void *workspace, size_t workspace_bytes, void *stream);

#define DF3D_MAX_HEAD_TASKS 8
typedef struct df3d_head_task {
  const float *hm, *reg, *height, *dim, *rot, *vel;
  int ld_hm, ld_reg, ld_height, ld_dim, ld_rot, ld_vel;
  int num_classes, label_base;
} df3d_head_task;
typedef struct df3d_head_decode_cfg {
  int batch, H, W;
  float out_size_factor, voxel_size[2], pc_range[2];
  int has_post_center_range;
  float post_center_range[6];
  float score_threshold;
  int nms_mode;
  float nms_threshold;
  int pre_max, post_max;
} df3d_head_decode_cfg;
size_t df3d_centerhead_predict_workspace_bytes(int ntasks, const df3d_head_decode_cfg *cfg);
int df3d_centerhead_predict(const df3d_head_task *tasks, int ntasks, const df3d_head_decode_cfg *cfg, float *out_boxes,
                            float *out_scores, int32_t *out_labels, int32_t *out_counts, void *workspace,
                            size_t workspace_bytes, void *stream);

int df3d_head_final_conv(const void *in_split, int in_channels, int batch, int H, int W, int groups, const float *weights,
                         const float *bias, const int32_t *out_cols, float *out, int out_channels, void *stream);
size_t df3d_head_final_packed_bytes(int groups);
int df3d_head_final_pack(const float *weights, int groups, void *packed, void *stream);
int df3d_head_final_conv_packed(const void *in_split, int in_channels, int batch, int H, int W, int groups,
                                const void *packed, const float *bias, const int32_t *out_cols, float *out,
                                int out_channels, void *stream);
int df3d_head_final_conv_backward(const float *acts, int act_channels, const float *grad_out, int out_channels, int batch,
                                  int H, int W, int groups, const float *weights, const int32_t *out_cols,
                                  float *grad_acts, float *grad_weights, void *stream);

#define DF3D_LOSS_MAX_CODES 10
#define DF3D_LOSS_FIELDS (4 + DF3D_LOSS_MAX_CODES)
typedef struct df3d_head_targets {
  const float *hm;
  const long long *ind;
  const unsigned char *mask;
  const long long *cat;
  const float *box;
} df3d_head_targets;
size_t df3d_centerhead_loss_workspace_bytes(int ntasks, int batch, int H, int W);
int df3d_centerhead_loss(const df3d_head_task *tasks, const df3d_head_targets *targets, int ntasks, int batch, int H, int W,
                         int max_objs, int box_dim, const float *code_weights, int ncodes, float weight, float *out,
                         void *workspace, size_t workspace_bytes, void *stream);
int df3d_centerhead_loss_grad(const df3d_head_task *tasks, const df3d_head_task *grad_tasks, const df3d_head_targets *targets,
                              int ntasks, int batch, int H, int W, int max_objs, int box_dim, const float *code_weights,
                              int ncodes, float weight, float *out, void *workspace, size_t workspace_bytes, void *stream);
int df3d_centerhead_loss_slots(const df3d_head_task *tasks, const df3d_head_targets *targets, int ntasks, int batch, int H,
                               int W, int max_objs, int box_dim, const float *code_weights, int ncodes, float weight,
                               float *out, void *workspace, size_t workspace_bytes, void *stream);

size_t df3d_head_regress_packed_bytes(int banks);
int df3d_head_regress_pack(const float *w1, int banks, void *packed, void *stream);
int df3d_head_regress_at(const void *s1_split, int batch, int H, int W, const df3d_head_targets *targets, int ntasks,
                         int max_objs, int branches, const void *w1_packed, const float *bias1, const float *scale1,
                         const float *shift1, const float *w2, const float *b2, const int32_t *cols, float *pred,
                         void *stream);

typedef struct df3d_query_heads {
  const float *heatmap, *center, *height, *dim, *rot, *vel;
  int ld_heatmap, ld_center, ld_height, ld_dim, ld_rot, ld_vel;
} df3d_query_heads;
size_t df3d_heatmap_proposals_workspace_bytes(int batch, int num_classes, int H, int W);
int df3d_heatmap_proposals(const float *heat_rows, int ld_heat, int batch, int num_classes, int H, int W,
                           int nms_kernel_size, unsigned exempt_classes, int num_proposals, const float *feat_rows,
                           int ld_feat, int channels, const float *class_weight, const float *class_bias,
                           int32_t *top_class, int32_t *top_pixel, float *query_score, float *query_pos,
                           float *query_feat, void *workspace, size_t workspace_bytes, void *stream);
int df3d_transfusion_decode(const df3d_query_heads *heads, const float *query_score, const int32_t *query_label,
                            int batch, int num_proposals, int num_classes, const df3d_head_decode_cfg *cfg,
                            float *out_boxes, float *out_scores, int32_t *out_labels, int32_t *out_counts, void *stream);

int df3d_sparse_maxpool(const float *features, int n_in, int channels, const int32_t *nbr, int kvol, int n_out, float *out,
                        void *stream);
int df3d_sparse_maxpool_backward(const float *features, const float *out_features, const float *grad_out, int n_in,
                                 int channels, const int32_t *inv, int kvol, float *grad_in, void *stream);

int df3d_dynamic_voxelize(const float *points, long long num_points, int num_features, const float *voxel_size,
                          const float *coors_range, int32_t *coors, void *stream);

size_t df3d_topk_keys_workspace_bytes(int segments, long long n, int k);
int df3d_topk_keys(const unsigned long long *keys, int segments, long long n, int k, unsigned long long *out,
                   int32_t *out_count, void *workspace, size_t workspace_bytes, void *stream);

size_t df3d_cross_attention_workspace_bytes(int batch, int heads, int nq, int nk);
int df3d_cross_attention(const float *q, int ld_q, const float *k, int ld_k, const float *v, int ld_v, int batch, int nq,
                         int nk, int heads, int head_dim, float scale, float *out, int ld_out, void *workspace,
                         size_t workspace_bytes, void *stream);
int df3d_cross_attention_train(const float *q, int ld_q, const float *k, int ld_k, const float *v, int ld_v, int batch, int nq,
                               int nk, int heads, int head_dim, float scale, float p, unsigned long long seed, float *out,
                               int ld_out, float *lse, void *workspace, size_t workspace_bytes, void *stream);
int df3d_cross_attention_backward(const float *q, int ld_q, const float *k, int ld_k, const float *v, int ld_v,
                                  const float *grad_out, int ld_do, const float *lse, const float *delta, int batch, int nq,
                                  int nk, int heads, int head_dim, float scale, float p, unsigned long long seed, float *dq,
                                  int ld_dq, float *dk, int ld_dk, float *dv, int ld_dv, void *stream);

int df3d_ms_deform_attn_forward(const float *value, const int64_t *spatial_shapes,
                                const int64_t *level_start_index, const float *sampling_loc,
                                const float *attn_weight, int N, int S, int M, int D, int Lq,
                                int L, int P, float *out, void *stream);

int df3d_ms_deform_attn_backward(const float *value, const int64_t *spatial_shapes, const int64_t *level_start_index,
                                 const float *sampling_loc, const float *attn_weight, const float *grad_output, int N,
                                 int S, int M, int D, int Lq, int L, int P, float *grad_value,
                                 float *grad_sampling_loc, float *grad_attn_weight, void *stream);
size_t df3d_ms_deform_attn_backward_binned_workspace_bytes(int N, int M, int Lq, int P, int H, int W);
size_t df3d_ms_deform_attn_backward_binned_slab_bytes(int N, int M, int D, int Lq, int P, int H, int W);
int df3d_ms_deform_attn_backward_binned(const float *value, const int64_t *spatial_shapes, const int64_t *level_start_index,
                                        const float *sampling_loc, const float *attn_weight, const float *grad_output, int N,
                                        int M, int D, int Lq, int P, int H, int W, float *grad_value, float *grad_sampling_loc,
                                        float *grad_attn_weight, void *workspace, size_t workspace_bytes, float *slabs, void *stream);
int df3d_ms_deform_attn_backward_plan(int N, int S, int M, int D, int Lq, int L, int P, const int64_t *level_hw,
                                      const int64_t *level_start, int mode);
size_t df3d_ms_deform_attn_backward_binned_ml_workspace_bytes(int N, int M, int Lq, int L, int P, const int64_t *level_hw, int ordered);
size_t df3d_ms_deform_attn_backward_binned_ml_slab_bytes(int N, int M, int D, int Lq, int L, int P, const int64_t *level_hw);
int df3d_ms_deform_attn_backward_binned_ml(const float *value, const int64_t *spatial_shapes, const int64_t *level_start_index,
                                           const float *sampling_loc, const float *attn_weight, const float *grad_output,
                                           const int64_t *level_hw, const int64_t *level_start, int N, int M, int D, int Lq, int L,
                                           int P, int ordered, float *grad_value, float *grad_sampling_loc, float *grad_attn_weight,
                                           void *workspace, size_t workspace_bytes, float *slabs, void *stream);

int df3d_ms_deform_attn_forward_f64(const double *value, const int64_t *spatial_shapes, const int64_t *level_start_index,
                                    const double *sampling_loc, const double *attn_weight, int N, int S, int M, int D, int Lq,
                                    int L, int P, double *out, void *stream);
size_t df3d_ms_deform_attn_backward_f64_workspace_bytes(int N, int S, int M, int Lq, int L, int P);
int df3d_ms_deform_attn_backward_f64(const double *value, const int64_t *spatial_shapes, const int64_t *level_start_index,
                                     const double *sampling_loc, const double *attn_weight, const double *grad_output, int N,
                                     int S, int M, int D, int Lq, int L, int P, double *grad_value, double *grad_sampling_loc,
                                     double *grad_attn_weight, void *workspace, size_t workspace_bytes, void *stream);

int df3d_group_attention(const float *qkv, int tokens, int groups, int heads, int head_dim, float *out, void *stream);
int df3d_group_attention_split(const float *qkv, int tokens, int groups, int heads, int head_dim, float *out, void *out_split,
                               void *stream);
int df3d_group_attention_backward(const float *qkv, const float *grad_out, int tokens, int groups, int heads, int head_dim,
// ... 329 lines not shown
```

Before: 405.1.

## Add dense halo-tiled 3x3 conv kernel for BEV neck and head convolutions

```diff
diff --git a/3d-dual-fusion_amd/csrc/spconv_split.hip b/3d-dual-fusion_amd/csrc/spconv_split.hip
--- a/3d-dual-fusion_amd/csrc/spconv_split.hip
+++ b/3d-dual-fusion_amd/csrc/spconv_split.hip
@@ -234,6 +234,7 @@
   const int32_t *order;
   unsigned long long *trace;
   int cbw;
+  int dB, dH, dW;
 };
 
 #ifdef DF3D_OS_TRACE
@@ -309,6 +310,92 @@
 };
 
 __device__ u32x4 g_zero_row[192];
+
+template <int NP, int RT, int CT, class RowOf>
+__device__ __forceinline__ void os_epilogue_rows(const SplitConvArgs &a, const f32x4 (&acc)[RT][CT], int col0, int n, RowOf row_of) {
+  f32x4 bi[CT / 4], sc[CT / 4], sh[CT / 4];
+#pragma unroll
+  for (int q = 0; q < CT / 4; ++q) {
+    const int col = col0 + n * CT + q * 4;
+    bi[q] = a.bias ? *(const f32x4 *)(a.bias + col) : (f32x4){0.f, 0.f, 0.f, 0.f};
+    sc[q] = a.scale ? *(const f32x4 *)(a.scale + col) : (f32x4){1.f, 1.f, 1.f, 1.f};
+    sh[q] = a.shift ? *(const f32x4 *)(a.shift + col) : (f32x4){0.f, 0.f, 0.f, 0.f};
+  }
+#pragma unroll
+  for (int rt = 0; rt < RT; ++rt) {
+#pragma unroll
+    for (int r = 0; r < 4; ++r) {
+      const int row = row_of(rt, r);
+      if (row >= a.n_out) continue;
+      if (OS_DBG(32) && acc[rt][0][r] != 1234.567f) continue;
+      const size_t o = (size_t)row * a.ldo + col0 + n * CT;
+      unsigned h[CT / 2], l[CT / 2], m3[CT / 2];
+#pragma unroll
+      for (int q = 0; q < CT / 4; ++q) {
+        f32x4 v = (f32x4){acc[rt][q * 4][r], acc[rt][q * 4 + 1][r], acc[rt][q * 4 + 2][r], acc[rt][q * 4 + 3][r]};
+        v = (v * acc_unscale<NP>() + bi[q]) * sc[q] + sh[q];
+        if (a.residual) {
+          if constexpr (NP == 1) {
+            const u32x2 rr = *(const u32x2 *)((const char *)a.residual + (o + q * 4) * 2);
+            v += (f32x4){bf16lo_to_f32(rr[0]), bf16hi_to_f32(rr[0]), bf16lo_to_f32(rr[1]), bf16hi_to_f32(rr[1])};
+          } else {
+            v += *(const f32x4 *)(a.residual + o + q * 4);
+          }
+        }
+        if (a.relu) {
+          v[0] = fmaxf(v[0], 0.f);
+          v[1] = fmaxf(v[1], 0.f);
+          v[2] = fmaxf(v[2], 0.f);
+          v[3] = fmaxf(v[3], 0.f);
+        }
+        if (a.out) *(f32x4 *)(a.out + o + q * 4) = v;
+        if (a.out_split) {
+          if constexpr (NP == 3) {
+            split3_pair(v[0], v[1], h[q * 2], m3[q * 2], l[q * 2]);
+            split3_pair(v[2], v[3], h[q * 2 + 1], m3[q * 2 + 1], l[q * 2 + 1]);
+          } else if constexpr (NP == 1) {
+            h[q * 2] = bf16_pair(v[0], v[1]);
+            h[q * 2 + 1] = bf16_pair(v[2], v[3]);
+          } else {
+            split_pair(v[0], v[1], h[q * 2], l[q * 2]);
+            split_pair(v[2], v[3], h[q * 2 + 1], l[q * 2 + 1]);
+          }
+        }
+      }
+      if constexpr (NP == 3) {
+        if (a.out_split) {
+          char *blk = (char *)a.out_split + (o >> 3) * 48;
+          if constexpr (CT == 8) {
+            *(u32x4 *)blk = (u32x4){h[0], h[1], h[2], h[3]};
+            *(u32x4 *)(blk + 16) = (u32x4){m3[0], m3[1], m3[2], m3[3]};
+            *(u32x4 *)(blk + 32) = (u32x4){l[0], l[1], l[2], l[3]};
+          } else {
+            blk += (n & 1) * 8;
+            *(u32x2 *)blk = (u32x2){h[0], h[1]};
+            *(u32x2 *)(blk + 16) = (u32x2){m3[0], m3[1]};
+            *(u32x2 *)(blk + 32) = (u32x2){l[0], l[1]};
+          }
+        }
+        continue;
+      }
+      if (a.out_split && NP == 1) {
+        char *dst = (char *)a.out_split + o * 2;
+        if constexpr (CT == 8) *(u32x4 *)dst = (u32x4){h[0], h[1], h[2], h[3]};
+        else *(u32x2 *)dst = (u32x2){h[0], h[1]};
+      } else if (a.out_split) {
+        char *blk = (char *)a.out_split + (o >> 3) * 32;
+        if constexpr (CT == 8) {
+          *(u32x4 *)blk = (u32x4){h[0], h[1], h[2], h[3]};
+          *(u32x4 *)(blk + 16) = (u32x4){l[0], l[1], l[2], l[3]};
+        } else {
+          blk += (n & 1) * 8;
+          *(u32x2 *)blk = (u32x2){h[0], h[1]};
+          *(u32x2 *)(blk + 16) = (u32x2){l[0], l[1]};
+        }
+      }
+    }
+  }
+}
 
 template <int CIN, int COUT, int RT, int NW, int KPS, int NP = 2, int KS = 1, bool MG = false>
 __global__ __launch_bounds__(NW * KS * 64) void spconv_os_split_kernel(SplitConvArgs a) {
@@ -741,89 +828,8 @@
     OS_STAMP(4);
     return;
   } else {
-  f32x4 bi[CT / 4], sc[CT / 4], sh[CT / 4];
-#pragma unroll
-  for (int q = 0; q < CT / 4; ++q) {
-    const int col = col0 + n * CT + q * 4;
-    bi[q] = a.bias ? *(const f32x4 *)(a.bias + col) : (f32x4){0.f, 0.f, 0.f, 0.f};
-    sc[q] = a.scale ? *(const f32x4 *)(a.scale + col) : (f32x4){1.f, 1.f, 1.f, 1.f};
-    sh[q] = a.shift ? *(const f32x4 *)(a.shift + col) : (f32x4){0.f, 0.f, 0.f, 0.f};
-  }
-#pragma unroll
-  for (int rt = 0; rt < RT; ++rt) {
-#pragma unroll
-    for (int r = 0; r < 4; ++r) {
-      const int row = rowL[wave * WROWS + rt * 16 + 4 * g + r];
-      if (row >= a.n_out) continue;
-      if (OS_DBG(32) && acc[rt][0][r] != 1234.567f) continue;
-      const size_t o = (size_t)row * a.ldo + col0 + n * CT;
-      unsigned h[CT / 2], l[CT / 2], m3[CT / 2];
-#pragma unroll
-      for (int q = 0; q < CT / 4; ++q) {
-        f32x4 v = (f32x4){acc[rt][q * 4][r], acc[rt][q * 4 + 1][r], acc[rt][q * 4 + 2][r], acc[rt][q * 4 + 3][r]};
-        v = (v * acc_unscale<NP>() + bi[q]) * sc[q] + sh[q];
-        if (a.residual) {
-          if constexpr (NP == 1) {
-            const u32x2 rr = *(const u32x2 *)((const char *)a.residual + (o + q * 4) * 2);
-            v += (f32x4){bf16lo_to_f32(rr[0]), bf16hi_to_f32(rr[0]), bf16lo_to_f32(rr[1]), bf16hi_to_f32(rr[1])};
-          } else {
-            v += *(const f32x4 *)(a.residual + o + q * 4);
-          }
-        }
-        if (a.relu) {
-          v[0] = fmaxf(v[0], 0.f);
-          v[1] = fmaxf(v[1], 0.f);
-          v[2] = fmaxf(v[2], 0.f);
-          v[3] = fmaxf(v[3], 0.f);
-        }
-        if (a.out) *(f32x4 *)(a.out + o + q * 4) = v;
-        if (a.out_split) {
-          if constexpr (NP == 3) {
-            split3_pair(v[0], v[1], h[q * 2], m3[q * 2], l[q * 2]);
-            split3_pair(v[2], v[3], h[q * 2 + 1], m3[q * 2 + 1], l[q * 2 + 1]);
-          } else if constexpr (NP == 1) {
-            h[q * 2] = bf16_pair(v[0], v[1]);
-            h[q * 2 + 1] = bf16_pair(v[2], v[3]);
-          } else {
-            split_pair(v[0], v[1], h[q * 2], l[q * 2]);
-            split_pair(v[2], v[3], h[q * 2 + 1], l[q * 2 + 1]);
-          }
-        }
-      }
-      if constexpr (NP == 3) {
-        if (a.out_split) {
-          char *blk = (char *)a.out_split + (o >> 3) * 48;
-          if constexpr (CT == 8) {
-            *(u32x4 *)blk = (u32x4){h[0], h[1], h[2], h[3]};
-            *(u32x4 *)(blk + 16) = (u32x4){m3[0], m3[1], m3[2], m3[3]};
-            *(u32x4 *)(blk + 32) = (u32x4){l[0], l[1], l[2], l[3]};
-          } else {
-            blk += (n & 1) * 8;
-            *(u32x2 *)blk = (u32x2){h[0], h[1]};
-            *(u32x2 *)(blk + 16) = (u32x2){m3[0], m3[1]};
-            *(u32x2 *)(blk + 32) = (u32x2){l[0], l[1]};
-          }
-        }
-        continue;
-      }
-      if (a.out_split && NP == 1) {
-        char *dst = (char *)a.out_split + o * 2;
-        if constexpr (CT == 8) *(u32x4 *)dst = (u32x4){h[0], h[1], h[2], h[3]};
-        else *(u32x2 *)dst = (u32x2){h[0], h[1]};
-      } else if (a.out_split) {
-        char *blk = (char *)a.out_split + (o >> 3) * 32;
-        if constexpr (CT == 8) {
-          *(u32x4 *)blk = (u32x4){h[0], h[1], h[2], h[3]};
-          *(u32x4 *)(blk + 16) = (u32x4){l[0], l[1], l[2], l[3]};
-        } else {
-          blk += (n & 1) * 8;
-          *(u32x2 *)blk = (u32x2){h[0], h[1]};
-          *(u32x2 *)(blk + 16) = (u32x2){l[0], l[1]};
-        }
-      }
-    }
-  }
-  OS_STAMP(4);
+    os_epilogue_rows<NP, RT, CT>(a, acc, col0, n, [&](int rt, int r) { return rowL[wave * WROWS + rt * 16 + 4 * g + r]; });
+    OS_STAMP(4);
   }
 }
 
@@ -1268,6 +1274,177 @@
   return DF3D_OK;
 }
 
+template <int CIN, int CW, int RT>
+__global__ __launch_bounds__(256, 2) void conv2d_halo_kernel(SplitConvArgs a) {
+  constexpr int NP = 2, NW = 4, NT = NW * 64, KB = CIN / 32, CT = CW / 16, KV = 9;
+  constexpr int TY = NW * RT, TX = 16, PX = TX + 2, NPIX = (TY + 2) * PX;
+  constexpr int PQ = 9;
+  constexpr int WQ = CT * NP * 64, WPT = WQ / NT;
+  constexpr int PPT = (NPIX * 8 + NT - 1) / NT;
+  constexpr int NBATCH = CT / 2;
+  static_assert(WQ % NT == 0 && NBATCH % 2 == 0, "column block");
+  __shared__ u32x4 Wl[3][WQ];
+  __shared__ u32x4 Pl[NPIX * PQ];
+
+  const int tid = threadIdx.x, lane = tid & 63, wave = tid >> 6;
+  const int g = lane >> 4, n = lane & 15;
+  const int H = a.dH, W = a.dW;
+  const int txn = (W + TX - 1) / TX, tyn = (H + TY - 1) / TY;
+  const int tile = xcd_tile(blockIdx.x, gridDim.x);
+  const int img = tile / (txn * tyn), trem = tile - img * (txn * tyn);
+  const int y0 = (trem / txn) * TY, x0 = (trem % txn) * TX;
+  const int col0 = blockIdx.y * CW;
+  const u32x4 *wbase = a.w + (size_t)blockIdx.y * KV * KB * WQ + tid;
+
+  const u32x4 *psrc[PPT];
+#pragma unroll
+  for (int i = 0; i < PPT; ++i) {
+    const int e = tid + NT * i, pix = e >> 3, unit = e & 7;
+    const int py = pix / PX, px = pix - py * PX;
+    const int gy = y0 - 1 + py, gx = x0 - 1 + px;
+    const bool in = e < NPIX * 8 && gy >= 0 && gy < H && gx >= 0 && gx < W;
+    psrc[i] = in ? a.feat + ((size_t)img * H * W + (size_t)gy * W + gx) * a.ldi + (size_t)blockIdx.y * a.in_goff + unit
+                 : g_zero_row + unit;
+  }
+  u32x4 pr[PPT];
+  auto load_p = [&](int kb) {
+#pragma unroll
+    for (int i = 0; i < PPT; ++i) pr[i] = psrc[i][kb * 8];
+  };
+  auto store_p = [&]() {
+#pragma unroll
+    for (int i = 0; i < PPT; ++i) {
+      const int e = tid + NT * i;
+      if (e < NPIX * 8) Pl[(e >> 3) * PQ + (e & 7)] = pr[i];
+    }
+  };
+  u32x4 wr[3][WPT];
+  auto load_w = [&](u32x4 (&wreg)[WPT], int kb, int k) {
+    kb += k / KV, k %= KV;
+    if (kb >= KB) kb = KB - 1, k = KV - 1;
+    const u32x4 *src = wbase + (size_t)(k * KB + kb) * WQ;
+#pragma unroll
+    for (int i = 0; i < WPT; ++i) wreg[i] = src[NT * i];
+  };
+  auto store_w = [&](int buf, u32x4 (&wreg)[WPT]) {
+#pragma unroll
+    for (int i = 0; i < WPT; ++i) Wl[buf][tid + NT * i] = wreg[i];
+  };
+
+  f32x4 acc[RT][CT];
+#pragma unroll
+  for (int rt = 0; rt < RT; ++rt)
+#pragma unroll
+    for (int ct = 0; ct < CT; ++ct) acc[rt][ct] = (f32x4){0.f, 0.f, 0.f, 0.f};
+
+  u32x4 af[2][RT][NP];
+  const u32x4 *pa = Pl + ((wave * RT) * PX + n) * PQ + g * NP;
+  auto read_a = [&](int k, u32x4 (&dst)[RT][NP]) {
+    const int d = (k / 3) * PX + (k % 3);
+#pragma unroll
+    for (int rt = 0; rt < RT; ++rt)
+#pragma unroll
+      for (int q = 0; q < NP; ++q) dst[rt][q] = pa[(rt * PX + d) * PQ + q];
+  };
+
+  load_p(0);
+  load_w(wr[0], 0, 0);
+  load_w(wr[1], 0, 1);
+  store_p();
+  store_w(0, wr[0]);
+  store_w(1, wr[1]);
+  load_w(wr[1], 0, 2);
+  load_w(wr[2], 0, 3);
+  load_w(wr[0], 0, 4);
+  load_p(KB > 1 ? 1 : 0);
+  __syncthreads();
+  u32x4 bq[2][2 * NP];
+#pragma unroll
+  for (int q = 0; q < 2 * NP; ++q) bq[0][q] = Wl[0][lane + q * 64];
+  read_a(0, af[0]);
+
+  for (int kb = 0; kb < KB; ++kb) {
+#pragma unroll
+    for (int k = 0; k < KV; ++k) {
+      __syncthreads();
+      if (k == 0 && kb > 0) {
+        store_p();
+        __syncthreads();
+        load_p(kb + 1 < KB ? kb + 1 : KB - 1);
+        read_a(0, af[0]);
+      }
+      const u32x4 *wb = Wl[k % 3] + lane;
+      u32x4 (&cur)[RT][NP] = af[k & 1];
+#pragma unroll
+      for (int i = 0; i < NBATCH; ++i) {
+        const int c2 = i * 2;
+        if (i == 1) {
+          store_w((k + 2) % 3, wr[(k + 1) % 3]);
+          load_w(wr[(k + 1) % 3], kb, k + 5);
+        }
+        if (i + 1 < NBATCH) {
+#pragma unroll
+          for (int q = 0; q < 2 * NP; ++q) bq[(i + 1) & 1][q] = wb[((i + 1) * 2 * NP + q) * 64];
+        }
+        const u32x4 bh0 = bq[i & 1][0], bl0 = bq[i & 1][1], bh1 = bq[i & 1][2], bl1 = bq[i & 1][3];
+#pragma unroll
+        for (int rt = 0; rt < RT; ++rt) {
+          acc[rt][c2] = DF3D_MFMA_F16(cur[rt][1], bh0, acc[rt][c2]);
+          acc[rt][c2 + 1] = DF3D_MFMA_F16(cur[rt][1], bh1, acc[rt][c2 + 1]);
+        }
+#pragma unroll
+        for (int rt = 0; rt < RT; ++rt) {
+          acc[rt][c2] = DF3D_MFMA_F16(cur[rt][0], bl0, acc[rt][c2]);
+          acc[rt][c2 + 1] = DF3D_MFMA_F16(cur[rt][0], bl1, acc[rt][c2 + 1]);
+        }
+#pragma unroll
+        for (int rt = 0; rt < RT; ++rt) {
+          acc[rt][c2] = DF3D_MFMA_F16(cur[rt][0], bh0, acc[rt][c2]);
+          acc[rt][c2 + 1] = DF3D_MFMA_F16(cur[rt][0], bh1, acc[rt][c2 + 1]);
+        }
+      }
+      const u32x4 *wn = Wl[(k + 1) % 3] + lane;
+#pragma unroll
+      for (int q = 0; q < 2 * NP; ++q) bq[0][q] = wn[q * 64];
+      if (k + 1 < KV) read_a(k + 1, af[(k + 1) & 1]);
+    }
+  }
+
+  os_epilogue_rows<NP, RT, CT>(a, acc, col0, n, [&](int rt, int r) {
+    const int y = y0 + wave * RT + rt, x = x0 + 4 * g + r;
+    return (y < H && x < W) ? (img * H + y) * W + x : a.n_out;
+  });
+}
+
+static int dense2d_forced() {
+  const char *t = getenv("DF3D_DENSE2D");
+  return (t && (t[0] == '0' || t[0] == '1')) ? t[0] - '0' : -1;
+}
+
+static bool dense2d_faster(int cin, int cout, int groups, int batch, int H, int W) {
+  return cin == 512 && cout == 64 && groups == 1 && (long long)batch * cdiv(H, 8) * cdiv(W, 16) >= 256;
+}
+
+#define DF3D_HALO_SHAPES(X) X(256, 128) X(128, 128) X(64, 128) X(512, 64)
+static bool halo_shape_ok(int cin, int cw) {
+#define X(CIN, CW) \
+  if (cin == CIN && cw == CW) return true;
+  DF3D_HALO_SHAPES(X)
+#undef X
+  return false;
+}
+static int launch_conv2d_halo(int cin, int cw, const SplitConvArgs &a, hipStream_t stream) {
+  const dim3 grid(a.dB * cdiv(a.dH, 8) * cdiv(a.dW, 16), a.gy);
+#define X(CIN, CW)                                                                                   \
+  if (cin == CIN && cw == CW) {                                                                      \
+    hipLaunchKernelGGL((conv2d_halo_kernel<CIN, CW, 2>), grid, dim3(256), 0, stream, a);             \
+    return DF3D_OK;                                                                                  \
+  }
+  DF3D_HALO_SHAPES(X)
+#undef X
+  return DF3D_EINVAL;
+}
+
 #define DF3D_CONV_SHAPES(X) \
   X(256, 256, wide, 1)      \
   X(256, 128, wide, 1)      \
@@ -1362,10 +1539,19 @@
   void *out_rows;
   const int32_t *order;
   bool tag_both;
+  int dense_b = 0, dense_h = 0, dense_w = 0;
 };
 
+static bool use_dense2d(const ConvFormat &f, const ConvCall &c) {
+  if (c.dense_h <= 0 || c.kvol != 9 || f.parts != 2 || c.out_cols || c.order || c.residual) return false;
+  if (!halo_shape_ok(c.cin, c.cout > 128 ? 128 : c.cout)) return false;
+  const int forced = dense2d_forced();
+  if (forced >= 0) return forced == 1;
+  return dense2d_faster(c.cin, c.cout, c.groups, c.dense_b, c.dense_h, c.dense_w);
+}
+
 static int conv_launch(const ConvFormat &f, const char *entry, const ConvCall &c, hipStream_t stream) {
-  DF3D_CHECK_ARG(c.in && c.packed && c.nbr && (c.out || c.out_rows), "%s: null argument", entry);
+  DF3D_CHECK_ARG(c.in && c.packed && (c.out || c.out_rows), "%s: null argument", entry);
   DF3D_CHECK_ARG(c.kvol > 0 && c.kvol <= DF3D_MAX_KVOL, "%s: kernel volume %d unsupported", entry, c.kvol);
   DF3D_CHECK_ARG(shape_ok(f.parts, c.cin, c.cout), "%s: cin=%d cout=%d has no %s kernel", entry, c.cin, c.cout, f.what);
   DF3D_CHECK_ARG(c.groups >= 1 && c.groups <= 65535, "%s: groups", entry);
@@ -1381,6 +1567,13 @@
     DF3D_CHECK_ARG(c.out_channels % 8 == 0 && (long long)c.groups * c.cout <= c.out_channels,
                    "%s: %d x %d output columns do not fit %d-channel rows", entry, c.groups, c.cout, c.out_channels);
   }
+  if (c.dense_h > 0 || c.dense_w > 0 || c.dense_b > 0)
+    DF3D_CHECK_ARG(c.dense_b > 0 && c.dense_h > 0 && c.dense_w > 0 && (long long)c.dense_b * c.dense_h * c.dense_w == c.n_out &&
+                       c.n_in == c.n_out && c.kvol == 9,
+                   "%s: %d maps of %d x %d are not the %d -> %d rows of a 3 x 3 same convolution", entry, c.dense_b, c.dense_h,
+                   c.dense_w, c.n_in, c.n_out);
+  const bool halo = use_dense2d(f, c);
+  DF3D_CHECK_ARG(c.nbr || halo, "%s: null argument", entry);
   if (c.n_out == 0) return DF3D_OK;
   const char *dbg = f.tuning ? getenv("DF3D_OS_DBG") : nullptr;
   SplitConvArgs a = {(const u32x4 *)c.in, (const u32x4 *)c.packed, c.nbr, c.bias, c.scale, c.shift, (const float *)c.residual,
@@ -1392,7 +1585,8 @@
 #endif
   int rec = timing_rec_begin(c.cin, c.cout * c.groups, c.kvol, c.n_out, c.nbr,
                              f.timing | (c.tag_both && c.out && c.out_rows ? f.both_bit : 0), stream);
-  int rc = f.launch(c.cin, c.cout, a, stream);
+  if (halo) a.dB = c.dense_b, a.dH = c.dense_h, a.dW = c.dense_w;
+  int rc = halo ? launch_conv2d_halo(c.cin, c.cout > 128 ? 128 : c.cout, a, stream) : f.launch(c.cin, c.cout, a, stream);
   if (rc) return rc;
   timing_rec_end(rec, stream);
   DF3D_LAUNCH_CHECK();
@@ -1534,6 +1728,17 @@
                      (hipStream_t)stream_);
 }
 
+extern "C" int df3d_conv2d_rows_split(const void *in_split, int batch, int H, int W, int in_channels, int cin, int in_group_stride,
+                                      const void *packed_filters, int cout, int groups, const int32_t *nbr, const float *bias,
+                                      const float *scale, const float *shift, int relu, float *out, int out_channels,
+                                      void *out_split, void *stream_) {
+  DF3D_CHECK_ARG(batch > 0 && H > 0 && W > 0 && (long long)batch * H * W <= 0x7fffffffLL, "conv2d_rows_split: bad map geometry");
+  ConvCall c{in_split, batch * H * W, in_channels, cin, in_group_stride, packed_filters, 9, cout, groups, nbr, batch * H * W,
+             bias, scale, shift, nullptr, relu, out, out_channels, nullptr, out_split, nullptr, false};
+  c.dense_b = batch, c.dense_h = H, c.dense_w = W;
+  return conv_launch(conv_format(2), "conv2d_rows_split", c, (hipStream_t)stream_);
+}
+
 extern "C" int df3d_rows_to_bf16(const float *features, long long n, int c, void *rows_bf16, void *stream_) {
   hipStream_t stream = (hipStream_t)stream_;
   DF3D_CHECK_ARG(c > 0 && c % 8 == 0 && n >= 0, "rows_to_bf16: channels must be a multiple of 8 (got %d)", c);
diff --git a/3d-dual-fusion_amd/dualfusion/_lib.py b/3d-dual-fusion_amd/dualfusion/_lib.py
--- a/3d-dual-fusion_amd/dualfusion/_lib.py
+++ b/3d-dual-fusion_amd/dualfusion/_lib.py
@@ -164,6 +164,8 @@
                                               c_void_p]),
     "df3d_conv_rows_split": (c_int, [c_void_p, c_int, c_int, c_int, c_int, c_void_p, c_int, c_int, c_int, c_void_p, c_int,
                                      c_void_p, c_void_p, c_void_p, c_int, c_void_p, c_int, c_void_p, c_void_p, c_void_p]),
+    "df3d_conv2d_rows_split": (c_int, [c_void_p, c_int, c_int, c_int, c_int, c_int, c_int, c_void_p, c_int, c_int, c_void_p,
+                                       c_void_p, c_void_p, c_void_p, c_int, c_void_p, c_int, c_void_p, c_void_p]),
     "df3d_conv_packed_weight_bytes3": (c_size_t, [c_int, c_int, c_int]),
     "df3d_conv_pack_weights3": (c_int, [c_void_p, c_int, c_int, c_int, c_int, c_void_p, c_void_p]),
     "df3d_split_rows3": (c_int, [c_void_p, ctypes.c_longlong, c_int, c_void_p, c_void_p]),
diff --git a/3d-dual-fusion_amd/dualfusion/apitimer.py b/3d-dual-fusion_amd/dualfusion/apitimer.py
--- a/3d-dual-fusion_amd/dualfusion/apitimer.py
+++ b/3d-dual-fusion_amd/dualfusion/apitimer.py
@@ -5,7 +5,7 @@
 _NO_STREAM = ("df3d_version", "df3d_last_error", "df3d_device_count", "df3d_device_arch", "df3d_timing_", "df3d_ffn_set_precision",
               "df3d_conv_tile_count", "df3d_bn_rows_supported", "df3d_bn_rows_scratch_doubles", "df3d_debug_")
 CONV_ENTRIES = ("df3d_sparse_conv_fused", "df3d_sparse_conv_grouped", "df3d_sparse_conv_fused_tiled", "df3d_sparse_conv_split", "df3d_sparse_conv_bf16",
-                "df3d_conv_rows_split", "df3d_backbone_run")
+                "df3d_conv_rows_split", "df3d_conv2d_rows_split", "df3d_backbone_run")
 
 
 def _ops_stream():
diff --git a/3d-dual-fusion_amd/dualfusion/heads.py b/3d-dual-fusion_amd/dualfusion/heads.py
--- a/3d-dual-fusion_amd/dualfusion/heads.py
+++ b/3d-dual-fusion_amd/dualfusion/heads.py
@@ -342,10 +342,10 @@
         n = B * H * W
         G = plan["groups"]
         _, s1 = _ops.conv_rows_split(split, 512, 0, plan["shared"], 64, 1, nbr, n, plan["s_bias"], plan["s_scale"],
-                                     plan["s_shift"], relu=True, want_out=False, want_split=True)
+                                     plan["s_shift"], relu=True, want_out=False, want_split=True, dense=(B, H, W))
         _, s2 = _ops.conv_rows_split(s1, 64, 0, plan["mid"], 64 * plan["mid_pair"], G // plan["mid_pair"], nbr, n,
                                      plan["mid_bias"], plan["mid_scale"], plan["mid_shift"], relu=True, want_out=False,
-                                     want_split=True)
+                                     want_split=True, dense=(B, H, W))
         if (plan["fin_w4"] is not None and os.environ.get("DF3D_HEAD_FINAL", "valu") == "valu"
                 and _ops.CONV_PRECISION != "split3"):
             if "fin_pk" not in plan:
@@ -452,10 +452,10 @@
         n = B * H * W
         T = len(self.tasks)
         _, s1 = _ops.conv_rows_split(split, 512, 0, plan["shared"], 64, 1, nbr, n, plan["s_bias"], plan["s_scale"],
-                                     plan["s_shift"], relu=True, want_out=False, want_split=True)
+                                     plan["s_shift"], relu=True, want_out=False, want_split=True, dense=(B, H, W))
         _, s2 = _ops.conv_rows_split(s1, 64, 0, sites["hm_mid"], 64 * sites["hm_pair"], T // sites["hm_pair"], nbr, n,
                                      sites["hm_bias"], sites["hm_scale"], sites["hm_shift"], relu=True, want_out=False,
-                                     want_split=True)
+                                     want_split=True, dense=(B, H, W))
         out = _ops.head_final_conv(s2, B, H, W, sites["hm_w4"], sites["hm_b4"], sites["hm_cols_dev"], sites["hm_width"],
                                    packed=sites["hm_pk"])
         return out, s1, (B, H, W)
diff --git a/3d-dual-fusion_amd/dualfusion/necks.py b/3d-dual-fusion_amd/dualfusion/necks.py
--- a/3d-dual-fusion_amd/dualfusion/necks.py
+++ b/3d-dual-fusion_amd/dualfusion/necks.py
@@ -211,8 +211,9 @@
     @staticmethod
     def _run(layer, pad, rows, split, B, H, W, tables):
         nbr, Ho, Wo = RPN._table(layer, pad, B, H, W, tables, rows.device)
+        dense = (B, H, W) if (layer.kh, layer.kw, layer.stride, layer.pad, layer.transposed) == (3, 3, 1, 1, False) else None
         out, orows = _ops.conv(layer.weights, nbr, nbr.shape[1], rows=rows, operand=split, bias=layer.bias, scale=layer.scale,
-                               shift=layer.shift, relu=layer.relu)
+                               shift=layer.shift, relu=layer.relu, dense=dense)
         return out, orows, Ho, Wo
 
     @torch.no_grad()
diff --git a/3d-dual-fusion_amd/dualfusion/ops.py b/3d-dual-fusion_amd/dualfusion/ops.py
--- a/3d-dual-fusion_amd/dualfusion/ops.py
+++ b/3d-dual-fusion_amd/dualfusion/ops.py
@@ -561,7 +561,7 @@
 
 
 def _conv_operands(kind, rows, packed, nbr, n_out, cin, cout, bias, scale, shift, residual, relu, want_f32, want_rows,
-                   order=None):
+                   order=None, dense=None):
     lib = _lib.load()
     fmt = FORMATS[kind]
     _chk(rows, fmt.dtype, "operand rows")
@@ -583,6 +583,12 @@
     if kind == "bf16":
         rc = lib.df3d_sparse_conv_bf16(*head, _ptr(packed), K, cout, _ptr(nbr), int(n_out), *epilogue, _ptr(out), _ptr(orows),
                                        _stream())
+    elif kind == "split" and dense is not None and K == 9 and residual is None and order is None:
+        B, H, W = (int(v) for v in dense)
+        if B * H * W != int(n_out) or rows.shape[0] != int(n_out):
+            raise _lib.Df3dError("conv: dense=(%d, %d, %d) does not match %d -> %d rows" % (B, H, W, rows.shape[0], n_out))
+        rc = lib.df3d_conv2d_rows_split(_ptr(rows), B, H, W, cin, cin, 0, _ptr(packed), cout, 1, _ptr(nbr), _ptr(bias), _ptr(scale),
+                                        _ptr(shift), int(bool(relu)), _ptr(out), cout, _ptr(orows), _stream())
     elif kind == "split":
         rc = lib.df3d_sparse_conv_split(*head, _ptr(packed), K, cout, _ptr(nbr), int(n_out), *epilogue, _ptr(out), _ptr(orows),
                                         _ptr(order), -1 if order is not None else 0, _stream())
@@ -631,7 +637,7 @@
 
 
 def conv(filters, nbr, n_out, rows=None, operand=None, bias=None, scale=None, shift=None, residual=None, relu=False,
-         want_f32=True, want_operand=True, tiles=None, order=None):
+         want_f32=True, want_operand=True, tiles=None, order=None, dense=None):
     kind = filters.kind
     K, cin, cout = filters.filters.shape
     if kind == "fp32":
@@ -648,7 +654,7 @@
         return _conv_operands(kind, operand, filters.packed, nbr, n_out, cin, cout, bias, scale, shift, residual, relu,
                               want_f32, want_operand)
     return _conv_operands(kind, operand, filters.packed, nbr, n_out, cin, cout, bias, scale, shift, residual, relu, True,
-                          want_operand, order)
+                          want_operand, order, dense)
 
 
 def invert_neighbors(nbr, n_in):
@@ -740,7 +746,7 @@
 
 
 def conv_rows_split(in_split, cin, in_group_stride, packed, cout, groups, nbr, n_out, bias=None, scale=None, shift=None,
-                    relu=False, out_channels=None, out_cols=None, want_out=True, want_split=False, into=None):
+                    relu=False, out_channels=None, out_cols=None, want_out=True, want_split=False, into=None, dense=None):
     lib = _lib.load()
     _chk(in_split, torch.uint8, "in_split")
     _chk(packed, torch.uint8, "packed")
@@ -757,6 +763,15 @@
     dev = in_split.device
 
     def launch(po, oc, pcols, ps):
+        if dense is not None and fmt.parts == 2 and K == 9 and out_cols is None:
+            B, H, W = (int(v) for v in dense)
+            if B * H * W != int(n_out) or n_in != int(n_out):
+                raise _lib.Df3dError("conv_rows_split: dense=(%d, %d, %d) does not match %d -> %d rows" % (B, H, W, n_in, n_out))
+            rc = lib.df3d_conv2d_rows_split(_ptr(in_split), B, H, W, in_channels, int(cin), int(in_group_stride), _ptr(packed),
+                                            int(cout), int(groups), _ptr(nbr), _ptr(bias), _ptr(scale), _ptr(shift),
+                                            int(bool(relu)), po, oc, ps, _stream())
+            _lib.check(rc, "df3d_conv2d_rows_split")
+            return
         residual = (None,) if fmt.parts == 3 else ()
         rc = getattr(lib, fmt.conv_rows)(_ptr(in_split), n_in, in_channels, int(cin), int(in_group_stride), _ptr(packed), K,
                                          int(cout), int(groups), _ptr(nbr), int(n_out), _ptr(bias), _ptr(scale), _ptr(shift),
diff --git a/include/df3d_hip.h b/include/df3d_hip.h
--- a/include/df3d_hip.h
+++ b/include/df3d_hip.h
@@ -147,6 +147,11 @@
                          const void *packed_filters, int kvol, int cout, int groups, const int32_t *nbr, int n_out,
                          const float *bias, const float *scale, const float *shift, int relu, float *out,
                          int out_channels, const int32_t *out_cols, void *out_split, void *stream);
+
+int df3d_conv2d_rows_split(const void *in_split, int batch, int H, int W, int in_channels, int cin, int in_group_stride,
+                           const void *packed_filters, int cout, int groups, const int32_t *nbr, const float *bias,
+                           const float *scale, const float *shift, int relu, float *out, int out_channels, void *out_split,
+                           void *stream);
 
 size_t df3d_conv_packed_weight_bytes3(int kvol, int cin, int cout);
 int df3d_conv_pack_weights3(const float *filters, int groups, int kvol, int cin, int cout, void *packed, void *stream);
```

Result: no change. 408.6, median of 6 (+0.9%).
